# whatshap/whatshap

Measured on AMD Instinct MI355X. Metric: variant-columns/sec at max-coverage 20 (bipartition-costs/sec reported alongside), higher is better.
Workload: dtype u32; 1 GPU; synthetic diploid single-individual, max-coverage 20: 1 block of 200000 SNVs (BASELINE configs[2]); blocks=1, blocks_in_flight_per_gpu=1, tables_per_launch=1, max_coverage=20, optimal_cost_checksum=1611545, rendezvous=none

## Files before the change

### include/whatshap_amd_debug.h

```cpp
#ifndef WHATSHAP_AMD_DEBUG_H
#define WHATSHAP_AMD_DEBUG_H

#include "whatshap_amd.h"

#ifdef __cplusplus
extern "C" {
#endif

whamd_status_t whamd_debug_emulate_slot_plan(const whamd_readset_view* readset, const uint32_t* recombcost, size_t n_recombcost,
                                            const whamd_pedigree_view* pedigree, int distrust_genotypes,
                                            const uint32_t* positions, size_t n_positions, int slot_l, int symmetry,
                                            uint32_t* index_out, uint32_t* score_out, uint64_t* n_run_columns_out);

whamd_status_t whamd_debug_emulate_pedslot_plan(const whamd_readset_view* readset, const uint32_t* recombcost, size_t n_recombcost,
                                               const whamd_pedigree_view* pedigree, int distrust_genotypes,
                                               const uint32_t* positions, size_t n_positions, int slot_l,
                                               uint32_t* index_out, uint32_t* transmission_out, uint32_t* score_out,
                                               uint64_t* n_run_columns_out);

whamd_status_t whamd_debug_lazy_terms_check(const whamd_readset_view* readset, const uint32_t* recombcost, size_t n_recombcost,
                                            const whamd_pedigree_view* pedigree, int distrust_genotypes,
                                            const uint32_t* positions, size_t n_positions, const uint8_t* need, int rounds,
                                            int* lazy_out, uint64_t* differences_out, uint64_t* built_before_out, uint64_t* built_after_out);

// ... 22 lines not shown
whamd_status_t whamd_debug_progeny_gl_host(const whamd_progeny_depths_view* problems, uint64_t n_problems, float* const* table_out,
                                           double* const* table_f64_out);

whamd_status_t whamd_debug_haplotag_host(const whamd_haplotag_view* problems, uint64_t n_problems, whamd_haplotag_result** out);

whamd_status_t whamd_debug_poly_reorder_host(const whamd_poly_reorder_view* problems, uint64_t n_problems, double log_match, double log_err,
                                             whamd_poly_reorder_result** out);

whamd_status_t whamd_debug_poly_compare_host(const whamd_poly_compare_view* jobs, uint64_t n_jobs, whamd_poly_compare_result** out);

whamd_status_t whamd_debug_tagphase_host(const whamd_tagphase_view* problems, uint64_t n_problems, whamd_tagphase_result** out);

whamd_status_t whamd_debug_prior_genotypes_host(const whamd_prior_genotypes_view* problems, uint64_t n_problems, whamd_prior_genotypes_result** out);

typedef struct whamd_debug_kernel {
	const void* kernel;
	const char* name;
	int32_t large_lds_opted_in;
	int32_t debug_only;
} whamd_debug_kernel;
size_t whamd_debug_solve_kernels(whamd_debug_kernel* out, size_t capacity);

enum {
	WHAMD_LAUNCH_COLUMN = 0,
	WHAMD_LAUNCH_RUN = 1,
	WHAMD_LAUNCH_SLOT_RUN = 2,
	WHAMD_LAUNCH_BATCH = 3,
	WHAMD_LAUNCH_GROUP = 4,
	WHAMD_LAUNCH_GROUP_WALK = 5,
	WHAMD_LAUNCH_TAIL = 6,
	WHAMD_LAUNCH_WINDOW_WALK = 7,
	WHAMD_LAUNCH_TABLES = 8
};

typedef struct whamd_debug_launch {
	const void* kernel;
	uint32_t site;
	uint32_t grid_x, grid_y, block;
	uint32_t lds;
	uint32_t own_stream;
	uint32_t forward;
	int32_t lr, yflags, spec, stamps, tb, nf, ncols, threads;
	int32_t streamed, pack;
	int32_t tight, variant;
	int32_t T, n_ind, mode, wide;
	int32_t ped, sym;
	int32_t entries;
	int32_t preview;
	int32_t reserved;
	uint64_t count;
	const char* name;
} whamd_debug_launch;
whamd_status_t whamd_debug_dptable_launches(const whamd_dptable* table, whamd_debug_launch* out, size_t capacity, size_t* n_out);

typedef struct whamd_debug_preview {
	int32_t ran, continued;
	uint32_t pieces, launched_steps, agreed_steps, from_hook;
	const char* why_not;
} whamd_debug_preview;
whamd_status_t whamd_debug_dptable_preview(const whamd_dptable* table, whamd_debug_preview* out);

typedef struct whamd_debug_preview_plan_result {
	uint32_t n_pieces, pieces, steps, n_steps;
	int32_t chunked_predicted, chunked, windowed, reserved;
	uint32_t n_seeds_predicted, n_seeds, stride_predicted, stride;
	uint64_t arena_predicted, arena_laid_out, exchange_predicted, exchange_laid_out;
	const char* why_not;
} whamd_debug_preview_plan_result;
whamd_status_t whamd_debug_preview_plan(const whamd_readset_view* readset, const uint32_t* recombcost, size_t n_recombcost,
                                        const whamd_pedigree_view* pedigree, int distrust_genotypes,
                                        const uint32_t* positions, size_t n_positions, uint32_t pieces, whamd_debug_preview_plan_result* out,
                                        uint64_t* rec_predicted, uint64_t* rec_laid_out, uint32_t* spec_predicted, uint32_t* spec_laid_out, size_t capacity);

typedef struct whamd_debug_head_plan_result {
	uint32_t n_pieces, head_steps, n_steps, hook_calls;
	uint64_t digest, head_digest_in_hook, head_digest;
	uint32_t edge_yflags[2];
	uint32_t n_runs, n_components;
} whamd_debug_head_plan_result;
whamd_status_t whamd_debug_head_first_plan(const whamd_readset_view* readset, const uint32_t* recombcost, size_t n_recombcost,
                                           const whamd_pedigree_view* pedigree, int distrust_genotypes,
                                           const uint32_t* positions, size_t n_positions, uint32_t head_pieces, whamd_debug_head_plan_result* out);

typedef struct whamd_debug_genotype_run {
	uint32_t c0, ncols;
	uint32_t rescale_f, rescale_b, emit_f, emit_b;
	uint32_t n_part_out, part_out_f, part_out_b;
	uint32_t part_in_f, n_part_in_f, part_in_b, n_part_in_b;
	uint32_t reserved;
} whamd_debug_genotype_run;
whamd_status_t whamd_debug_genotype_run_plan(const whamd_readset_view* readset, const uint32_t* recombcost, size_t n_recombcost,
                                             const whamd_pedigree_view* pedigree, const uint32_t* positions, size_t n_positions,
                                             whamd_debug_genotype_run* out, size_t capacity, size_t* n_out, double* min_total_out);

whamd_status_t whamd_debug_poly_thread_inputs_host(const whamd_poly_thread_view* problems, uint64_t n_problems, whamd_poly_thread_result** out);
whamd_status_t whamd_debug_poly_select_clusters_host(uint64_t n_pos, const uint64_t* pc_ptr, const uint32_t* pc_cluster, const uint32_t* pc_total, uint32_t ploidy,
                                                     uint32_t max_cluster_gap, uint64_t* cov_ptr_out, uint32_t* cluster_out, uint8_t* readded_out, uint32_t* rank_out);
whamd_status_t whamd_debug_poly_haplotypes_host(const uint32_t* paths, uint64_t n_pos, uint32_t ploidy, const uint64_t* pc_ptr, const uint32_t* pc_cluster,
                                                const int8_t* pc_consensus, int8_t* haplotypes_out);

#ifdef __cplusplus
}
#endif

#endif
```

### whatshap_amd/_native.py

```python

from __future__ import annotations

import ctypes as C
import os
import threading
from typing import Optional, Sequence

import numpy as np

_HERE = os.path.dirname(os.path.abspath(__file__))
LIB_PATH = os.path.join(_HERE, "libwhatshap_amd.so")
DEBUG_LIB_PATH = os.path.join(_HERE, "libwhatshap_amd_debug.so")
ABI_VERSION = 3

WHAMD_OK = 0
WHAMD_ERR_INVALID = 1
WHAMD_ERR_MENDELIAN_CONFLICT = 2
WHAMD_ERR_UNSORTED = 3
WHAMD_ERR_UNSUPPORTED = 4
WHAMD_ERR_DEVICE = 5
WHAMD_ERR_OVERFLOW = 6
WHAMD_ERR_HOST = 7
GT_OTHER = 255

# ... 813 lines not shown
        except Exception:
            pass

    def positions(self) -> np.ndarray:
        out = np.zeros(self.n_columns, dtype=np.uint32)
        _check(self._L.whamd_dptable_positions(self._h, _ptr(out, C.c_uint32)))
        return out

    def optimal_score(self) -> int:
        v = C.c_uint32()
        _check(self._L.whamd_dptable_get_optimal_score(self._h, C.byref(v)))
        return int(v.value)

    def super_reads(self):
        n, ni = self.n_columns, self.n_individuals
        a0 = np.zeros((ni, n), dtype=np.uint8)
        a1 = np.zeros((ni, n), dtype=np.uint8)
        q = np.zeros((ni, n), dtype=np.uint32)
        tv = np.zeros(n, dtype=np.uint32)
        sid = np.zeros(ni, dtype=np.uint32)
        _check(self._L.whamd_dptable_get_super_reads(
            self._h, _ptr(a0, C.c_uint8), _ptr(a1, C.c_uint8), _ptr(q, C.c_uint32), _ptr(tv, C.c_uint32), _ptr(sid, C.c_uint32)))
        return a0, a1, q, tv, sid

    def partitioning(self) -> np.ndarray:
        out = np.zeros(self.n_reads, dtype=np.uint8)
        _check(self._L.whamd_dptable_get_optimal_partitioning(self._h, _ptr(out, C.c_uint8)))
        return out

    def index_path(self):
        idx = np.zeros(self.n_columns, dtype=np.uint32)
        tv = np.zeros(self.n_columns, dtype=np.uint32)
        _check(self._L.whamd_dptable_get_index_path(self._h, _ptr(idx, C.c_uint32), _ptr(tv, C.c_uint32)))
        return idx, tv

    def stats(self) -> dict:
        s = SolveStats()
        _check(self._L.whamd_dptable_get_stats(self._h, C.byref(s)))
        return s.as_dict()


def plan_summary(problem: ProblemArrays, path: str = "auto") -> dict:
    out = PlanSummary()
    _check(lib().whamd_plan_summarize(*problem.call_args(), path.encode(), C.byref(out)))
    return out.as_dict()


def emulate_slot_plan(problem: ProblemArrays, n_columns: int, slot_l: int = 11, symmetry: int = 1, slot_r: int = 2):
    if slot_r >= 3:
        slot_l += 100
    elif slot_r <= 1:
        slot_l += 200
    idx = np.zeros(max(n_columns, 1), dtype=np.uint32)
    score = C.c_uint32()
    ncols = C.c_uint64()
    D = debug_lib()
    _check(D.whamd_debug_emulate_slot_plan(*problem.call_args(), C.c_int(slot_l), C.c_int(symmetry), _ptr(idx, C.c_uint32),
                                           C.byref(score), C.byref(ncols)), D)
    return idx[:n_columns], int(score.value), int(ncols.value)


def emulate_pedslot_plan(problem: ProblemArrays, n_columns: int, slot_l: int = 0):
    idx = np.zeros(max(n_columns, 1), dtype=np.uint32)
    trans = np.zeros(max(n_columns, 1), dtype=np.uint32)
    score = C.c_uint32()
    ncols = C.c_uint64()
    D = debug_lib()
    _check(D.whamd_debug_emulate_pedslot_plan(*problem.call_args(), C.c_int(slot_l), _ptr(idx, C.c_uint32), _ptr(trans, C.c_uint32),
                                              C.byref(score), C.byref(ncols)), D)
    return idx[:n_columns], trans[:n_columns], int(score.value), int(ncols.value)


def debug_lazy_terms_check(problem: ProblemArrays, need=None, rounds: int = 1) -> dict:
    D = debug_lib()
    fn = D.whamd_debug_lazy_terms_check
    fn.restype = C.c_int
    lazy, diff, before, after = C.c_int(), C.c_uint64(), C.c_uint64(), C.c_uint64()
    need_arr = None if need is None else np.ascontiguousarray(need, dtype=np.uint8)
    _check(fn(*problem.call_args(), None if need_arr is None else _ptr(need_arr, C.c_uint8), C.c_int(int(rounds)), C.byref(lazy), C.byref(diff),
              C.byref(before), C.byref(after)), D)
    return {"lazy": bool(lazy.value), "differences": int(diff.value), "built_before": int(before.value), "built_after": int(after.value)}


class DebugGenotypeRun(C.Structure):
    _fields_ = [(name, C.c_uint32) for name in ("c0", "ncols", "rescale_f", "rescale_b", "emit_f", "emit_b", "n_part_out", "part_out_f", "part_out_b",
                                                "part_in_f", "n_part_in_f", "part_in_b", "n_part_in_b", "reserved")]


def debug_genotype_run_plan(problem: ProblemArrays):
    D = debug_lib()
    fn = D.whamd_debug_genotype_run_plan
    fn.restype = C.c_int
    a = problem.call_args()
    args = (a[0], a[1], a[2], a[3], a[5], a[6])
    n, min_total = C.c_size_t(), C.c_double()
    status = fn(*args, None, C.c_size_t(0), C.byref(n), C.byref(min_total))
    if status == WHAMD_ERR_UNSUPPORTED:
        return None
    _check(status, D)
    runs = (DebugGenotypeRun * max(n.value, 1))()
    _check(fn(*args, runs, C.c_size_t(n.value), C.byref(n), C.byref(min_total)), D)
    names = [f[0] for f in DebugGenotypeRun._fields_ if f[0] != "reserved"]
    return [{k: int(getattr(runs[i], k)) for k in names} for i in range(n.value)], float(min_total.value)


class DebugKernel(C.Structure):
    _fields_ = [("kernel", C.c_void_p), ("name", C.c_char_p), ("large_lds_opted_in", C.c_int32), ("debug_only", C.c_int32)]


LAUNCH_SITES = ("column", "run", "slot_run", "batch", "group", "group_walk", "tail", "window_walk", "tables")
LAUNCH_FACTS = ("lr", "yflags", "spec", "stamps", "tb", "nf", "ncols", "threads", "streamed", "pack", "tight", "variant", "T", "n_ind", "mode", "wide",
                "ped", "sym", "entries")


class DebugLaunch(C.Structure):
    _fields_ = ([("kernel", C.c_void_p), ("site", C.c_uint32), ("grid_x", C.c_uint32), ("grid_y", C.c_uint32), ("block", C.c_uint32), ("lds", C.c_uint32),
                 ("own_stream", C.c_uint32), ("forward", C.c_uint32)] + [(f, C.c_int32) for f in LAUNCH_FACTS] +
                [("preview", C.c_int32), ("reserved", C.c_int32), ("count", C.c_uint64), ("name", C.c_char_p)])


class DebugPreview(C.Structure):
    _fields_ = [("ran", C.c_int32), ("continued", C.c_int32), ("pieces", C.c_uint32), ("launched_steps", C.c_uint32), ("agreed_steps", C.c_uint32),
                ("from_hook", C.c_uint32), ("why_not", C.c_char_p)]


def debug_preview(table) -> dict:
    D = debug_lib()
    if table._L is not D:
        raise ValueError("the preview's record exists in the debug library only (use_debug_library() before the table is made)")
    out = DebugPreview()
    _check(D.whamd_debug_dptable_preview(table._h, C.byref(out)), D)
    return {"ran": bool(out.ran), "continued": bool(out.continued), "pieces": int(out.pieces), "launched_steps": int(out.launched_steps),
            "agreed_steps": int(out.agreed_steps), "from_hook": bool(out.from_hook), "why_not": (out.why_not or b"").decode()}


class DebugHeadPlan(C.Structure):
    _fields_ = [("n_pieces", C.c_uint32), ("head_steps", C.c_uint32), ("n_steps", C.c_uint32), ("hook_calls", C.c_uint32),
                ("digest", C.c_uint64), ("head_digest_in_hook", C.c_uint64), ("head_digest", C.c_uint64),
                ("edge_yflags", C.c_uint32 * 2), ("n_runs", C.c_uint32), ("n_components", C.c_uint32)]


def debug_head_first_plan(problem: ProblemArrays, head_pieces: int = 0) -> dict:
    D = debug_lib()
    fn = D.whamd_debug_head_first_plan
    fn.restype = C.c_int
    out = DebugHeadPlan()
    _check(fn(*problem.call_args(), C.c_uint32(head_pieces), C.byref(out)), D)
    rec = {name: int(getattr(out, name)) for name, _ in DebugHeadPlan._fields_ if name != "edge_yflags"}
    rec["edge_yflags"] = tuple(None if v == 0xFFFFFFFF else int(v) for v in out.edge_yflags)
    return rec


class DebugPreviewPlan(C.Structure):
    _fields_ = [("n_pieces", C.c_uint32), ("pieces", C.c_uint32), ("steps", C.c_uint32), ("n_steps", C.c_uint32),
                ("chunked_predicted", C.c_int32), ("chunked", C.c_int32), ("windowed", C.c_int32), ("reserved", C.c_int32),
                ("n_seeds_predicted", C.c_uint32), ("n_seeds", C.c_uint32), ("stride_predicted", C.c_uint32), ("stride", C.c_uint32),
                ("arena_predicted", C.c_uint64), ("arena_laid_out", C.c_uint64), ("exchange_predicted", C.c_uint64), ("exchange_laid_out", C.c_uint64),
                ("why_not", C.c_char_p)]


def debug_preview_plan(problem: ProblemArrays, pieces: int = 0) -> dict:
    D = debug_lib()
    fn = D.whamd_debug_preview_plan
    fn.restype = C.c_int
    out = DebugPreviewPlan()
    _check(fn(*problem.call_args(), C.c_uint32(pieces), C.byref(out), None, None, None, None, C.c_size_t(0)), D)
# ... 182 lines not shown
```

### whatshap_amd/csrc/c_api.cpp

```cpp
#include <cstdio>
#include <cstdlib>
#include <cstring>
#include <functional>
#include <memory>
#include <new>
#include <stdexcept>
#include <string>

#include "api_guard.h"
#include "debug_build.h"
#ifdef WHAMD_DEBUG_BUILD
#include "../../include/whatshap_amd_debug.h"
#endif
#include "device_runtime.h"
#include "device_table.h"
#include "genotype.h"
#include "genotype_plan.h"
#include "heuristic.h"
#include "host_parallel.h"
#include "problem.h"
#include "resident.h"
#include "slots.h"
#include <algorithm>
#include <vector>

using namespace whamd;

struct whamd_dptable {
	Problem problem;
	Solution solution;
	DeviceTable device;
	whamd_solve_stats stats{};
	int device_index = 0;
	bool uploaded = false;
	bool solved = false;
	bool in_flight = false;
};

namespace {

thread_local std::string g_last_error;

}

namespace whamd {
void set_last_error(const std::string& msg) { g_last_error = msg; }
}

extern "C" {

int whamd_abi_version(void) { return WHAMD_ABI_VERSION; }

int whamd_device_count(void) { return DeviceTable::device_count(); }

whamd_status_t whamd_device_pci_bus_id(int device, char* out, size_t capacity) {
	if (!out || capacity < 16) return fail(WHAMD_ERR_INVALID, "whamd_device_pci_bus_id: buffer of at least 16 bytes expected");
	std::string id;
	if (!DeviceTable::device_pci_bus_id(device, id)) return fail(WHAMD_ERR_DEVICE, "no HIP device " + std::to_string(device));
	if (id.size() + 1 > capacity) return fail(WHAMD_ERR_INVALID, "whamd_device_pci_bus_id: buffer too small");
	std::memcpy(out, id.c_str(), id.size() + 1);
	return WHAMD_OK;
}

const char* whamd_last_error(void) { return g_last_error.c_str(); }

namespace {
whamd_status_t apply_option(whamd_dptable* t, const std::string& k, const char* value);

whamd_status_t create_table(const whamd_readset_view* readset, const uint32_t* recombcost, size_t n_recombcost, const whamd_pedigree_view* pedigree,
                            int distrust_genotypes, const uint32_t* positions, size_t n_positions, const char* const* keys, const char* const* values,
                            size_t n_options, int device, whamd_dptable** out) {
	if (!out) return fail(WHAMD_ERR_INVALID, "out is NULL");
	*out = nullptr;
	if (n_options && (!keys || !values)) return fail(WHAMD_ERR_INVALID, "option arrays are NULL");
	const double t0 = now_ms();
	std::unique_ptr<whamd_dptable> t(new whamd_dptable());
	std::string msg;
	struct ThreadsGuard { uint32_t saved = whamd::host_threads_override(); ~ThreadsGuard() { whamd::host_threads_override() = saved; } } threads_guard;
	for (size_t i = 0; i < n_options; ++i) {
		if (!keys[i] || !values[i]) return fail(WHAMD_ERR_INVALID, "null option");
		if (std::string(keys[i]) == "host_threads") whamd::host_threads_override() = (uint32_t)std::max(0, std::atoi(values[i]));
	}
	whamd_status_t st = build_problem(readset, recombcost, n_recombcost, pedigree, distrust_genotypes != 0,
	                                  positions, n_positions, t->problem, msg, false, true);
	if (st != WHAMD_OK) return fail(st, msg);
	const double t1 = now_ms();
	t->device_index = device;
	t->device.set_thread_budget(whamd::host_threads_override() != 0);
	for (size_t i = 0; i < n_options; ++i) {
		if (std::string(keys[i]) == "host_threads") continue;
		st = apply_option(t.get(), keys[i], values[i]);
		if (st != WHAMD_OK) return st;
	}
	st = t->device.upload(t->problem, device, msg, true);
	if (st != WHAMD_OK) return fail(st, msg);
	if (getenv("WHAMD_DEBUG_TIMING"))
		fprintf(stderr, "[whamd timing] create: flatten %.1f ms, plan + upload %.1f ms\n", t1 - t0, now_ms() - t1);
	t->uploaded = true;
	t->stats.host_prepare_ms = now_ms() - t0;
	t->stats.host_flatten_ms = t1 - t0;
	*out = t.release();
	return WHAMD_OK;
}
}

whamd_status_t whamd_dptable_create(const whamd_readset_view* readset, const uint32_t* recombcost,
                                    size_t n_recombcost, const whamd_pedigree_view* pedigree,
                                    int distrust_genotypes, const uint32_t* positions, size_t n_positions,
                                    int device, whamd_dptable** out) {
	return guarded([&]() -> whamd_status_t {
		return create_table(readset, recombcost, n_recombcost, pedigree, distrust_genotypes, positions, n_positions, nullptr, nullptr, 0, device, out);
	});
}

whamd_status_t whamd_dptable_create_with_options(const whamd_readset_view* readset, const uint32_t* recombcost,
                                                 size_t n_recombcost, const whamd_pedigree_view* pedigree,
                                                 int distrust_genotypes, const uint32_t* positions, size_t n_positions,
                                                 const char* const* keys, const char* const* values, size_t n_options,
                                                 int device, whamd_dptable** out) {
	return guarded([&]() -> whamd_status_t {
		return create_table(readset, recombcost, n_recombcost, pedigree, distrust_genotypes, positions, n_positions, keys, values, n_options, device, out);
	});
}

namespace {

whamd_status_t begin_enqueue(whamd_dptable* t) {
	if (!t) return fail(WHAMD_ERR_INVALID, "table is NULL");
	if (t->in_flight) return fail(WHAMD_ERR_INVALID, "a solve of this table is already in flight");
	std::string msg;
	if (!t->uploaded) {
		whamd_status_t st = t->device.upload(t->problem, t->device_index, msg);
		if (st != WHAMD_OK) return fail(st, msg);
		t->uploaded = true;
	}
	const Problem& p = t->problem;
	whamd_solve_stats& s = t->stats;
	s.n_columns = p.n_cols;
	s.n_cells = p.n_cells;
	s.n_costs = p.n_cells * p.T;
	s.algorithmic_bytes = p.algorithmic_bytes;
	s.max_coverage = p.max_k;
	s.transmissions = p.T;
	t->solved = false;
	return WHAMD_OK;
}

}

whamd_status_t whamd_dptable_enqueue(whamd_dptable* t) {
	return guarded([&]() -> whamd_status_t {
	whamd_status_t st = begin_enqueue(t);
	if (st != WHAMD_OK) return st;
	std::string msg;
	t->device.set_side_by_side(false);
	st = t->device.enqueue(t->problem, t->solution, msg);
	if (st != WHAMD_OK) return fail(st, msg);
	t->in_flight = true;
// ... 479 lines not shown
			if (rc.mode != RES_MODE_GENERIC) s.n_vectorised_columns++;
			if (rc.nfold) ok = ok && rc.nfold <= RES_MAXFOLD && i >= rc.nfold;
			ok = ok && c + 1 < p.n_cols;
		}
		ok = ok && stage == sg.stage_words;
		const uint64_t lds = sg.kind == 1
			? (((uint64_t)sg.ncols * (PED_LDSWORDS + PED_TABLE) + (uint64_t)sg.n_terms * 2 + 3) & ~3ull) * 4 + 2 * (16ull << sg.max_l) + (uint64_t)sg.stage_words * 8
			: (uint64_t)sg.ncols * (64 + RES_TABLE) * 4 + 2 * (4ull << sg.max_l) + (uint64_t)sg.stage_words * 8;
		ok = ok && lds <= 160 * 1024;
		s.max_lds_bytes = std::max<uint64_t>(s.max_lds_bytes, lds);
		s.max_run_columns = std::max<uint64_t>(s.max_run_columns, sg.ncols);
		s.max_workgroups = std::max<uint64_t>(s.max_workgroups, 1ull << (sg.g - sg.half));
		if (sg.half) s.n_halved_runs++;
		s.n_resident_columns += sg.ncols;
		s.backtrace_bytes += (uint64_t)sg.stage_words * (1ull << sg.g) * 8;
	}
	ok = ok && expect == p.n_cols;
	for (uint32_t c = 0; c < p.n_cols; ++c) ok = ok && seen[c] == 1;
	s.invariants_ok = ok ? 1 : 0;
	*out = s;
	return WHAMD_OK;
	});
}

#ifdef WHAMD_DEBUG_BUILD
whamd_status_t whamd_debug_emulate_slot_plan(const whamd_readset_view* readset, const uint32_t* recombcost, size_t n_recombcost,
                                            const whamd_pedigree_view* pedigree, int distrust_genotypes, const uint32_t* positions,
                                            size_t n_positions, int slot_l, int symmetry, uint32_t* index_out, uint32_t* score_out,
                                            uint64_t* n_run_columns_out) {
	return guarded([&]() -> whamd_status_t {
	const int lr = slot_l >= 200 ? 1 : slot_l >= 100 ? 3 : 2;
	if (slot_l >= 100) slot_l -= slot_l >= 200 ? 200 : 100;
	Problem p;
	std::string msg;
	whamd_status_t st = build_problem(readset, recombcost, n_recombcost, pedigree, distrust_genotypes != 0, positions,
	                                  n_positions, p, msg);
	if (st != WHAMD_OK) return fail(st, msg);
	SlotPlan sp;
	if (p.T != 1 || !plan_forward_slots(p, slot_l, symmetry, sp, lr)) return fail(WHAMD_ERR_UNSUPPORTED, "slot runs apply to a single individual only");
	std::vector<uint32_t> path;
	uint32_t score = 0;
	if (!emulate_slot_plan(p, sp, path, score, msg)) return fail(WHAMD_ERR_INVALID, "slot plan inconsistent: " + msg);
	if (index_out && !path.empty()) std::memcpy(index_out, path.data(), path.size() * sizeof(uint32_t));
	if (score_out) *score_out = score;
	if (n_run_columns_out) *n_run_columns_out = sp.n_run_columns;
	return WHAMD_OK;
	});
}

whamd_status_t whamd_debug_emulate_pedslot_plan(const whamd_readset_view* readset, const uint32_t* recombcost, size_t n_recombcost,
                                               const whamd_pedigree_view* pedigree, int distrust_genotypes, const uint32_t* positions,
                                               size_t n_positions, int slot_l, uint32_t* index_out, uint32_t* transmission_out,
                                               uint32_t* score_out, uint64_t* n_run_columns_out) {
	return guarded([&]() -> whamd_status_t {
	Problem p;
	std::string msg;
	whamd_status_t st = build_problem(readset, recombcost, n_recombcost, pedigree, distrust_genotypes != 0, positions,
	                                  n_positions, p, msg);
	if (st != WHAMD_OK) return fail(st, msg);
	SlotPlan sp;
	if (p.T == 1 || !plan_forward_slots(p, slot_l > 0 ? -slot_l : 0, 0, sp) || !sp.ped)
		return fail(WHAMD_ERR_UNSUPPORTED, "pedigree slot runs apply to tables with one or two trios whose columns need at most 4 cost forms per transmission value");
	std::vector<uint32_t> path, trans;
	uint32_t score = 0;
	if (!emulate_pedslot_plan(p, sp, path, trans, score, msg)) return fail(WHAMD_ERR_INVALID, "pedigree slot plan inconsistent: " + msg);
	if (index_out && !path.empty()) std::memcpy(index_out, path.data(), path.size() * sizeof(uint32_t));
	if (transmission_out && !trans.empty()) std::memcpy(transmission_out, trans.data(), trans.size() * sizeof(uint32_t));
	if (score_out) *score_out = score;
	if (n_run_columns_out) *n_run_columns_out = sp.n_run_columns;
	return WHAMD_OK;
	});
}
whamd_status_t whamd_debug_lazy_terms_check(const whamd_readset_view* readset, const uint32_t* recombcost, size_t n_recombcost,
                                            const whamd_pedigree_view* pedigree, int distrust_genotypes, const uint32_t* positions, size_t n_positions,
                                            const uint8_t* need_in, int rounds, int* lazy_out, uint64_t* differences_out, uint64_t* built_before_out,
                                            uint64_t* built_after_out) {
	return guarded([&]() -> whamd_status_t {
	Problem eager, lazy;
	std::string msg;
	whamd_status_t st = build_problem(readset, recombcost, n_recombcost, pedigree, distrust_genotypes != 0, positions, n_positions, eager, msg);
	if (st != WHAMD_OK) return fail(st, msg);
	st = build_problem(readset, recombcost, n_recombcost, pedigree, distrust_genotypes != 0, positions, n_positions, lazy, msg, false, true);
	if (st != WHAMD_OK) return fail(st, msg);
	if (lazy_out) *lazy_out = lazy.lazy_terms ? 1 : 0;
	const uint32_t n = eager.n_cols;
	uint64_t before = 0, after = 0, diff = 0;
	for (uint32_t c = 0; c < n; ++c) before += lazy.term_end(c, lazy.T - 1) > lazy.term_begin(c, 0);
	std::vector<uint8_t> need(n, 1);
	if (need_in) for (uint32_t c = 0; c < n; ++c) need[c] = need_in[c] != 0;
	rounds = std::max(1, rounds);
	for (int r = 0; r < rounds; ++r) {
		std::vector<uint8_t> part(n, 0);
		for (uint32_t c = 0; c < n; ++c) part[c] = need[c] && (int)(c % (uint32_t)rounds) == r;
		st = fill_lazy_terms(lazy, part, msg);
		if (st != WHAMD_OK) return fail(st, msg);
	}
	for (uint32_t c = 0; c < n; ++c) {
		after += lazy.term_end(c, lazy.T - 1) > lazy.term_begin(c, 0);
		if (!need[c]) continue;
		bool same = true;
		for (uint32_t t = 0; t < eager.T && same; ++t) {
			const uint64_t a0 = eager.term_begin(c, t), a1 = eager.term_end(c, t), b0 = lazy.term_begin(c, t), b1 = lazy.term_end(c, t);
			same = a1 - a0 == b1 - b0;
			for (uint64_t i = 0; same && i < a1 - a0; ++i)
				same = eager.terms[a0 + i].c == lazy.terms[b0 + i].c && eager.terms[a0 + i].plus == lazy.terms[b0 + i].plus && eager.terms[a0 + i].minus == lazy.terms[b0 + i].minus;
		}
		diff += !same;
	}
	if (eager.fterm_kind != lazy.fterm_kind || eager.fterms.size() != lazy.fterms.size()) diff += n;
	else for (size_t i = 0; i < eager.fterms.size(); ++i) if (eager.fterms[i].c != lazy.fterms[i].c || eager.fterms[i].plus != lazy.fterms[i].plus || eager.fterms[i].minus != lazy.fterms[i].minus) { ++diff; break; }
	if (lazy.value_bound < eager.value_bound) diff += n;
	if (differences_out) *differences_out = diff;
	if (built_before_out) *built_before_out = before;
	if (built_after_out) *built_after_out = after;
	return WHAMD_OK;
	});
}

size_t whamd_debug_solve_kernels(whamd_debug_kernel* out, size_t capacity) { return DeviceTable::debug_solve_kernels(out, capacity); }

whamd_status_t whamd_debug_dptable_launches(const whamd_dptable* table, whamd_debug_launch* out, size_t capacity, size_t* n_out) {
	if (!table || !n_out) return fail(WHAMD_ERR_INVALID, "null argument");
	if (!table->solved) return fail(WHAMD_ERR_INVALID, "the table has not been solved: its ledger is read after whamd_dptable_wait");
	*n_out = table->device.debug_launches(out, capacity);
	return WHAMD_OK;
}

whamd_status_t whamd_debug_dptable_preview(const whamd_dptable* table, whamd_debug_preview* out) {
	if (!table || !out) return fail(WHAMD_ERR_INVALID, "null argument");
	table->device.debug_preview(out);
	return WHAMD_OK;
}

whamd_status_t whamd_debug_preview_plan(const whamd_readset_view* readset, const uint32_t* recombcost, size_t n_recombcost,
                                        const whamd_pedigree_view* pedigree, int distrust_genotypes,
                                        const uint32_t* positions, size_t n_positions, uint32_t pieces, whamd_debug_preview_plan_result* out,
                                        uint64_t* rec_predicted, uint64_t* rec_laid_out, uint32_t* spec_predicted, uint32_t* spec_laid_out, size_t capacity) {
	return guarded([&]() -> whamd_status_t {
	if (!out) return fail(WHAMD_ERR_INVALID, "out is NULL");
	Problem p;
	std::string msg;
	whamd_status_t st = build_problem(readset, recombcost, n_recombcost, pedigree, distrust_genotypes != 0, positions, n_positions, p, msg);
	if (st != WHAMD_OK) return fail(st, msg);
	st = DeviceTable::debug_preview_plan(p, pieces, out, rec_predicted, rec_laid_out, spec_predicted, spec_laid_out, capacity, msg);
	return st == WHAMD_OK ? WHAMD_OK : fail(st, msg);
	});
}

whamd_status_t whamd_debug_head_first_plan(const whamd_readset_view* readset, const uint32_t* recombcost, size_t n_recombcost,
                                           const whamd_pedigree_view* pedigree, int distrust_genotypes,
                                           const uint32_t* positions, size_t n_positions, uint32_t head_pieces, whamd_debug_head_plan_result* out) {
	return guarded([&]() -> whamd_status_t {
	if (!out) return fail(WHAMD_ERR_INVALID, "out is NULL");
	Problem p;
	std::string msg;
	whamd_status_t st = build_problem(readset, recombcost, n_recombcost, pedigree, distrust_genotypes != 0, positions, n_positions, p, msg);
	if (st != WHAMD_OK) return fail(st, msg);
	if (p.T != 1) return fail(WHAMD_ERR_UNSUPPORTED, "the head hook applies to a single individual only");
	*out = whamd_debug_head_plan_result{};
	auto mix = [](uint64_t& h, const void* data, size_t bytes) {
		const unsigned char* b = static_cast<const unsigned char*>(data);
		for (size_t i = 0; i < bytes; ++i) h = (h ^ b[i]) * 1099511628211ull;
	};
	auto runs_digest = [&mix](const SlotPlan& sp, size_t n_runs) {
		uint64_t h = 1469598103934665603ull;
		for (size_t ri = 0; ri < n_runs; ++ri) {
			const SlotRun& run = sp.runs[ri];
			mix(h, &run, sizeof run);
			mix(h, sp.rows.data() + run.row_off, (size_t)run.ncols * sizeof(SlotRow));
			mix(h, sp.bt_cols.data() + run.row_off, (size_t)run.ncols * sizeof(SlotBtCol));
			mix(h, sp.ctrl.data() + run.ctrl_off, (size_t)SLOT_CTRL_WORDS * 4);
			mix(h, sp.end_slots.data() + sp.end_off[ri], run.n_ends);
		}
		return h;
	};
	SlotPlan sp;
	SlotPlanHead head;
	const uint32_t n_pieces = slot_plan_pieces(p.n_cols);
	head.col_limit = slot_plan_piece_begin(p.n_cols, std::min(head_pieces, n_pieces));
	uint32_t calls = 0, head_steps = 0;
	uint64_t in_hook = 0;
	head.at_head = [&](uint32_t n_head) {
		++calls;
		head_steps = n_head;
		in_hook = runs_digest(sp, n_head);
	};
	if (!plan_forward_slots(p, 11, 1, sp, 2, false, head_pieces ? &head : nullptr)) return fail(WHAMD_ERR_UNSUPPORTED, "the table is not eligible for slot runs");
	out->n_pieces = n_pieces;
	out->head_steps = head_steps;
	out->n_steps = (uint32_t)sp.steps.size();
	out->hook_calls = calls;
	out->head_digest_in_hook = in_hook;
	out->head_digest = runs_digest(sp, head_steps);
	out->n_runs = (uint32_t)sp.runs.size();
	out->n_components = (uint32_t)sp.component_first_step.size();
	uint64_t h = runs_digest(sp, sp.runs.size());
	mix(h, sp.steps.data(), sp.steps.size() * sizeof(Step));
	mix(h, sp.end_off.data(), sp.end_off.size() * 4);
	mix(h, sp.start_slots.data(), sp.start_slots.size());
	mix(h, sp.start_off.data(), sp.start_off.size() * 4);
	mix(h, sp.f_exit.data(), sp.f_exit.size() * 4);
	for (const std::vector<uint8_t>& e : sp.exit_slot) mix(h, e.data(), e.size());
	mix(h, sp.col_to_row.data(), sp.col_to_row.size() * 4);
	mix(h, sp.component_first_step.data(), sp.component_first_step.size() * 4);
	mix(h, &sp.n_run_columns, sizeof sp.n_run_columns);
	out->digest = h;
	out->edge_yflags[0] = out->edge_yflags[1] = 0xFFFFFFFFu;
	if (head_steps) {
		out->edge_yflags[0] = sp.runs[head_steps - 1].yflags;
		if (head_steps < sp.steps.size() && sp.steps[head_steps].kind == 2) out->edge_yflags[1] = sp.runs[sp.steps[head_steps].index].yflags;
	}
	return WHAMD_OK;
	});
}

whamd_status_t whamd_debug_genotype_run_plan(const whamd_readset_view* readset, const uint32_t* recombcost, size_t n_recombcost,
                                             const whamd_pedigree_view* pedigree, const uint32_t* positions, size_t n_positions,
                                             whamd_debug_genotype_run* out, size_t capacity, size_t* n_out, double* min_total_out) {
	return guarded([&]() -> whamd_status_t {
	if (!n_out) return fail(WHAMD_ERR_INVALID, "n_out is NULL");
	Problem p;
	std::string msg;
	whamd_status_t st = build_problem(readset, recombcost, n_recombcost, pedigree, false, positions, n_positions, p, msg, true);
	if (st != WHAMD_OK) return fail(st, msg);
	GenotypeModel model;
	st = build_genotype_model(p, model, msg);
	if (st != WHAMD_OK) return fail(st, msg);
	GenoRunPlan pl;
// ... 259 lines not shown
```

### whatshap_amd/csrc/dp_device.hip

```cpp
#include <hip/hip_runtime.h>

#include <algorithm>
#include <atomic>
#include <cctype>
#include <chrono>
#include <cstdio>
#include <cstdlib>
#include <cstring>
#include <mutex>
#include <string>
#include <vector>

#include "debug_build.h"
#ifdef WHAMD_DEBUG_BUILD
#include "../../include/whatshap_amd_debug.h"
#endif
#include "device_runtime.h"
#include "device_table.h"
#include "genotype.h"
#include "table_plan.h"

namespace whamd {

namespace {
// ... 354 lines not shown

whamd_status_t DeviceTable::Impl::open(int dev, std::string& msg) {
	Impl& m = *this;
	m.device = dev;
	const whamd_status_t opened = open_device(dev, msg);
	if (opened != WHAMD_OK) return opened;
	if (!m.stream) {
		StreamSet ss;
		if (!streamset_take(dev, ss)) { msg = "could not create the table's stream and events"; return WHAMD_ERR_DEVICE; }
		m.adopt(ss);
	}
	m.release();
	if (!m.counted && dev >= 0 && dev < 64) { Impl::tables_on_device[dev].fetch_add(1); m.counted = true; }
	return WHAMD_OK;
}

whamd_status_t DeviceTable::Impl::choose_plan(Problem& p, TableBuild& b, bool from_create, std::string& msg) {
	Impl& m = *this;
	m.preview.tried = false;
	m.preview.from_hook = false;
	m.tp.wide = !select_kernels(p.T, p.n_ind, m.fused, m.keysfn);
	if (m.tp.wide && (p.T > (uint32_t)MAX_T_WIDE || p.n_ind > (uint32_t)MAX_IND_WIDE)) {
		msg = "no device kernel for T=" + std::to_string(p.T) + ", individuals=" + std::to_string(p.n_ind);
		return WHAMD_ERR_UNSUPPORTED;
	}
	for (uint32_t c = 0; c < p.n_cols && !m.tp.wide; ++c) m.tp.wide = p.term_end(c, p.T - 1) - p.term_begin(c, 0) > (uint64_t)COL_MAXTERMS;
	b.laps.lap("plan: kernels chosen, term counts scanned");
	b.force_keys = m.opt.path == "column_keys" || m.tp.wide;
	const bool want_resident = (m.opt.path == "auto" || m.opt.path == "resident") && !m.tp.wide;
	size_t free_b = 0, total_b = 0;
	HIP_TRY(hipMemGetInfo(&free_b, &total_b));
	if (free_b < total_b / 2) {
		genotype_release_cache();
		HIP_TRY(hipMemGetInfo(&free_b, &total_b));
	}
	if (free_b < total_b / 4) {
		arena_release();
		devpool_release();
		HIP_TRY(hipMemGetInfo(&free_b, &total_b));
	}
	free_b += arena_idle_bytes(m.device);
	b.free_b = free_b;
	b.laps.lap("plan: free device memory asked");
	int slot_lr = m.opt.slot_lr, slot_l = m.opt.slot_l;
	if (m.opt.shared_hint && p.T == 1 && p.max_k >= 18 && !m.opt.slot_l_set && m.opt.slot_lr == 2) { slot_lr = 3; slot_l = 12; }
	if (p.T == 1 && p.max_k >= 21 && p.max_k <= 22 && !m.opt.slot_l_set && m.opt.slot_lr == 2 && !debug_env("WHAMD_NO_WIDE_LAYOUT")) { slot_lr = 3; slot_l = 12; }
	m.tp.slot_lr_used = slot_lr;
	whamd_status_t head_status = WHAMD_OK;
	bool steps_adopted = false;
	auto adopt_steps = [&]() {
		m.tp.plan = ResidentPlan();
		m.tp.plan.steps = m.tp.splan.steps;
		m.tp.plan.component_first_step = m.tp.splan.component_first_step;
		m.tp.plan.col_to_res.assign(p.n_cols, -1);
		steps_adopted = true;
	};
	SlotPlanHead head;
	{
		const uint32_t n_pieces = slot_plan_pieces(p.n_cols);
		const uint32_t pieces = std::min(n_pieces - 1, preview_pieces_of(m.opt.preview_pieces, n_pieces));
		head.col_limit = slot_plan_piece_begin(p.n_cols, pieces);
		head.at_head = [&](uint32_t n_head) {
			if (n_head == 0) return;
			m.tp.use_slots = true;
			m.tp.table_bytes = 0;
			adopt_steps();
			b.laps.lap("plan: the planner up to the head's callback");
			m.preview.tried = true;
			m.preview.from_hook = true;
			head_status = m.start_preview(p, b, from_create, msg);
			if (m.preview.why != PV_RAN) m.preview.from_hook = false;
		};
	}
	bool head_first = from_create && p.T == 1 && m.opt.preview_mode != 0 && slot_plan_pieces(p.n_cols) >= 2 && !m.opt.shared_hint && !m.opt.side_by_side && !debug_env("WHAMD_NO_PREVIEW") &&
	                  !debug_env("WHAMD_NO_HEAD_FIRST");
	if (head_first && m.opt.preview_mode < 0)
		head_first = !m.opt.thread_budget && slot_plan_pieces(p.n_cols) >= 8 && m.alone_on_device();
	m.tp.use_slots = (m.opt.path == "auto" || m.opt.path == "slots") && !m.tp.wide &&
	              plan_forward_slots(p, p.T > 1 ? (m.opt.slot_l_set ? -m.opt.slot_l : 0) : std::max(8, slot_l), m.opt.symmetry, m.tp.splan, slot_lr, false, head_first ? &head : nullptr);
	if (head_status != WHAMD_OK) return head_status;
	b.laps.lap("plan: the planner");
	if (m.tp.use_slots && m.tp.splan.ped && m.tp.splan.table_words * 4ull > free_b / 4) m.tp.use_slots = false;
	m.tp.table_bytes = m.tp.use_slots && m.tp.splan.ped ? m.tp.splan.table_words * 4ull : 0ull;
	if (p.lazy_terms) {
		std::vector<uint8_t> need(p.n_cols, 1);
		if (m.tp.use_slots && m.tp.splan.ped) for (uint32_t c = 0; c < p.n_cols; ++c) need[c] = m.tp.splan.col_to_row[c] < 0;
		const whamd_status_t st = fill_lazy_terms(p, need, msg);
		if (st != WHAMD_OK) return st;
	}
	if (m.tp.use_slots) {
		if (!steps_adopted) adopt_steps();
	} else {
		m.tp.splan = SlotPlan();
		plan_forward(p, want_resident, m.opt.l_pref, m.opt.fold, m.tp.plan, m.opt.symmetry);
	}
	m.tp.device_superreads = p.n_ind == 1 && p.T == 1 && p.P == 2 && !p.distrust && p.h2p.size() >= 2 && p.h2p[0] == 0 && p.h2p[1] == 1 && p.genotype.size() >= p.n_cols &&
	                      !debug_env("WHAMD_HOST_SUPERREADS");
	b.laps.lap("plan: steps adopted, lazy terms");
	return WHAMD_OK;
}

void DeviceTable::Impl::dump_plan(const Problem& p) const {
	const Impl& m = *this;
	for (const Step& st : m.tp.plan.steps) {
		if (st.kind == 0) { fprintf(stderr, "[plan] column %u k=%u b=%u f=%u\n", st.index, p.k[st.index], p.b[st.index], p.f[st.index]); continue; }
		if (st.kind == 2) {
			const SlotRun& r = m.tp.splan.runs[st.index];
			fprintf(stderr, "[plan] slot run c0=%u ncols=%u g=%u L=%u half=%u ends=%u has_prev=%u in_identity=%u in_half=%u mirror_pos=%u in_occ=%x out_occ=%x mirror_out=%u\n",
			        r.c0, r.ncols, r.g, r.L, r.half, r.n_ends, r.has_prev, r.in_identity, r.in_half, r.in_mirror_pos, r.in_occ, r.out_occ, r.mirror_out);
			if (m.tp.splan.ped) fprintf(stderr, "[plan]   pedigree run: T=%u forms per value=%u table words=%u record words per workgroup=%u\n", 1u << m.tp.splan.pextra[st.index].tb,
			                         m.tp.splan.pextra[st.index].nf, m.tp.splan.pextra[st.index].s_off + r.ncols * 64u * pslot_ns(m.tp.splan.pextra[st.index].nf), m.tp.splan.pextra[st.index].rec_words);
			continue;
		}
		const ResSegment& sgm = m.tp.plan.segments[st.index];
		fprintf(stderr, "[plan] run c0=%u ncols=%u g=%u threads=%u max_l=%u stage_words=%u\n", sgm.c0, sgm.ncols, sgm.g, sgm.threads, sgm.max_l, sgm.stage_words);
		for (uint32_t i = 0; i < sgm.ncols; ++i) {
			const ResColumn& rc = m.tp.plan.columns[sgm.col_off + i];
			const ResBacktrace& rb = m.tp.plan.backtrace[sgm.col_off + i];
			fprintf(stderr, "[plan]   col %u mode=%u nfold=%u Lb=%u Lf=%u ebits=%u epos0=%u nthr=%u stage_off=%u nwords=%u | bt layout=%u n_g=%u n_l=%u\n",
			        sgm.c0 + i, rc.mode, rc.nfold, rc.Lb, rc.Lf, rc.ebits, rc.epos[0], rc.nthr, rc.stage_off, rc.nwords, rb.layout, rb.n_g, rb.n_l);
		}
	}
}

whamd_status_t DeviceTable::Impl::upload_column_arrays(const Problem& p, TableBuild& b, TableUploader& up, std::string& msg) {
	Impl& m = *this;
	const uint32_t n = b.n;
	static_assert(sizeof(CostTerm) == sizeof(DevTerm), "Problem::terms / fterms are uploaded as they are");
	const RawVec<CostTerm>& terms = p.terms;
	const int32_t* delta_src = p.delta.data();
	size_t delta_count = (size_t)p.col_ptr[n] * p.n_ind;
	if (p.n_ind == 0) { b.delta_fallback.assign(std::max<size_t>(p.col_ptr[n], 1), 0); delta_src = b.delta_fallback.data(); delta_count = b.delta_fallback.size(); }
	const bool sparse_columns = m.tp.use_slots && !b.ped_slots && p.T == 1 && !m.tp.windowed && !debug_env("WHAMD_DENSE_COLUMN_UPLOAD");
	if (sparse_columns) {
		std::vector<std::pair<size_t, size_t>> pc_cols, pc_delta, pc_tptr, pc_terms;
		for (uint32_t c = 0; c < n;) {
			if (m.tp.splan.col_to_row[c] >= 0) { ++c; continue; }
			uint32_t e = c + 1;
			while (e < n && m.tp.splan.col_to_row[e] < 0) ++e;
			pc_cols.emplace_back((size_t)c * sizeof(DevColumn), (size_t)e * sizeof(DevColumn));
			pc_delta.emplace_back((size_t)p.col_ptr[c] * p.n_ind * sizeof(int32_t), (size_t)p.col_ptr[e] * p.n_ind * sizeof(int32_t));
			pc_tptr.emplace_back((size_t)c * (p.T + 1) * sizeof(uint32_t), (size_t)e * (p.T + 1) * sizeof(uint32_t));
			pc_terms.emplace_back((size_t)p.term_ptr[(size_t)c * p.T] * sizeof(DevTerm), (size_t)p.term_ptr[(size_t)e * p.T] * sizeof(DevTerm));
			c = e;
		}
		HIP_TRY(up.up_pieces((void**)&m.dev.d_cols, m.tp.cols.data(), m.tp.cols.size() * sizeof(DevColumn), pc_cols));
		if (m.tp.device_superreads) HIP_TRY(up.up((void**)&m.dev.dp.delta, delta_src, delta_count * sizeof(int32_t)));
		else HIP_TRY(up.up_pieces((void**)&m.dev.dp.delta, delta_src, delta_count * sizeof(int32_t), pc_delta));
		HIP_TRY(up.up_pieces((void**)&m.dev.dp.term_ptr, b.term_ptr32.data(), b.term_ptr32.size() * sizeof(uint32_t), pc_tptr));
		HIP_TRY(up.up_pieces((void**)&m.dev.dp.terms, terms.data(), terms.size() * sizeof(DevTerm), pc_terms));
	} else {
		HIP_TRY(up.up((void**)&m.dev.d_cols, m.tp.cols.data(), m.tp.cols.size() * sizeof(DevColumn)));
		HIP_TRY(up.up((void**)&m.dev.dp.delta, delta_src, delta_count * sizeof(int32_t)));
		HIP_TRY(up.up((void**)&m.dev.dp.term_ptr, b.term_ptr32.data(), b.term_ptr32.size() * sizeof(uint32_t)));
		HIP_TRY(up.up((void**)&m.dev.dp.terms, terms.data(), terms.size() * sizeof(DevTerm)));
	}
	m.dev.dp.cols = m.dev.d_cols;
	if (m.tp.device_superreads) {
		m.dev.super_args = SuperreadArgs{};
		HIP_TRY(up.up((void**)&m.dev.super_args.col_ptr, p.col_ptr.data(), ((size_t)n + 1) * sizeof(uint64_t)));
		HIP_TRY(up.up((void**)&m.dev.super_args.genotype, p.genotype.data(), (size_t)n));
		m.dev.super_args.delta = m.dev.dp.delta;
		m.dev.super_args.n_cols = n;
		m.tp.super_words = (size_t)n + ((size_t)2 * n + 3) / 4;
	}
	b.d_fterms = nullptr;
	if (!p.fterms.empty()) HIP_TRY(up.up((void**)&b.d_fterms, p.fterms.data(), p.fterms.size() * sizeof(DevTerm)));
// ... 280 lines not shown
	e.units = m.dev.d_units; e.chunks = m.dev.d_chunks;
	e.n_chunks = (uint32_t)m.tp.chunks.size(); e.n_units = (uint32_t)m.tp.units.size(); e.n_orient_max = m.tp.n_orient_max; e.n_cols = n;
	e.path2 = m.dev.d_path2; e.trans2 = m.dev.d_trans2; e.out_score = m.dev.d_score; e.unit_x2 = m.dev.d_unit_x; e.guess = m.dev.d_guess; e.sel = m.dev.d_sel; e.counters = m.dev.d_bt_counters;
	e.path_index = m.dev.d_path_index; e.path_trans = m.dev.d_path_trans;
	if (m.tp.device_superreads) e.super = m.dev.super_args;
	void* d_entry = nullptr;
	HIP_TRY(up.alloc(&d_entry, sizeof(BtGroupEntry)));
	HIP_TRY(hipMemcpyAsync(d_entry, &m.dev.h_bt_entry, sizeof(BtGroupEntry), hipMemcpyHostToDevice, up.stream));
	HIP_TRY(hipEventRecord(m.ev_upload, up.stream));
	m.dev.d_bt_entry = (BtGroupEntry*)d_entry;
	return WHAMD_OK;
}

whamd_status_t DeviceTable::Impl::start_preview(const Problem& p, TableBuild& b, bool from_create, std::string& msg) {
	Impl& m = *this;
	Preview& pv = m.preview;
	PreviewPlan pp;
	plan_preview(p, m.opt, b, m.tp, from_create, m.alone_on_device(), pp);
	pv.why = pp.why;
	if (pp.why != PV_RAN) return WHAMD_OK;
	const uint32_t n = b.n, S = pp.steps, pieces = pp.pieces, end_col = pp.end_col, n_spec = pp.n_spec, stride = pp.stride, max_f = pp.max_f;
	const uint64_t bt = pp.arena, tab_words = pp.tab_words;
	const size_t ctrl_words = pp.ctrl_words;
	const bool chunked = pp.chunked;
	const std::vector<uint64_t>& rec = pp.rec;
	const std::vector<uint32_t>& spec = pp.spec;
	const std::vector<SlotRun>& runs = m.tp.splan.runs;
	b.laps.lap("preview: steps, offsets, seeds (host)");
	{
		const whamd_status_t taken = m.take_arena(bt, msg);
		if (taken != WHAMD_OK) return taken;
	}
	pv.exchange_bytes = (size_t)(1ull << max_f) * p.T * 4;
	HIP_TRY(pool_alloc(m.device, m.dev.allocations, (void**)&pv.d_pr[0], pv.exchange_bytes));
	HIP_TRY(pool_alloc(m.device, m.dev.allocations, (void**)&pv.d_pr[1], pv.exchange_bytes));
	pv.spec_bytes = chunked ? ((size_t)n_spec + 1) * stride * 8 : 0;
	if (chunked) HIP_TRY(pool_alloc(m.device, m.dev.allocations, (void**)&pv.spec_keys, pv.spec_bytes));
	DevProblem hdp{};
	hdp.n_cols = n; hdp.T = p.T; hdp.tbits = b.tbits; hdp.n_ind = p.n_ind;
	{
		const hipStream_t us = m.upload_stream;
		TableUploader up(m.device, us, pv.allocations);
		const size_t row_count = (size_t)end_col + SLOT_ROW_PAD;
		up.open_block(row_count * sizeof(SlotRow) + ctrl_words * 4 + (size_t)S * sizeof(SlotRun) + 4096);
		const SlotRun* d_runs = nullptr;
		HIP_TRY(up.up((void**)&hdp.slot_rows, m.tp.splan.rows.data(), row_count * sizeof(SlotRow)));
		HIP_TRY(up.up((void**)&hdp.slot_ctrl, m.tp.splan.ctrl.data(), ctrl_words * 4));
		HIP_TRY(up.up((void**)&d_runs, runs.data(), (size_t)S * sizeof(SlotRun)));
		HIP_TRY(up.alloc((void**)&hdp.slot_tab, tab_words * 4));
		HIP_TRY(up.flush());
		uint32_t most = 0;
		for (uint32_t k = 0; k < S; ++k) most = std::max<uint32_t>(most, ((runs[k].ncols + 8u) << (runs[k].g - runs[k].half)) + (runs[k].ncols + 8u) * ((runs[k].threads >> 6) + 64u));
		const uint32_t bx = std::max(1u, std::min(64u, (most + 255u) / 256u));
		for (uint32_t r0 = 0; r0 < S; r0 += 32768) hipLaunchKernelGGL(slot_tables, dim3(bx, std::min<uint32_t>(32768, S - r0)), dim3(256), 0, us, hdp, d_runs + r0, (uint32_t*)hdp.slot_tab);
		HIP_TRY(hipGetLastError());
		HIP_TRY(hipEventRecord(m.ev_upload, us));
		if (up.unstaged_copies || !up.stage.image || !up.stage.park()) {
			HIP_TRY(hipStreamSynchronize(us));
			up.stage.finish();
		}
	}
	b.laps.lap("preview: rows, control words, tables: allocations + copies");
	{
		const whamd_status_t opted = opt_in_large_lds(m.device, msg);
		if (opted != WHAMD_OK) return opted;
	}
	const hipStream_t rs = m.stream;
	m.inflight.run_stream = rs;
	m.own_stream_used = true;
	HIP_TRY(hipStreamWaitEvent(rs, m.ev_upload, 0));
	hdp.bt = (uint8_t*)m.dev.d_arena;
	hdp.spec_keys = pv.spec_keys;
	hdp.spec_stride = stride;
	if (chunked) HIP_TRY(hipMemsetAsync(pv.spec_keys, 0xFF, pv.spec_bytes, rs));
	m.inflight.timing_pending = false;
	HIP_TRY(hipEventRecord(m.ev0, rs));
	m.tp.use_chunks = chunked;
#ifdef WHAMD_DEBUG_BUILD
	m.ledger.clear();
#endif
	pv.runs.resize(S);
	uint64_t launches = 0;
	pv.launching = true;
	if (b.laps.on)
		fprintf(stderr, "[whamd timing] preview: first launch %.2f ms after the create's upload began, at t = %.2f ms (%s)\n", b.laps.since_origin_ms(), timing_stamp_ms(),
		        pv.from_hook ? "from the planner's head hook" : "behind the plan");
	for (uint32_t k = 0; k < S; ++k) {
		SlotBatchEntry e{};
		e.run = runs[k];
		if (k == 0) e.run.has_prev = 0;
		e.run.rec_lo = (uint32_t)rec[k];
		e.run.rec_hi = (uint32_t)(rec[k] >> 32);
		e.run.spec_id = spec[k];
		e.prev = pv.d_pr[k & 1u];
		e.cur = pv.d_pr[(k & 1u) ^ 1u];
		pv.runs[k] = e.run;
		m.launch_slot_run(hdp, e, launches);
	}
	pv.launching = false;
	HIP_TRY(hipGetLastError());
	HIP_TRY(hipEventRecord(m.ev3, rs));
	pv.dp = hdp;
	pv.use_chunks = chunked;
	pv.why = PV_RAN;
	pv.pieces = pieces;
	pv.launched = S;
	pv.launches = launches;
	pv.pending = true;
	b.laps.lap("preview: launches submitted");
	return WHAMD_OK;
}

void DeviceTable::Impl::verify_preview() {
	Impl& m = *this;
	Preview& pv = m.preview;
	pv.agreed = 0;
	if (!pv.launched) return;
	const bool same_ground = m.tp.use_slots && !m.tp.windowed && m.tp.jobs.size() == 1 && m.tp.lanes.size() == 1 && m.dev.dp.bt == pv.dp.bt && m.dev.dp.spec_keys == pv.dp.spec_keys &&
	                         m.tp.use_chunks == pv.use_chunks && (!m.tp.use_chunks || m.dev.dp.spec_stride == pv.dp.spec_stride) && !m.dev.dp.dbg && !m.dev.dp.dbg_flags &&
	                         m.dev.d_pr[0] == pv.d_pr[0] && m.dev.d_pr[1] == pv.d_pr[1] && !m.opt.side_by_side;
	for (uint32_t k = 0; same_ground && k < pv.launched && k + 1 < m.tp.schedule.size(); ++k) {
		const SuperStep& ss = m.tp.schedule[k];
		if (ss.entry_count != 1 || !ss.singles.empty() || ss.ck_load >= 0 || ss.ck_save >= 0 || ss.bt_window >= 0) break;
		const SlotBatchEntry& e = m.tp.slot_entries[ss.entry_off];
		if (std::memcmp(&e.run, &pv.runs[k], sizeof(SlotRun)) != 0 || e.prev != pv.d_pr[k & 1u] || e.cur != pv.d_pr[(k & 1u) ^ 1u] || e.score_out) break;
		++pv.agreed;
	}
	if (const char* at = debug_env("WHAMD_PREVIEW_MISMATCH_AT")) pv.agreed = std::min<uint32_t>(pv.agreed, (uint32_t)std::max(0, atoi(at)));
	if (getenv("WHAMD_DEBUG_TIMING"))
		fprintf(stderr, "[whamd timing] preview: %u plan pieces, %u steps launched, %u agree with the schedule\n", pv.pieces, pv.launched, pv.agreed);
}

whamd_status_t DeviceTable::upload(Problem& p, int device, std::string& msg, bool from_create) {
	Impl& m = *impl_;
	whamd_status_t st = m.open(device, msg);
	if (st != WHAMD_OK || p.n_cols == 0) return st;
	TableBuild b;
	b.n = p.n_cols;
	b.tbits = 2 * p.n_triples;
	b.ni = std::max<uint32_t>(p.n_ind, 1);
	m.dev.dp.n_cols = b.n;
	m.dev.dp.T = p.T;
	m.dev.dp.tbits = b.tbits;
	m.dev.dp.n_ind = p.n_ind;
	m.upload_stream = debug_env("WHAMD_UPLOAD_ON_TABLE_STREAM") ? nullptr : upload_stream_of(device);
	if (!m.upload_stream) m.upload_stream = m.stream;
	if (m.upload_stream == m.stream) m.own_stream_used = true;
	if ((st = m.choose_plan(p, b, from_create, msg)) != WHAMD_OK) return st;
	b.ped_slots = m.tp.use_slots && m.tp.splan.ped;
	b.laps.next_stage();
	if (debug_env("WHAMD_DEBUG_PLAN")) m.dump_plan(p);
	if (!m.preview.tried && (st = m.start_preview(p, b, from_create, msg)) != WHAMD_OK) return st;
	if ((st = describe_columns(p, b, m.tp, msg)) != WHAMD_OK) return st;
	if ((st = lay_out_arena(p, m.opt, b, m.tp, msg)) != WHAMD_OK) return st;
	TableUploader up(device, m.upload_stream, m.dev.allocations);
	b.laps.lap("staging area taken");
	up.open_block(upload_bound(p, b, m.tp));
	b.laps.lap("staging image sized, device block taken");
	if ((st = m.upload_column_arrays(p, b, up, msg)) != WHAMD_OK) return st;
	if ((st = m.upload_slot_arrays(b, up, msg)) != WHAMD_OK) return st;
	make_jobs(m.opt, m.tp);
	make_units(b, m.tp);
	if ((st = m.make_windows(b, up, msg)) != WHAMD_OK) return st;
	if ((st = m.take_result_block(b.n, up, msg)) != WHAMD_OK) return st;
	if ((st = m.make_chunks(p, up, msg)) != WHAMD_OK) return st;
	if ((st = m.take_solve_buffers(p, b, up, msg)) != WHAMD_OK) return st;
	if ((st = m.make_lanes(b, up, msg)) != WHAMD_OK) return st;
	if ((st = make_schedule(b, m.dev.dp, m.dev.d_job_scores, m.tp, msg)) != WHAMD_OK) return st;
	make_briefs(m.tp);
	if ((st = m.upload_entries(up, msg)) != WHAMD_OK) return st;
	if ((st = m.launch_table_kernels(p, b, up, msg)) != WHAMD_OK) return st;
	b.laps.summary((double)b.bt / 1e9);
	if ((st = m.arm_debug_stamps(up, msg)) != WHAMD_OK) return st;
	if ((st = opt_in_large_lds(device, msg)) != WHAMD_OK) return st;
	if ((st = m.record_group_backtrace(b.n, up, msg)) != WHAMD_OK) return st;
	m.verify_preview();
	return WHAMD_OK;
}

namespace {

SegmentFn segment_kernel(bool stamps, bool sym) {
#ifdef WHAMD_DEBUG_BUILD
	if (stamps) return resident_segment<true, true>;
#endif
	return sym ? resident_segment<false, true> : resident_segment<false, false>;
}

PedSegmentFn ped_segment_kernel(bool stamps, bool spec) {
#ifdef WHAMD_DEBUG_BUILD
	if (stamps) return resident_segment_ped<true>;
#endif
	return spec ? resident_segment_ped<false, true> : resident_segment_ped<false>;
}

ResBatchFn resident_batch_kernel(bool sym) { return sym ? resident_batch<true> : resident_batch<false>; }

#ifdef WHAMD_DEBUG_BUILD
PedSlotRunFn pedslot_runx_kernel(uint32_t tb, uint32_t nf, uint32_t xc, bool spec) {
#define WHAMD_ROW(TB, NF) { pedslot_runx<TB, NF, 16, true>, pedslot_runx<TB, NF, 16, false>, pedslot_runx<TB, NF, 32, true>, pedslot_runx<TB, NF, 32, false> }
	static const PedSlotRunFn table[6][4] = {WHAMD_ROW(2, PSLOT_FACT), WHAMD_ROW(2, 16), WHAMD_ROW(2, 2), WHAMD_ROW(2, 4), WHAMD_ROW(4, 2), WHAMD_ROW(4, 4)};
#undef WHAMD_ROW
	const int row = tb == 2 ? (nf == (uint32_t)PSLOT_FACT ? 0 : nf == 16 ? 1 : nf == 2 ? 2 : 3) : (nf == 2 ? 4 : 5);
	return table[row][(xc == 16 ? 0 : 2) + (spec ? 0 : 1)];
}
#endif

PedSlotRunFn pedslot_run_kernel(uint32_t tb, uint32_t nf, bool spec, bool packed) {
#define WHAMD_ROW(TB, NF) { pedslot_run<TB, NF, true, true>, pedslot_run<TB, NF, true, false>, pedslot_run<TB, NF, false, true>, pedslot_run<TB, NF, false, false> }
	static const PedSlotRunFn table[7][4] = {WHAMD_ROW(2, PSLOT_FACT), WHAMD_ROW(4, PSLOT_FACT4), WHAMD_ROW(2, 16), WHAMD_ROW(2, 2), WHAMD_ROW(2, 4), WHAMD_ROW(4, 2), WHAMD_ROW(4, 4)};
#undef WHAMD_ROW
	const int row = tb == 2 && nf == (uint32_t)PSLOT_FACT ? 0 : tb == 4 && nf == (uint32_t)PSLOT_FACT4 ? 1 : tb == 2 ? (nf == 16 ? 2 : nf == 2 ? 3 : 4) : (nf == 2 ? 5 : 6);
	return table[row][(spec ? 0 : 2) + (packed ? 0 : 1)];
}

SlotRunXFn slot_runx_kernel(uint32_t xc, bool stamps, bool spec) {
#define WHAMD_PAIR(XC, STAMPS) { slot_runx<2, XC, STAMPS, true>, slot_runx<2, XC, STAMPS, false> }
#ifdef WHAMD_DEBUG_BUILD
	static const SlotRunXFn stamped[2][2] = {WHAMD_PAIR(24, true), WHAMD_PAIR(32, true)};
	if (stamps && xc) return stamped[xc == 24 ? 0 : 1][spec ? 0 : 1];
#endif
	static const SlotRunXFn table[5][2] = {WHAMD_PAIR(0, false), WHAMD_PAIR(8, false), WHAMD_PAIR(16, false), WHAMD_PAIR(24, false), WHAMD_PAIR(32, false)};
#undef WHAMD_PAIR
	return table[xc / 8][spec ? 0 : 1];
}

SlotRunFn slot_run_kernel(uint32_t lr, bool yform, bool stamps, bool spec) {
#ifdef WHAMD_DEBUG_BUILD
#define WHAMD_ROW(LR, YF) { slot_run<LR, true, true, YF>, slot_run<LR, true, false, YF>, slot_run<LR, false, true, YF>, slot_run<LR, false, false, YF> }
#else
#define WHAMD_ROW(LR, YF) { nullptr, nullptr, slot_run<LR, false, true, YF>, slot_run<LR, false, false, YF> }
#endif
	static const SlotRunFn table[5][4] = {WHAMD_ROW(3, true), WHAMD_ROW(3, false), WHAMD_ROW(1, false), WHAMD_ROW(2, true), WHAMD_ROW(2, false)};
#undef WHAMD_ROW
	const int row = lr == 3 ? (yform ? 0 : 1) : lr == 1 ? 2 : (yform ? 3 : 4);
	return table[row][(stamps ? 0 : 2) + (spec ? 0 : 1)];
}
// ... 861 lines not shown
```

### whatshap_amd/csrc/problem.cpp

```cpp
#include "debug_build.h"
#include "problem.h"

#include <algorithm>
#include <chrono>
#include <cmath>
#include <cstdio>
#include <cstdlib>
#include <cstring>
#include <thread>
#include <unordered_map>

namespace whamd {

namespace {

bool id_to_index(const Problem& p, uint32_t id, uint32_t& index, std::string& msg) {
	for (uint32_t i = p.n_ind; i-- > 0;) {
		if (p.individual_id[i] == id) {
			index = i;
			return true;
		}
	}
	msg = "Individual with ID " + std::to_string(id) + " not present in pedigree.";
	return false;
}

bool build_partitions(Problem& p, std::string& msg) {
	p.P = 2 * (p.n_ind - p.n_triples);
	p.h2p.assign((size_t)p.T * p.n_ind * 2, -1);
	std::vector<int> child_triple(p.n_ind, -1);
	for (uint32_t i = 0; i < p.n_triples; ++i) child_triple[p.triples[i][2]] = (int)i;
	std::vector<uint32_t> order;
	std::vector<uint8_t> state(p.n_ind, 0);
	for (uint32_t root = 0; root < p.n_ind; ++root) {
		std::vector<std::pair<uint32_t, int>> stack{{root, 0}};
		while (!stack.empty()) {
			auto [i, phase] = stack.back();
			stack.pop_back();
			if (state[i] == 2) continue;
			if (phase == 1) {
				state[i] = 2;
				order.push_back(i);
				continue;
			}
			if (state[i] == 1) {
				msg = "pedigree relationships contain a cycle";
				return false;
			}
			state[i] = 1;
			stack.push_back({i, 1});
			if (child_triple[i] >= 0) {
				stack.push_back({p.triples[child_triple[i]][1], 0});
				stack.push_back({p.triples[child_triple[i]][0], 0});
			}
		}
	}
	for (uint32_t t = 0; t < p.T; ++t) {
		int8_t* map = p.h2p.data() + (size_t)t * p.n_ind * 2;
		int next = 0;
		for (uint32_t i = 0; i < p.n_ind; ++i) {
			if (child_triple[i] < 0) {
				map[2 * i] = (int8_t)next;
				map[2 * i + 1] = (int8_t)(next + 1);
				next += 2;
			}
		}
		for (uint32_t i : order) {
			int ti = child_triple[i];
			if (ti < 0) continue;
			uint32_t father = p.triples[ti][0], mother = p.triples[ti][1];
			map[2 * i] = map[2 * father + (((t >> (2 * ti)) & 1) ? 0 : 1)];
			map[2 * i + 1] = map[2 * mother + (((t >> (2 * ti + 1)) & 1) ? 0 : 1)];
		}
	}
	return true;
}

}

whamd_status_t build_problem(const whamd_readset_view* rs, const uint32_t* recombcost, size_t n_recombcost,
                             const whamd_pedigree_view* ped, bool distrust, const uint32_t* positions,
                             size_t n_positions, Problem& p, std::string& msg, bool columns_only, bool lazy_fact_terms) {
	if (!rs || !ped) {
		msg = "null readset or pedigree view";
		return WHAMD_ERR_INVALID;
	}
	const bool timing = getenv("WHAMD_DEBUG_TIMING") != nullptr;
	auto lap_t = std::chrono::steady_clock::now();
	long lap_faults = timing ? thread_minor_faults() : 0;
	auto lap = [&](const char* what) {
		if (!timing) return;
		const auto now = std::chrono::steady_clock::now();
		const long faults = thread_minor_faults();
		fprintf(stderr, "[whamd timing]   flatten: %s %.2f ms (%ld page faults of this thread)\n", what, std::chrono::duration<double, std::milli>(now - lap_t).count(), faults - lap_faults);
		lap_faults = faults;
		lap_t = now;
	};
	p.n_reads = rs->n_reads;
	const uint64_t nnz = rs->n_reads ? rs->read_ptr[rs->n_reads] : 0;
	p.read_ptr.assign(rs->n_reads + 1, 0);
	if (rs->n_reads) std::copy(rs->read_ptr, rs->read_ptr + rs->n_reads + 1, p.read_ptr.begin());
	{
		const uint32_t n_threads = host_threads(nnz, 1u << 18);
		std::vector<uint8_t> bad(n_threads, 0);
		parallel_ranges(nnz, n_threads, [&](uint64_t i0, uint64_t i1, uint32_t t) {
			if (i1 <= i0) return;
			uint8_t worst = 0;
			for (uint64_t i = i0; i < i1; ++i) worst = std::max(worst, rs->var_allele[i]);
			bad[t] = worst > WHAMD_ALLELE_BLANK;
		});
		for (uint8_t v : bad) {
			if (v) {
				msg = "read allele must be 0 (REF), 1 (ALT) or 2 (BLANK)";
				return WHAMD_ERR_INVALID;
			}
		}
	}
	lap("copies of the read arrays");
	p.n_ind = ped->n_individuals;
	p.n_triples = ped->n_triples;
	p.n_variants = ped->n_variants;
	p.individual_id.assign(ped->individual_id, ped->individual_id + p.n_ind);
	const size_t ng = (size_t)p.n_ind * p.n_variants;
	if (ng) p.genotype.assign(ped->genotype, ped->genotype + ng);
	p.have_gl = ped->genotype_likelihoods != nullptr;
	if (p.have_gl && ng) {
		p.gl.assign(ped->genotype_likelihoods, ped->genotype_likelihoods + ng * 3);
		if (ped->gl_present) {
			for (size_t i = 0; i < ng; ++i) {
				if (!ped->gl_present[i]) p.gl[3 * i] = p.gl[3 * i + 1] = p.gl[3 * i + 2] = std::nan("");
			}
		}
	}
	p.distrust = distrust;
	p.triples.resize(p.n_triples);
	for (uint32_t i = 0; i < p.n_triples; ++i) {
		for (int m = 0; m < 3; ++m) {
			if (!id_to_index(p, ped->triple_ids[3 * i + m], p.triples[i][m], msg)) return WHAMD_ERR_INVALID;
		}
	}
	if (columns_only) {
		if (p.n_triples > 2 || p.n_ind > (uint32_t)MAX_IND) {
			msg = "pedigree too large for the genotyping device path (at most " + std::to_string(MAX_IND) + " individuals and 2 trios)";
			return WHAMD_ERR_UNSUPPORTED;
		}
	} else if (p.n_triples > (uint32_t)MAX_TRIPLES_WIDE || p.n_ind > (uint32_t)MAX_IND_WIDE || 2 * (p.n_ind - std::min(p.n_ind, p.n_triples)) > 14) {
		msg = "pedigree too large for the device path (at most " + std::to_string(MAX_IND_WIDE) + " individuals, " + std::to_string(MAX_TRIPLES_WIDE) +
		      " trios, 14 founder haplotypes)";
		return WHAMD_ERR_UNSUPPORTED;
	}
	p.T = 1u << (2 * p.n_triples);

	if (positions == nullptr) {
		p.positions.resize(nnz);
		for (uint64_t i = 0; i < nnz; ++i) p.positions[i] = (uint32_t)rs->var_position[i];
		std::sort(p.positions.begin(), p.positions.end());
		p.positions.erase(std::unique(p.positions.begin(), p.positions.end()), p.positions.end());
	} else {
		p.positions.assign(positions, positions + n_positions);
	}
	p.n_cols = (uint32_t)p.positions.size();
	const uint32_t n = p.n_cols;
	lap("pedigree + positions");
	bool positions_increase = true;
	for (uint32_t i = 1; i < n && positions_increase; ++i) positions_increase = p.positions[i - 1] < p.positions[i];
	std::unordered_map<uint32_t, uint32_t> position_map;
	if (!positions_increase) {
		position_map.reserve(n * 2 + 1);
		for (uint32_t i = 0; i < n; ++i) position_map[p.positions[i]] = i;
	}
	auto column_of = [&](uint32_t position, uint32_t& col, uint32_t hint = 0) -> bool {
		if (positions_increase) {
			if (n == 0) return false;
			const uint32_t* pos0 = p.positions.data();
			size_t lo_i = hint < n ? hint : 0, step = 1;
			if (pos0[lo_i] > position) lo_i = 0;
			size_t hi_i = lo_i;
			while (hi_i < n && pos0[hi_i] < position) { lo_i = hi_i; hi_i += step; step <<= 1; }
			if (hi_i > n) hi_i = n;
			const auto it = std::lower_bound(p.positions.begin() + lo_i, p.positions.begin() + hi_i + (hi_i < n ? 1 : 0), position);
			if (it == p.positions.end() || *it != position) return false;
			col = (uint32_t)(it - p.positions.begin());
			return true;
		}
		const auto it = position_map.find(position);
		if (it == position_map.end()) return false;
		col = it->second;
		return true;
	};
	p.read_first_col.resize(p.n_reads);
	p.read_last_col.resize(p.n_reads);
	std::vector<uint32_t>&first_col = p.read_first_col, &last_col = p.read_last_col;
	{
		struct ReadError { uint32_t read = 0xFFFFFFFFu; whamd_status_t status = WHAMD_OK; std::string msg; };
		const uint32_t n_threads = positions_increase ? host_threads(p.n_reads, 1u << 14) : 1u;
		std::vector<ReadError> errors(n_threads);
		const uint64_t* ptr = rs->read_ptr;
		const int32_t* vp = rs->var_position;
		parallel_ranges(p.n_reads, n_threads, [&](uint64_t r0, uint64_t r1, uint32_t t) {
			auto fail_read = [&](uint32_t r, whamd_status_t st, std::string m) { errors[t].read = r; errors[t].status = st; errors[t].msg = std::move(m); };
			uint32_t hint_col = 0;
			for (uint32_t r = (uint32_t)r0; r < (uint32_t)r1; ++r) {
				const uint64_t lo = ptr[r], hi = ptr[r + 1];
				if (hi <= lo || hi > nnz) return fail_read(r, WHAMD_ERR_INVALID, "No variants present");
				const int pos = r == 0 ? 0 : ((ptr[r] > ptr[r - 1] && ptr[r] <= nnz) ? vp[ptr[r - 1]] : 0);
				if (vp[lo] < pos) return fail_read(r, WHAMD_ERR_UNSORTED, "ColumnIterator: reads in ReadSet are not sorted.");
				for (uint64_t i = lo + 1; i < hi; ++i) {
					if (!(vp[i - 1] < vp[i])) return fail_read(r, WHAMD_ERR_UNSORTED, "ColumnIterator: encountered read with unsorted variants.");
				}
				uint32_t fc = 0, lc = 0;
				if (vp[lo] < 0 || !column_of((uint32_t)vp[lo], fc, hint_col) || !column_of((uint32_t)vp[hi - 1], lc, fc) || fc > lc) {
					return fail_read(r, WHAMD_ERR_INVALID, "read " + std::to_string(r) + " starts or ends at a position that is not in the position list");
				}
				first_col[r] = fc;
				last_col[r] = lc;
				hint_col = fc;
			}
		});
		for (const ReadError& e : errors) {
			if (e.status != WHAMD_OK) {
				msg = e.msg;
				return e.status;
			}
		}
	}
	if (!positions_increase) {
		msg = "positions must be strictly increasing";
		return WHAMD_ERR_INVALID;
	}
	lap("position map + read validation");
	p.read_source.resize(p.n_reads);
	for (uint32_t r = 0; r < p.n_reads; ++r) {
		if (!id_to_index(p, (uint32_t)rs->read_sample_id[r], p.read_source[r], msg)) return WHAMD_ERR_INVALID;
	}
	if (n && p.n_ind && p.n_variants < n) {
		msg = "pedigree has fewer variants (" + std::to_string(p.n_variants) + ") than there are columns (" + std::to_string(n) + ")";
		return WHAMD_ERR_INVALID;
	}
	if (n && p.n_ind && distrust) {
		bool ok = p.have_gl;
		for (uint32_t i = 0; ok && i < p.n_ind; ++i) {
			for (uint32_t c = 0; ok && c < n; ++c) {
				for (int g = 0; g < 3; ++g) {
					const double v = p.gl[((size_t)i * p.n_variants + c) * 3 + g];
					if (!(v >= 0.0 && v <= 1e9)) ok = false;
				}
			}
		}
		if (!ok) {
			msg = "distrust_genotypes requires genotype likelihoods in [0, 1e9] for every individual and column";
			return WHAMD_ERR_INVALID;
		}
	}
	p.recomb.assign(n, n_recombcost ? recombcost[n_recombcost - 1] : 0u);
	for (uint32_t c = 0; c < n && c < n_recombcost; ++c) p.recomb[c] = recombcost[c];

	if (!build_partitions(p, msg)) return WHAMD_ERR_INVALID;
	if (n == 0) return WHAMD_OK;

	std::vector<uint32_t> start_idx(n + 2, 0);
	p.col_ptr.assign(n + 1, 0);
	{
		std::vector<int64_t> diff(n + 1, 0);
		for (uint32_t r = 0; r < p.n_reads; ++r) {
			start_idx[first_col[r] + 1]++;
			diff[first_col[r]]++;
			diff[last_col[r] + 1]--;
		}
		for (uint32_t c = 0; c <= n; ++c) start_idx[c + 1] += start_idx[c];
		int64_t cov = 0;
		for (uint32_t c = 0; c < n; ++c) {
			cov += diff[c];
			if (cov > (int64_t)MAX_COVERAGE) {
				msg = "coverage " + std::to_string(cov) + " at column " + std::to_string(c) + " exceeds the device limit of " + std::to_string(MAX_COVERAGE);
				return WHAMD_ERR_UNSUPPORTED;
			}
			p.col_ptr[c + 1] = p.col_ptr[c] + (uint64_t)cov;
		}
	}
	lap("column pointers");
	p.entries.resize(p.col_ptr[n]);
	p.k.resize(n);
	p.b.resize(n);
	p.f.resize(n);
	p.fwd_mask.resize(n);
	if (!columns_only) {
		p.delta.resize((size_t)p.col_ptr[n] * std::max<uint32_t>(p.n_ind, 1));
		p.term_ptr.assign((size_t)n * p.T + 1, 0);
		p.terms.clear();
	}
	struct RangeResult {
		std::vector<CostTerm> terms;
		double bound = 0.0;
		uint64_t n_cells = 0, algorithmic_bytes = 0;
		uint32_t max_k = 0;
		bool conflict = false;
		bool fact_ok = true;
	};
	struct FactRoles {
		int child = -1, X = -1, Y = -1;
		bool oX = false, oY = false;
		uint32_t bx = 0, bx2 = 0, by = 0, by2 = 0;
		bool ok = false;
	};
	bool want_fact = distrust && p.n_ind == 3 && p.P == 4 && p.T == 4 && !columns_only && !getenv("WHAMD_NO_PED_FACT");
	FactRoles roles[4];
	for (uint32_t t = 0; t < 4 && want_fact; ++t) {
		const int8_t* map = p.h2p.data() + (size_t)t * p.n_ind * 2;
		const int8_t* map0 = p.h2p.data();
		FactRoles r;
		int n_children = 0;
		for (uint32_t s = 0; s < 3; ++s) {
			bool varies = false;
			for (uint32_t tt = 1; tt < p.T; ++tt) {
				const int8_t* mt = p.h2p.data() + (size_t)tt * p.n_ind * 2;
				varies = varies || mt[2 * s] != map0[2 * s] || mt[2 * s + 1] != map0[2 * s + 1];
			}
			if (varies) { r.child = (int)s; ++n_children; }
		}
		int nx = 0, ny = 0;
		for (uint32_t s = 0; s < 3 && n_children == 1; ++s) {
			if ((int)s == r.child) continue;
			for (int h = 0; h < 2; ++h) {
				if (map[2 * s + h] == map[2 * r.child]) { r.X = (int)s; r.oX = h == 0; r.bx = (uint32_t)map[2 * s + h]; r.bx2 = (uint32_t)map[2 * s + 1 - h]; ++nx; }
				if (map[2 * s + h] == map[2 * r.child + 1]) { r.Y = (int)s; r.oY = h == 0; r.by = (uint32_t)map[2 * s + h]; r.by2 = (uint32_t)map[2 * s + 1 - h]; ++ny; }
			}
		}
		r.ok = n_children == 1 && nx == 1 && ny == 1 && r.X != r.Y;
		if (!r.ok) want_fact = false;
		roles[t] = r;
	}
	if (want_fact) { p.fterms.resize((size_t)n * p.T * 16); p.fterm_kind = 1; }
	struct Fact4Roles {
		int X = -1, Y = -1, C1 = -1, C2 = -1;
		uint32_t px[2] = {0, 0}, py[2] = {0, 0};
		uint32_t u[2][16], v[2][16];
		bool ok = false;
	} roles4;
	bool want_fact4 = distrust && p.n_ind == 4 && p.P == 4 && p.T == 16 && p.n_triples == 2 && !columns_only && !getenv("WHAMD_NO_PED_FACT");
	if (want_fact4) {
		Fact4Roles& r = roles4;
		const int8_t* map0 = p.h2p.data();
		int n_children = 0;
		for (uint32_t s = 0; s < 4; ++s) {
			bool varies = false;
			for (uint32_t tt = 1; tt < p.T; ++tt) {
				const int8_t* mt = p.h2p.data() + (size_t)tt * p.n_ind * 2;
				varies = varies || mt[2 * s] != map0[2 * s] || mt[2 * s + 1] != map0[2 * s + 1];
			}
			if (varies) { (n_children == 0 ? r.C1 : r.C2) = (int)s; ++n_children; }
		}
		r.ok = n_children == 2;
		for (uint32_t s = 0; s < 4 && r.ok; ++s) {
			if ((int)s == r.C1 || (int)s == r.C2) continue;
			for (int h = 0; h < 2; ++h) {
				if (map0[2 * s + h] == map0[2 * r.C1]) r.X = (int)s;
				if (map0[2 * s + h] == map0[2 * r.C1 + 1]) r.Y = (int)s;
			}
		}
		r.ok = r.ok && r.X >= 0 && r.Y >= 0 && r.X != r.Y;
// ... 6 lines not shown
					const int c = k == 0 ? r.C1 : r.C2;
					const uint32_t h0 = (uint32_t)mt[2 * c], h1 = (uint32_t)mt[2 * c + 1];
					r.ok = (h0 == r.px[0] || h0 == r.px[1]) && (h1 == r.py[0] || h1 == r.py[1]);
					r.u[k][t] = h0 == r.px[1] ? 1u : 0u;
					r.v[k][t] = h1 == r.py[1] ? 1u : 0u;
				}
			}
		}
		want_fact4 = r.ok;
		if (want_fact4) {
			p.fterms.resize((size_t)n * 20);
			p.fterm_kind = 2;
			p.fact4_roles[0] = p.fact4_roles[1] = 0;
			for (uint32_t t = 0; t < 16; ++t) {
				p.fact4_roles[0] |= (r.u[0][t] << t) | (r.v[0][t] << (16 + t));
				p.fact4_roles[1] |= ((r.u[0][t] == r.u[1][t] ? 1u : 0u) << t) | ((r.v[0][t] == r.v[1][t] ? 1u : 0u) << (16 + t));
			}
		}
	}
	auto factorised_line4 = [&](uint32_t c, const std::vector<uint32_t>& R, const std::vector<uint32_t>& W) -> CostTerm* {
		const Fact4Roles& r = roles4;
		auto g = [&](int s, uint32_t k) { return (uint32_t)(0.0 + p.gl[((size_t)s * p.n_variants + c) * 3 + k]); };
		CostTerm* ft = p.fterms.data() + (size_t)c * 20;
		const int who[4] = {r.X, r.Y, r.C1, r.C2};
		for (int i = 0; i < 4; ++i) {
			const int s = who[i];
			ft[i] = CostTerm{0, 1u << s, 0};
			ft[4 + 4 * i + 0] = CostTerm{g(s, 0) + R[s], 0, 0};
			ft[4 + 4 * i + 1] = CostTerm{g(s, 1) + R[s], 0, 0};
			ft[4 + 4 * i + 2] = CostTerm{g(s, 1) + W[s] - R[s], 0, 0};
			ft[4 + 4 * i + 3] = CostTerm{g(s, 2) + W[s] - R[s], 0, 0};
		}
		return ft;
	};
	auto factorised_form4 = [&](const CostTerm* ft, uint32_t t, uint32_t asg) -> CostTerm {
		const Fact4Roles& r = roles4;
		const uint32_t a[2] = {(asg >> r.px[0]) & 1u, (asg >> r.px[1]) & 1u}, b[2] = {(asg >> r.py[0]) & 1u, (asg >> r.py[1]) & 1u};
		const uint32_t h[4][2] = {{a[0], a[1]}, {b[0], b[1]}, {a[r.u[0][t]], b[r.v[0][t]]}, {a[r.u[1][t]], b[r.v[1][t]]}};
		const int who[4] = {r.X, r.Y, r.C1, r.C2};
		CostTerm tm{0, 0, 0};
		for (int i = 0; i < 4; ++i) {
			tm.c += ft[4 + 4 * i + h[i][0] * 2 + h[i][1]].c;
			if (h[i][0] != h[i][1]) (h[i][0] == 0 ? tm.plus : tm.minus) |= 1u << who[i];
		}
		return tm;
	};
	auto factorised_line = [&](uint32_t c, uint32_t t, const std::vector<uint32_t>& R, const std::vector<uint32_t>& W) -> CostTerm* {
		const FactRoles& r = roles[t];
		auto g = [&](int s, uint32_t k) { return (uint32_t)(0.0 + p.gl[((size_t)s * p.n_variants + c) * 3 + k]); };
		CostTerm* ft = p.fterms.data() + ((size_t)c * p.T + t) * 16;
		auto signed_sum = [](int s, bool positive) { return positive ? CostTerm{0, 1u << s, 0} : CostTerm{0, 0, 1u << s}; };
		ft[0] = signed_sum(r.X, r.oX);
		ft[1] = signed_sum(r.Y, r.oY);
		ft[2] = signed_sum(r.child, true);
		ft[3] = CostTerm{0, 0, 0};
		auto founder = [&](int s, bool o, CostTerm* k) {
			k[0] = CostTerm{g(s, 0) + R[s], 0, 0};
			k[1] = CostTerm{g(s, 1) + (o ? R[s] : W[s] - R[s]), 0, 0};
			k[2] = CostTerm{g(s, 2) + W[s] - R[s], 0, 0};
			k[3] = CostTerm{g(s, 1) + (o ? W[s] - R[s] : R[s]), 0, 0};
		};
		founder(r.X, r.oX, ft + 4);
		founder(r.Y, r.oY, ft + 8);
		ft[12] = CostTerm{g(r.child, 0) + R[r.child], 0, 0};
		ft[13] = CostTerm{g(r.child, 1) + R[r.child], 0, 0};
		ft[14] = CostTerm{g(r.child, 1) + W[r.child] - R[r.child], 0, 0};
		ft[15] = CostTerm{g(r.child, 2) + W[r.child] - R[r.child], 0, 0};
		return ft;
	};
	auto factorised_form = [&](const CostTerm* ft, uint32_t t, uint32_t asg) -> CostTerm {
		const FactRoles& r = roles[t];
		const uint32_t a = (asg >> r.bx) & 1u, a2 = (asg >> r.bx2) & 1u, b = (asg >> r.by) & 1u, b2 = (asg >> r.by2) & 1u;
		CostTerm tm{0, 0, 0};
		tm.c = ft[4 + (a == 0 ? (a2 == 0 ? 0 : 1) : (a2 == 1 ? 2 : 3))].c + ft[8 + (b == 0 ? (b2 == 0 ? 0 : 1) : (b2 == 1 ? 2 : 3))].c + ft[12 + a * 2 + b].c;
		if (a != a2) ((a == 0) == r.oX ? tm.plus : tm.minus) |= 1u << r.X;
		if (b != b2) ((b == 0) == r.oY ? tm.plus : tm.minus) |= 1u << r.Y;
		if (a != b) (a == 0 ? tm.plus : tm.minus) |= 1u << r.child;
		return tm;
	};
	bool lazy = lazy_fact_terms && (want_fact || want_fact4) && !debug_env("WHAMD_EAGER_TERMS");
	auto lazy_sample = [](uint32_t c) { return c < 256u || (c & 63u) == 0u; };
	p.lazy_terms = false;
	const bool single_trusted = p.n_ind == 1 && p.T == 1 && p.P == 2 && !distrust && p.h2p.size() >= 2 && p.h2p[0] == 0 && p.h2p[1] == 1 && !debug_env("WHAMD_NO_SINGLE_FAST_TERMS");
	struct CompatCache {
		bool enabled = false;
		std::vector<uint8_t> known;
		std::vector<std::vector<uint8_t>> lists;
	};
	auto make_compat = [&]() {
		CompatCache cc;
		cc.enabled = !distrust && p.n_ind >= 2 && p.n_ind <= 6 && p.P <= 8 && !debug_env("WHAMD_NO_COMPAT_CACHE");
		if (cc.enabled) {
			const size_t slots = ((size_t)1 << (2 * p.n_ind)) * p.T;
			cc.known.assign(slots, 0);
			cc.lists.resize(slots);
		}
		return cc;
	};
	auto column_terms = [&](uint32_t c, RangeResult& out, std::vector<uint32_t>& R, std::vector<uint32_t>& W, CompatCache& compat) -> bool {
		const ColumnEntry* col = p.col_begin(c);
		const uint32_t kc = p.k[c];
		std::fill(R.begin(), R.end(), 0u);
		std::fill(W.begin(), W.end(), 0u);
		int32_t* dl = p.delta.data() + (size_t)p.col_ptr[c] * p.n_ind;
		double wsum = 0.0;
		if (p.n_ind == 1) {
			uint32_t w = 0, r = 0;
			uint64_t wide = 0;
			for (uint32_t j = 0; j < kc; ++j) {
				const ColumnEntry& e = col[j];
				const uint32_t q = e.allele == WHAMD_ALLELE_BLANK ? 0u : e.phred;
				const uint32_t alt = e.allele == WHAMD_ALLELE_ALT ? q : 0u;
				w += q;
				wide += q;
				r += alt;
				dl[j] = (int32_t)(q - 2u * alt);
			}
			W[0] = w;
			R[0] = r;
			wsum = (double)wide;
		} else {
		std::fill(dl, dl + (size_t)kc * p.n_ind, 0);
		uint64_t wide = 0;
		for (uint32_t j = 0; j < kc; ++j) {
			const ColumnEntry& e = col[j];
			const uint32_t q = e.allele == WHAMD_ALLELE_BLANK ? 0u : e.phred;
			const uint32_t alt = e.allele == WHAMD_ALLELE_ALT ? q : 0u;
			W[e.sample] += q;
			wide += q;
			R[e.sample] += alt;
			dl[(size_t)e.sample * kc + j] = (int32_t)(q - 2u * alt);
		}
		wsum = (double)wide;
		}
		double max_acost = 0.0;
		bool any = false;
		if (single_trusted) {
			const uint8_t g = p.genotype[c];
			if (g == 1) {
				out.terms.push_back(CostTerm{W[0] - R[0], 0, 1u});
				out.terms.push_back(CostTerm{R[0], 1u, 0});
				any = true;
			} else if (g == 0) {
				out.terms.push_back(CostTerm{R[0], 0, 0});
				any = true;
			} else if (g == 2) {
				out.terms.push_back(CostTerm{W[0] - R[0], 0, 0});
				any = true;
			}
			p.term_ptr[(size_t)c + 1] = out.terms.size();
		} else if (lazy && out.fact_ok && !lazy_sample(c)) {
			for (uint32_t t = 0; t < p.T; ++t) {
				if (want_fact) (void)factorised_line(c, t, R, W);
				else if (t == 0) (void)factorised_line4(c, R, W);
				p.term_ptr[(size_t)c * p.T + t + 1] = out.terms.size();
			}
			for (uint32_t s2 = 0; s2 < p.n_ind; ++s2) {
				const double* g3 = p.gl.data() + ((size_t)s2 * p.n_variants + c) * 3;
				max_acost += std::max(g3[0], std::max(g3[1], g3[2]));
			}
			any = true;
		} else
		for (uint32_t t = 0; t < p.T; ++t) {
			const int8_t* map = p.h2p.data() + (size_t)t * p.n_ind * 2;
			const size_t begin = out.terms.size();
			const CostTerm* fline = (want_fact && out.fact_ok) ? factorised_line(c, t, R, W) : nullptr;
			const CostTerm* fline4 = (want_fact4 && out.fact_ok) ? (t == 0 ? factorised_line4(c, R, W) : p.fterms.data() + (size_t)c * 20) : nullptr;
			const std::vector<uint8_t>* shortlist = nullptr;
			if (!distrust && compat.enabled) {
				uint32_t key = 0;
				for (uint32_t s = 0; s < p.n_ind; ++s) key = key * 4u + std::min<uint32_t>(p.genotype[(size_t)s * p.n_variants + c], 3u);
				const size_t slot = (size_t)key * p.T + t;
				if (!compat.known[slot]) {
					std::vector<uint8_t>& list = compat.lists[slot];
					for (uint32_t a = 0; a < (1u << p.P); ++a) {
						bool ok = true;
						for (uint32_t s = 0; s < p.n_ind && ok; ++s)
							ok = p.genotype[(size_t)s * p.n_variants + c] == ((a >> map[2 * s]) & 1) + ((a >> map[2 * s + 1]) & 1);
						if (ok) list.push_back((uint8_t)a);
					}
					compat.known[slot] = 1;
				}
				shortlist = &compat.lists[slot];
			}
			const uint32_t n_try = shortlist ? (uint32_t)shortlist->size() : (1u << p.P);
			for (uint32_t ai = 0; ai < n_try; ++ai) {
				const uint32_t a = shortlist ? (*shortlist)[ai] : ai;
				bool compatible = true;
				uint32_t acost = 0;
				CostTerm term{0, 0, 0};
				for (uint32_t s = 0; s < p.n_ind; ++s) {
					const uint32_t a0 = (a >> map[2 * s]) & 1, a1 = (a >> map[2 * s + 1]) & 1;
					const size_t gi = (size_t)s * p.n_variants + c;
					if (distrust) {
						acost = (uint32_t)((double)acost + p.gl[gi * 3 + a0 + a1]);
					} else if (p.genotype[gi] != a0 + a1) {
						compatible = false;
						break;
					}
					if (a0 == 0 && a1 == 0) term.c += R[s];
					else if (a0 == 1 && a1 == 1) term.c += W[s] - R[s];
					else if (a0 == 0) { term.c += R[s]; term.plus |= 1u << s; }
					else { term.c += W[s] - R[s]; term.minus |= 1u << s; }
				}
				if (!compatible) continue;
				term.c += acost;
				max_acost = std::max(max_acost, (double)acost);
				if (fline) {
					const CostTerm pred = factorised_form(fline, t, a);
					if (pred.c != term.c || pred.plus != term.plus || pred.minus != term.minus) { out.fact_ok = false; fline = nullptr; }
				}
				if (fline4) {
					const CostTerm pred = factorised_form4(fline4, t, a);
					if (pred.c != term.c || pred.plus != term.plus || pred.minus != term.minus) { out.fact_ok = false; fline4 = nullptr; }
				}
				bool dominated = false;
				for (size_t q = begin; q < out.terms.size(); ++q) {
					if (out.terms[q].plus == term.plus && out.terms[q].minus == term.minus) {
						if (term.c < out.terms[q].c) out.terms[q].c = term.c;
						dominated = true;
						break;
					}
				}
				if (!dominated) out.terms.push_back(term);
			}
			if (out.terms.size() > begin) any = true;
			p.term_ptr[(size_t)c * p.T + t + 1] = out.terms.size();
		}
		if (!any) {
			out.conflict = true;
			return false;
		}
		out.bound += wsum + max_acost + 2.0 * p.n_triples * (double)p.recomb[c];
		const uint64_t Tl = p.T;
		out.n_cells += 1ull << kc;
		out.algorithmic_bytes += (c > 0 ? 4 * Tl * (1ull << p.b[c]) : 0) + (c + 1 < n ? 12 * Tl * (1ull << p.f[c]) : 0) + 12ull * kc;
		return true;
	};
	auto columns_range = [&](uint32_t c_begin, uint32_t c_end, RangeResult& out) {
		if (c_begin >= c_end) return;
		out.terms.reserve(columns_only ? 0 : (size_t)(c_end - c_begin) * p.T * (distrust ? (size_t)1 << p.P : 2));
		std::vector<uint32_t> R(p.n_ind), W(p.n_ind);
		CompatCache compat = make_compat();
		const uint32_t width = c_end - c_begin;
		std::vector<uint8_t> cnt(width, 0);
		std::vector<uint32_t> masks(width, 0);
		for (uint32_t r = 0; r < start_idx[c_end]; ++r) {
			const uint32_t last = last_col[r];
			if (last < c_begin) continue;
			const uint32_t first = first_col[r];
			uint64_t v = p.read_ptr[r];
			if (first < c_begin) {
				const int32_t* lo = rs->var_position + p.read_ptr[r];
				const int32_t* hi = rs->var_position + p.read_ptr[r + 1];
				v = (uint64_t)(std::lower_bound(lo, hi, (int32_t)p.positions[c_begin]) - rs->var_position);
			}
			const uint8_t sample = (uint8_t)p.read_source[r];
			const uint32_t c_hi = std::min(last, c_end - 1u);
			for (uint32_t c = std::max(first, c_begin); c <= c_hi; ++c) {
				const int cpos = (int)p.positions[c];
				while (rs->var_position[v] < cpos) ++v;
				const uint32_t j = cnt[c - c_begin]++;
				ColumnEntry& e = p.entries[p.col_ptr[c] + j];
				e.read_id = r;
				e.sample = sample;
				if (rs->var_position[v] == cpos) {
					e.allele = rs->var_allele[v];
					e.phred = rs->var_quality[v];
				} else {
					e.allele = WHAMD_ALLELE_BLANK;
					e.phred = 0;
				}
				if (last > c) masks[c - c_begin] |= 1u << j;
			}
		}
		for (uint32_t c = c_begin; c < c_end; ++c) {
			const uint32_t kc = cnt[c - c_begin], mask = masks[c - c_begin];
			p.k[c] = (uint8_t)kc;
			p.b[c] = (uint8_t)(kc - (start_idx[c + 1] - start_idx[c]));
			p.fwd_mask[c] = mask;
			p.f[c] = (uint8_t)__builtin_popcount(mask);
			out.max_k = std::max(out.max_k, kc);
			if (!columns_only && !column_terms(c, out, R, W, compat)) return;
		}
	};
	double bound = 0.0;
	{
		const uint32_t n_threads = host_threads(n, 8192);
		std::vector<RangeResult> parts(n_threads);
		std::vector<uint32_t> bounds(n_threads + 1);
		for (uint32_t t = 0; t <= n_threads; ++t) bounds[t] = (uint32_t)((uint64_t)n * t / n_threads);
		parallel_ranges(n, n_threads, [&](uint64_t c0, uint64_t c1, uint32_t t) { columns_range((uint32_t)c0, (uint32_t)c1, parts[t]); });
		if (lazy) {
			bool all_ok = true;
			for (uint32_t t = 0; t < n_threads; ++t) all_ok = all_ok && parts[t].fact_ok;
			if (!all_ok) {
				lazy = false;
				for (RangeResult& part : parts) part = RangeResult();
				parallel_ranges(n, n_threads, [&](uint64_t c0, uint64_t c1, uint32_t t) { columns_range((uint32_t)c0, (uint32_t)c1, parts[t]); });
			}
		}
		p.lazy_terms = lazy;
		for (uint32_t t = 0; t < n_threads; ++t) p.max_k = std::max(p.max_k, parts[t].max_k);
		lap("column entries, indexing scheme, deltas + cost terms");
		if (columns_only) return WHAMD_OK;
		std::vector<uint64_t> base(n_threads + 1, 0);
		for (uint32_t t = 0; t < n_threads; ++t) {
			if (parts[t].conflict) {
				msg = "Error: Mendelian conflict";
				return WHAMD_ERR_MENDELIAN_CONFLICT;
			}
			base[t + 1] = base[t] + parts[t].terms.size();
			bound += parts[t].bound;
			if (!parts[t].fact_ok) { p.fterms.clear(); p.fterm_kind = 0; }
			p.n_cells += parts[t].n_cells;
			p.algorithmic_bytes += parts[t].algorithmic_bytes;
		}
		p.terms.resize(base[n_threads]);
		parallel_ranges(n_threads, n_threads, [&](uint64_t t0, uint64_t t1, uint32_t) {
			for (uint64_t t = t0; t < t1; ++t) {
				for (size_t i = (size_t)bounds[t] * p.T + 1; i <= (size_t)bounds[t + 1] * p.T; ++i) p.term_ptr[i] += base[t];
				if (!parts[t].terms.empty()) std::memcpy(p.terms.data() + base[t], parts[t].terms.data(), parts[t].terms.size() * sizeof(CostTerm));
			}
		});
	}
	lap("term lists joined");
	p.value_bound = bound;
	if (bound >= 4294967295.0) {
		msg = "costs may exceed 32 bits (upper bound " + std::to_string(bound) + "); the reference's unsigned arithmetic wraps there and results are undefined";
		return WHAMD_ERR_OVERFLOW;
	}
	return WHAMD_OK;
}

whamd_status_t fill_lazy_terms(Problem& p, const std::vector<uint8_t>& need, std::string& msg) {
	if (!p.lazy_terms) return WHAMD_OK;
	const uint32_t n = p.n_cols;
	if (p.terms_built.size() != n) {
		p.terms_built.assign(n, 0);
		for (uint32_t c = 0; c < n; ++c) p.terms_built[c] = p.term_end(c, p.T - 1) > p.term_begin(c, 0);
	}
	std::vector<uint32_t> todo;
	for (uint32_t c = 0; c < n; ++c) if (need[c] && !p.terms_built[c]) todo.push_back(c);
	if (todo.empty()) return WHAMD_OK;
	std::vector<std::vector<CostTerm>> fresh(todo.size());
	std::vector<std::vector<uint32_t>> fresh_count(todo.size());
	parallel_ranges(todo.size(), host_threads(todo.size(), 256), [&](uint64_t i0, uint64_t i1, uint32_t) {
		std::vector<uint32_t> R(p.n_ind), W(p.n_ind);
		for (size_t i = i0; i < i1; ++i) {
			const uint32_t c = todo[i];
			const ColumnEntry* col = p.col_begin(c);
			std::fill(R.begin(), R.end(), 0u);
			std::fill(W.begin(), W.end(), 0u);
			for (uint32_t j = 0; j < p.k[c]; ++j) {
				const ColumnEntry& e = col[j];
				if (e.allele == WHAMD_ALLELE_BLANK) continue;
				W[e.sample] += e.phred;
				if (e.allele == WHAMD_ALLELE_ALT) R[e.sample] += e.phred;
			}
			std::vector<CostTerm>& out = fresh[i];
			fresh_count[i].assign(p.T, 0);
			for (uint32_t t = 0; t < p.T; ++t) {
				const int8_t* map = p.h2p.data() + (size_t)t * p.n_ind * 2;
				const size_t begin = out.size();
				for (uint32_t a = 0; a < (1u << p.P); ++a) {
					bool compatible = true;
					uint32_t acost = 0;
					CostTerm term{0, 0, 0};
					for (uint32_t s = 0; s < p.n_ind; ++s) {
						const uint32_t a0 = (a >> map[2 * s]) & 1, a1 = (a >> map[2 * s + 1]) & 1;
						const size_t gi = (size_t)s * p.n_variants + c;
						if (p.distrust) acost = (uint32_t)((double)acost + p.gl[gi * 3 + a0 + a1]);
						else if (p.genotype[gi] != a0 + a1) { compatible = false; break; }
						if (a0 == 0 && a1 == 0) term.c += R[s];
						else if (a0 == 1 && a1 == 1) term.c += W[s] - R[s];
						else if (a0 == 0) { term.c += R[s]; term.plus |= 1u << s; }
						else { term.c += W[s] - R[s]; term.minus |= 1u << s; }
					}
					if (!compatible) continue;
					term.c += acost;
					bool dominated = false;
					for (size_t q = begin; q < out.size(); ++q) {
						if (out[q].plus == term.plus && out[q].minus == term.minus) {
							if (term.c < out[q].c) out[q].c = term.c;
							dominated = true;
							break;
						}
					}
					if (!dominated) out.push_back(term);
				}
				fresh_count[i][t] = (uint32_t)(out.size() - begin);
			}
		}
	});
	RawVec<CostTerm> merged;
	std::vector<uint64_t> ptr((size_t)n * p.T + 1, 0);
	size_t total = p.terms.size();
	for (const auto& v : fresh) total += v.size();
	merged.resize(total);
	size_t at = 0, ti = 0;
	for (uint32_t c = 0; c < n; ++c) {
		const bool is_new = ti < todo.size() && todo[ti] == c;
		size_t off = 0;
		for (uint32_t t = 0; t < p.T; ++t) {
			ptr[(size_t)c * p.T + t] = at;
			if (is_new) {
				const uint32_t cnt = fresh_count[ti][t];
				if (cnt) std::memcpy(merged.data() + at, fresh[ti].data() + off, cnt * sizeof(CostTerm));
				off += cnt;
				at += cnt;
			} else {
				const uint64_t b = p.term_begin(c, t), e = p.term_end(c, t);
				if (e > b) std::memcpy(merged.data() + at, p.terms.data() + b, (e - b) * sizeof(CostTerm));
				at += e - b;
			}
		}
		if (is_new) { p.terms_built[c] = 1; ++ti; }
	}
	ptr[(size_t)n * p.T] = at;
	merged.resize(at);
// ... 152 lines not shown
```

### whatshap_amd/csrc/problem.h

```cpp
#pragma once

#include <array>
#include <cstdint>
#include <string>
#include <vector>

#include "../../include/whatshap_amd.h"
#include "host_parallel.h"

namespace whamd {

constexpr uint32_t INF = 0xFFFFFFFFu;
constexpr int MAX_COVERAGE = 25;
constexpr int MAX_IND = 6;
constexpr int MAX_T = 16;
constexpr int MAX_IND_WIDE = 12;
constexpr int MAX_TRIPLES_WIDE = 3;
constexpr int MAX_T_WIDE = 64;

struct ColumnEntry {
	uint32_t read_id;
	uint32_t phred;
	uint8_t allele;
	uint8_t sample;
};

struct CostTerm {
	uint32_t c;
	uint32_t plus;
	uint32_t minus;
};

struct Problem {
	uint32_t n_reads = 0;
	std::vector<uint64_t> read_ptr;
	RawVec<int32_t> var_position;
	RawVec<uint8_t> var_allele;
	RawVec<uint32_t> var_quality;
	std::vector<uint32_t> read_source;
	std::vector<uint32_t> read_first_col, read_last_col;
	uint32_t n_ind = 0, n_triples = 0, n_variants = 0;
	std::vector<uint32_t> individual_id;
	std::vector<std::array<uint32_t, 3>> triples;
	std::vector<uint8_t> genotype;
	std::vector<double> gl;
	bool have_gl = false;
	bool distrust = false;
	std::vector<uint32_t> recomb;
	std::vector<uint32_t> positions;
	uint32_t n_cols = 0;
	uint32_t T = 1, P = 0;
	std::vector<int8_t> h2p;
	std::vector<uint64_t> col_ptr;
	RawVec<ColumnEntry> entries;
	std::vector<uint8_t> k, b, f;
	std::vector<uint32_t> fwd_mask;
	std::vector<uint64_t> term_ptr;
	RawVec<CostTerm> terms;
	RawVec<CostTerm> fterms;
	uint32_t fterm_kind = 0;
	bool lazy_terms = false;
	std::vector<uint8_t> terms_built;
	uint32_t fact4_roles[2] = {0, 0};
	RawVec<int32_t> delta;
	uint32_t max_k = 0;
	uint64_t n_cells = 0, algorithmic_bytes = 0;
	double value_bound = 0.0;

	const ColumnEntry* col_begin(uint32_t c) const { return entries.data() + col_ptr[c]; }
	uint64_t term_begin(uint32_t c, uint32_t t) const { return term_ptr[(size_t)c * T + t]; }
	uint64_t term_end(uint32_t c, uint32_t t) const { return term_ptr[(size_t)c * T + t + 1]; }
};

whamd_status_t build_problem(const whamd_readset_view* rs, const uint32_t* recombcost, size_t n_recombcost,
                             const whamd_pedigree_view* ped, bool distrust, const uint32_t* positions,
                             size_t n_positions, Problem& out, std::string& msg, bool columns_only = false, bool lazy_fact_terms = false);
whamd_status_t fill_lazy_terms(Problem& p, const std::vector<uint8_t>& need, std::string& msg);

struct Solution {
	uint32_t optimal_score = 0;
	std::vector<uint32_t> path_index, path_trans;
	std::vector<uint8_t> allele0, allele1;
	std::vector<uint32_t> quality;
	std::vector<uint8_t> partition;
	bool superreads_done = false;
};
whamd_status_t finish_solution(const Problem& p, Solution& s, std::string& msg);

}
```

### whatshap_amd/csrc/slot_plan.cpp

```cpp
#include <algorithm>
#include <cstdlib>
#include <cstring>
#include <chrono>
#include <iterator>
#include <cstdio>
#include <thread>

#include "debug_build.h"
#include "slots.h"
#include "genotype_plan.h"

namespace whamd {

namespace {

struct RunDraft {
	uint32_t c0 = 0, ncols = 0, g = 0, L = 0, lw = 0;
	std::vector<int32_t> entry_read;
	std::vector<int32_t> exit_read;
	bool symmetric = true;
};

inline uint32_t parity32(uint32_t v) { return (uint32_t)__builtin_popcount(v) & 1u; }

}

bool plan_forward_slots(const Problem& p, int l_pref, int use_symmetry, SlotPlan& plan, int lr, bool genotype_mode, const SlotPlanHead* head) {
	const auto tp0 = std::chrono::steady_clock::now();
	const long pf0 = thread_minor_faults();
	plan = SlotPlan();
	const uint32_t n = p.n_cols;
	const bool ped = p.T > 1 || genotype_mode;
	const uint32_t TB = p.T == 4 ? 2u : (p.T == 16 ? 4u : 0u);
	if (ped && !genotype_mode && (TB == 0 || p.n_ind < 3)) return false;
	if (genotype_mode && p.T != 1 && TB == 0) return false;
	if (!ped && !(p.T == 1 && p.n_ind == 1)) return false;
	if (!genotype_mode && !(p.value_bound < 1073741824.0)) return false;
	plan.ped = ped;
	const uint32_t fact_nf = (ped && !genotype_mode && !p.fterms.empty()) ? (TB == 2 && p.fterm_kind == 1 ? (uint32_t)PSLOT_FACT : (TB == 4 && p.fterm_kind == 2 ? (uint32_t)PSLOT_FACT4 : 0u)) : 0u;
	const bool fact = fact_nf != 0;
	lr = ped ? 0 : std::max(1, std::min(lr, SLOT_LR));
	const int n_lane = ped ? 6 - (int)TB : SLOT_LANE;
	plan.col_to_row.assign(n, -1);
	const int LMIN = lr + n_lane, LMAX = lr + n_lane + SLOT_LWMAX;
	if (ped) l_pref = l_pref < 0 ? -l_pref : LMAX;
	l_pref = std::max(LMIN, std::min(l_pref, LMAX));
	const uint32_t max_run_cols = ped ? (uint32_t)PSLOT_MAXCOLS : (uint32_t)SLOT_MAXCOLS;
	const std::vector<uint32_t>& last_col = p.read_last_col;
	std::vector<int32_t>& col_to_row = plan.col_to_row;
	if (ped) plan.prows.resize(n);
	else {
		plan.rows.reserve((size_t)n + SLOT_ROW_PAD);
		plan.rows.resize(n);
	}
	plan.bt_cols.resize(n);
	auto& rows_g = plan.rows;
	auto& prows_g = plan.prows;
	auto& btc_g = plan.bt_cols;
	auto plan_range = [&](const uint32_t c_begin, const uint32_t c_end, SlotPlan& plan, std::vector<RunDraft>& drafts) {
	std::vector<int8_t> slot_of(p.n_reads, -1);
	SlotRow scratch_row{};
	PedSlotRow scratch_prow{};
	uint32_t c = c_begin;
	while (c < c_end) {
		auto column_step = [&]() { plan.steps.push_back(Step{0, c}); ++c; };
		if (c + 1 >= n && !genotype_mode) { column_step(); continue; }
		const uint32_t b0 = p.b[c];
		const ColumnEntry* first = p.col_begin(c);
		constexpr uint32_t LOOK = 12;
		uint32_t kmax_at[LOOK], n_look = 0;
		for (uint32_t cc = c; cc < std::min(n, c + LOOK); ++cc) {
			if (cc > c && p.b[cc] == 0) break;
			kmax_at[n_look] = std::max<uint32_t>(n_look ? kmax_at[n_look - 1] : 0u, p.k[cc]);
			++n_look;
		}
		const uint32_t kmax = kmax_at[std::min<uint32_t>(n_look, genotype_mode ? 6u : LOOK) - 1];
		const uint32_t L = std::min<uint32_t>((uint32_t)l_pref, std::max<uint32_t>((uint32_t)LMIN, kmax));
		uint32_t g = kmax > L ? kmax - L : 0;
		if (genotype_mode) g = std::min(g, b0);
		std::vector<uint32_t> order(b0);
		for (uint32_t j = 0; j < b0; ++j) order[j] = j;
		std::stable_sort(order.begin(), order.end(), [&](uint32_t a, uint32_t bb) {
			const uint32_t ea = last_col[first[a].read_id], eb = last_col[first[bb].read_id];
			if (ea != eb) return ea > eb;
			return a > bb;
		});
		if (!genotype_mode) {
			auto probe = [&](uint32_t gg) -> uint32_t {
				uint32_t grid_end = 0xFFFFFFFFu;
				for (uint32_t i = 0; i < gg; ++i) grid_end = std::min(grid_end, last_col[first[order[i]].read_id]);
				uint32_t n_free = L - (b0 - gg), ends = 0, c1 = c;
				for (; c1 < n && c1 - c < max_run_cols; ++c1) {
					if (c1 + 1 == n || c1 >= grid_end || c1 >= c_end || (c1 > c && p.b[c1] == 0)) break;
					const uint32_t kc = p.k[c1], bc = c1 == c ? b0 : p.b[c1], n_new = kc - bc, n_end = kc - p.f[c1];
					if (n_end > (uint32_t)(ped ? PSLOT_MAXEND : SLOT_MAXEND) || ends + n_end > (uint32_t)SLOT_MAXENDS_RUN || n_new > n_free) break;
					n_free = n_free - n_new + n_end;
					ends += n_end;
				}
				return c1 - c;
			};
			uint32_t best_g = 0xFFFFFFFFu, best_len = 0, last_g = 0xFFFFFFFFu;
			for (uint32_t q = 0; q < n_look; ++q) {
				const uint32_t gg = kmax_at[q] > L ? kmax_at[q] - L : 0;
				if (gg == last_g) continue;
				last_g = gg;
				if (gg > b0 || gg > (uint32_t)SLOT_GMAX || p.k[c] > L + gg || b0 - gg > L) continue;
				const uint32_t len = probe(gg);
				if (len > best_len) { best_len = len; best_g = gg; }
			}
			if (best_g == 0xFFFFFFFFu) { column_step(); continue; }
			g = best_g;
		}
		if (g > b0 || g > (uint32_t)SLOT_GMAX || p.k[c] > L + g) { column_step(); continue; }
		if (genotype_mode) {
			while (g > 0 && c + 1 < n && last_col[first[order[g - 1]].read_id] <= c) --g;
			if (p.k[c] > L + g) { column_step(); continue; }
		}
		RunDraft d;
		d.c0 = c; d.g = g; d.L = L; d.lw = L - (uint32_t)LMIN;
		const uint32_t nslots = L + g;
		d.entry_read.assign(nslots, -1);
		uint32_t grid_end = 0xFFFFFFFFu;
		{
			std::vector<uint32_t> grid_reads;
			for (uint32_t i = 0; i < g; ++i) {
				grid_reads.push_back(first[order[i]].read_id);
				grid_end = std::min(grid_end, last_col[first[order[i]].read_id]);
			}
			std::stable_sort(grid_reads.begin(), grid_reads.end(), [&](uint32_t a, uint32_t bb) {
				if (last_col[a] != last_col[bb]) return last_col[a] < last_col[bb];
				return a < bb;
			});
			if (g >= 5) {
				d.entry_read[L + g - 1] = (int32_t)grid_reads[g - 1];
				for (uint32_t i = 0; i < 3; ++i) d.entry_read[L + i] = (int32_t)grid_reads[g - 4 + i];
				for (uint32_t i = 3; i + 1 < g; ++i) d.entry_read[L + i] = (int32_t)grid_reads[i - 3];
			} else {
				for (uint32_t i = 0; i < g; ++i) d.entry_read[L + i] = (int32_t)grid_reads[i];
			}
			uint32_t s = 0;
			for (uint32_t i = b0; i-- > g;) d.entry_read[s++] = (int32_t)first[order[i]].read_id;
		}
		std::vector<int32_t> cur = d.entry_read;
		auto release_marks = [&]() {
			for (int32_t r : d.entry_read) if (r >= 0) slot_of[r] = -1;
			for (int32_t r : cur) if (r >= 0) slot_of[r] = -1;
		};
		for (uint32_t s = 0; s < nslots; ++s) if (cur[s] >= 0) slot_of[cur[s]] = (int8_t)s;
		const size_t rows_mark = c, ends_mark = plan.end_slots.size(), starts_mark = plan.start_slots.size();
		std::vector<int32_t> started;
		uint32_t c1 = c, n_ends = 0;
		bool symmetric = true;
		uint32_t run_forms = 2;
		while (c1 < n && c1 - c < max_run_cols) {
			if (c1 + 1 == n && !genotype_mode) break;
			if (c1 >= grid_end && !(genotype_mode && c1 + 1 == n)) break;
			if (c1 >= c_end) break;
			if (c1 > c && p.b[c1] == 0) break;
			const ColumnEntry* col = p.col_begin(c1);
			const uint32_t kc = p.k[c1], bc = c1 == c ? b0 : p.b[c1];
			const uint32_t n_new = kc - bc, n_end = kc - p.f[c1];
			if (!genotype_mode && (n_end > (uint32_t)(ped ? PSLOT_MAXEND : SLOT_MAXEND) || n_ends + n_end > (uint32_t)SLOT_MAXENDS_RUN)) break;
			if (genotype_mode && n_ends + n_end > 250u) break;
			if (genotype_mode && c1 > c && run_lds_bytes(64u << d.lw, c1 - c + 1, p.T, 2u * p.P, 1u << p.P) > GS_MAX_LDS) break;
			uint32_t n_free = 0;
			for (uint32_t s = 0; s < L; ++s) n_free += cur[s] < 0;
			if (n_new > n_free) break;
			bool ok = true;
			if (!ped) {
				const int32_t* dcol = p.delta.data() + (size_t)p.col_ptr[c1];
				uint32_t bad = 0;
				for (uint32_t j = 0; j < kc; ++j) bad |= (uint32_t)(std::abs(dcol[j]) >= SLOT_DELTA_LIMIT);
				for (uint32_t j = 0; j < bc; ++j) bad |= (uint32_t)(slot_of[col[j].read_id] < 0);
				ok = bad == 0;
			}
			if (ped && !genotype_mode) {
				uint32_t most = 0;
				for (uint32_t t = 0; t < p.T; ++t) most = std::max<uint32_t>(most, (uint32_t)(p.term_end(c1, t) - p.term_begin(c1, t)));
				if (!fact && (most > (uint32_t)PSLOT_MAXFORMS || (most > 4u && TB != 2u))) {
					if (debug_env("WHAMD_DEBUG_PLAN")) fprintf(stderr, "[plan] column %u: %u cost forms per transmission value: no pedigree run\n", c1, most);
					break;
				}
				const uint32_t nf = fact ? pslot_na(fact_nf) : std::max(run_forms, most > 4 ? 16u : (most > 2 ? 4u : 2u));
				if ((c1 - c + 1) * pslot_ta(fact_nf, p.T) * nf > (uint32_t)PSLOT_FORMWORDS) break;
				run_forms = nf;
			}
			if (ped) for (uint32_t j = 0; j < bc && ok; ++j) ok = slot_of[col[j].read_id] >= 0;
			if (!ok) break;
			{
				uint32_t s = 0;
				for (uint32_t j = bc; j < kc; ++j) {
					while (cur[s] >= 0) ++s;
					cur[s] = (int32_t)col[j].read_id;
					slot_of[col[j].read_id] = (int8_t)s;
					started.push_back((int32_t)col[j].read_id);
					if (genotype_mode) plan.start_slots.push_back((uint8_t)s);
				}
			}
			const int32_t* dl = genotype_mode ? nullptr : p.delta.data() + (size_t)p.col_ptr[c1] * p.n_ind;
			SlotRow& row = ped ? scratch_row : rows_g[c1];
			PedSlotRow& prow = ped ? prows_g[c1] : scratch_prow;
			if (ped) prow = PedSlotRow{}; else row = SlotRow{};
			SlotBtCol bc_rec{};
			bc_rec.k = (uint8_t)kc;
			bc_rec.kf = (uint8_t)n_ends;
			if (ped) {
				prow.recomb = p.recomb[c1];
				for (uint32_t j = 0; j < kc; ++j) {
					const int s = slot_of[col[j].read_id];
					if (!genotype_mode) prow.dslot[s] = dl[(size_t)col[j].sample * kc + j];
					prow.ind[s] = col[j].sample;
					bc_rec.slot[j] = (uint8_t)s;
				}
				symmetric = false;
			} else {
				uint32_t Cp = RES_ABSENT, Cm = RES_ABSENT, Cc = INF;
				for (uint64_t q = p.term_begin(c1, 0); q < p.term_end(c1, 0); ++q) {
					const CostTerm& t = p.terms[q];
					if (t.plus) Cp = t.c;
					else if (t.minus) Cm = t.c;
					else Cc = std::min(Cc, t.c);
				}
				row.K = Cp + Cm;
				row.Cc = Cc;
				row.Cp = Cp;
				uint32_t dsum = 0;
				for (uint32_t j = 0; j < kc; ++j) {
					const int s = slot_of[col[j].read_id];
					row.dslot[s] = dl[j];
					dsum += (uint32_t)dl[j];
					bc_rec.slot[j] = (uint8_t)s;
				}
				for (int s = 0; s < lr; ++s) row.dreg[s] = row.dslot[s];
				for (int s = 0; s < SLOT_LANE; ++s) row.dlane[s] = row.dslot[lr + s];
				const bool both_absent = Cp == RES_ABSENT && Cm == RES_ABSENT;
				if (!both_absent && (Cp == RES_ABSENT || Cm == RES_ABSENT || Cp + dsum != Cm)) symmetric = false;
			}
			uint32_t en = 0;
			const uint32_t ending_bits = ~p.fwd_mask[c1] & (kc >= 32 ? 0xFFFFFFFFu : ((1u << kc) - 1u));
			for (uint32_t rest = ending_bits; rest; rest &= rest - 1u) {
				const uint32_t j = (uint32_t)__builtin_ctz(rest);
				if (genotype_mode && c1 + 1 == n) break;
				const int s = slot_of[col[j].read_id];
				if (s >= (int)L) { ok = false; break; }
				uint32_t M = 0;
				for (uint32_t q = j + 1; q < kc; ++q) M |= 1u << slot_of[col[q].read_id];
				const uint32_t mflip = parity32(M);
				uint32_t qmask = 0;
				for (uint32_t r = 0; r < (1u << lr); ++r) {
					uint32_t bit = parity32(r & M);
					if (s < lr) bit ^= ((r >> s) & 1u) & mflip;
					qmask |= bit << r;
				}
				if (qmask & 1u) { ok = false; break; }
				if (en < (uint32_t)SLOT_MAXEND) {
					row.end[en].info = (uint32_t)s | (qmask << 8) | (mflip << 24);
					row.end[en].M = s >= lr ? M ^ (mflip << s) : M;
				}
				if (ped && !genotype_mode) {
					if (en == 0) { prow.info0 = (uint32_t)s; prow.M0 = M; }
					else if (en == 1) { prow.info1 = (uint32_t)s; prow.M1 = M; }
					else if (en == 2) { prow.info2 = (uint32_t)s; prow.M2 = M; }
					else { prow.pad[2] = (uint32_t)s; prow.pad[3] = M; }
					if (en < 3) bc_rec.slot[25 + en] = (uint8_t)s; else bc_rec.pad[1] = (uint8_t)s;
				}
				plan.end_slots.push_back((uint8_t)s);
				++en;
			}
			if (!ok) break;
			row.n_end = en;
			prow.n_end = en;
			if (ped) bc_rec.pad[0] = (uint8_t)en;
			if (genotype_mode) {
				prow.pad[0] = n_new;
				prow.pad[1] = (uint32_t)(plan.start_slots.size() - starts_mark) - n_new;
			}
			for (uint32_t rest = ending_bits; rest; rest &= rest - 1u) cur[slot_of[col[__builtin_ctz(rest)].read_id]] = -1;
			n_ends += en;
			col_to_row[c1] = (int32_t)c1;
			btc_g[c1] = bc_rec;
			++c1;
		}
		{
			size_t keep = 0;
			for (size_t i = rows_mark; i < c1; ++i) keep += ped ? prows_g[i].n_end : rows_g[i].n_end;
			plan.end_slots.resize(ends_mark + keep);
			if (genotype_mode) {
				size_t keep_starts = 0;
				for (size_t i = rows_mark; i < c1; ++i) keep_starts += prows_g[i].pad[0];
				plan.start_slots.resize(starts_mark + keep_starts);
			}
		}
		if (c1 - c < (genotype_mode ? 1u : 2u)) {
			for (uint32_t cc = c; cc < c1; ++cc) col_to_row[cc] = -1;
			plan.end_slots.resize(ends_mark);
			plan.start_slots.resize(starts_mark);
			release_marks();
			for (int32_t r : started) slot_of[r] = -1;
			column_step();
			continue;
		}
		d.exit_read.assign(nslots, -1);
		{
			const ColumnEntry* col = p.col_begin(c1 - 1);
			for (uint32_t j = 0; j < p.k[c1 - 1]; ++j)
				if ((p.fwd_mask[c1 - 1] >> j) & 1u) d.exit_read[btc_g[c1 - 1].slot[j]] = (int32_t)col[j].read_id;
		}
		release_marks();
		for (int32_t r : started) slot_of[r] = -1;
		d.ncols = c1 - c;
		d.symmetric = symmetric;
		SlotRun run{};
		run.c0 = c; run.ncols = d.ncols; run.g = g; run.L = L; run.lw = d.lw;
		run.ctrl_off = (uint32_t)plan.ctrl.size();
		plan.ctrl.resize(plan.ctrl.size() + SLOT_CTRL_WORDS, 0);
		uint32_t exchanges = 0;
		for (uint32_t i = 0; i < d.ncols; ++i) {
			if (!ped) {
				SlotRow& xrow = rows_g[rows_mark + i];
				for (uint32_t k = 0; k < std::min<uint32_t>(xrow.n_end, SLOT_MAXEND); ++k) {
					if ((xrow.end[k].info & 31u) < (uint32_t)(lr + SLOT_LANE)) continue;
					if (exchanges & 1u) xrow.end[k].info |= 1u << 16;
					++exchanges;
				}
			}
			const uint32_t ne = ped ? prows_g[rows_mark + i].n_end : rows_g[rows_mark + i].n_end;
			const uint32_t s0 = ped ? prows_g[rows_mark + i].info0 : (rows_g[rows_mark + i].end[0].info & 31u);
			const uint32_t byte = std::min(ne, 3u) | ((ne ? (s0 & 31u) : 0u) << 2);
			if (ped) plan.ctrl[run.ctrl_off + (i >> 2)] |= byte << ((i & 3u) * 8u);
			else {
				const uint32_t qm = ne ? ((rows_g[rows_mark + i].end[0].info >> 8) & 255u) : 0u;
				const uint32_t xbuf = ne ? ((rows_g[rows_mark + i].end[0].info >> 16) & 1u) : 0u;
				plan.ctrl[run.ctrl_off + (i >> 1)] |= (byte | (qm << 7) | (xbuf << 15)) << ((i & 1u) * 16u);
			}
		}
		run.lr = (uint32_t)lr;
		run.row_off = (uint32_t)rows_mark;
		run.n_ends = 0;
		for (size_t i = rows_mark; i < c1; ++i) run.n_ends += ped ? prows_g[i].n_end : rows_g[i].n_end;
		if (ped) {
			PedSlotExtra ex{};
			ex.tb = TB;
			ex.nf = 2;
			for (uint32_t i = 0; i < d.ncols && !genotype_mode; ++i)
				for (uint32_t t = 0; t < p.T; ++t) {
					const uint32_t cnt = (uint32_t)(p.term_end(c + i, t) - p.term_begin(c + i, t));
					ex.nf = std::max(ex.nf, cnt > 4 ? 16u : (cnt > 2 ? 4u : 2u));
				}
			if (fact) ex.nf = fact_nf;
			if (fact_nf == (uint32_t)PSLOT_FACT4) { ex.pad[0] = p.fact4_roles[0]; ex.pad[1] = p.fact4_roles[1]; }
			ex.fwn = d.ncols * pslot_ta(ex.nf, p.T) * pslot_na(ex.nf);
			ex.arow = (ex.fwn + 3u) & ~3u;
			ex.rec_words = ((d.ncols + 3u) / 4u) * (64u << d.lw);
			plan.pextra.push_back(ex);
		}
		run.threads = 64u << d.lw;
		run.has_prev = c > 0;
		run.half = (use_symmetry > 0 && symmetric && g >= 1) ? 1u : 0u;
		for (uint32_t s = 0; s < nslots; ++s) {
			if (d.entry_read[s] >= 0) run.in_occ |= 1u << s;
			if (d.exit_read[s] >= 0) run.out_occ |= 1u << s;
		}
		plan.steps.push_back(Step{2, (uint32_t)plan.runs.size()});
		plan.runs.push_back(run);
		plan.end_off.push_back((uint32_t)ends_mark);
		plan.start_off.push_back((uint32_t)starts_mark);
		drafts.push_back(d);
		plan.n_run_columns += d.ncols;
		c = c1;
	}
	};
	std::vector<RunDraft> drafts;
	const auto tp1 = std::chrono::steady_clock::now();
	const long pf1 = thread_minor_faults();
	long pf2 = pf1;
	auto tp2 = tp1;
	{
		const uint32_t n_pieces = slot_plan_pieces(n);
		std::vector<SlotPlan> parts(n_pieces);
		std::vector<std::vector<RunDraft>> part_drafts(n_pieces);
		std::vector<uint32_t> bounds(n_pieces + 1);
		for (uint32_t t = 0; t <= n_pieces; ++t) bounds[t] = slot_plan_piece_begin(n, t);
		parallel_ranges(n_pieces, host_threads(n_pieces, 1), [&](uint64_t q0, uint64_t q1, uint32_t) {
			for (uint64_t q = q0; q < q1; ++q) plan_range(bounds[q], bounds[q + 1], parts[q], part_drafts[q]);
		});
		tp2 = std::chrono::steady_clock::now();
		pf2 = thread_minor_faults();
		const uint32_t n_threads = n_pieces;
		{
			size_t n_steps = 0, n_runs = 0, n_ends_all = 0, n_starts = 0, n_ctrl = 0, n_extra = 0;
			for (const SlotPlan& q : parts) {
				n_steps += q.steps.size(); n_runs += q.runs.size(); n_ends_all += q.end_slots.size(); n_starts += q.start_slots.size();
				n_ctrl += q.ctrl.size(); n_extra += q.pextra.size();
			}
			plan.steps.reserve(n_steps); plan.runs.reserve(n_runs); plan.end_off.reserve(n_runs); plan.start_off.reserve(n_runs);
			plan.end_slots.reserve(n_ends_all); plan.start_slots.reserve(n_starts); plan.ctrl.reserve(n_ctrl); plan.pextra.reserve(n_extra);
			drafts.reserve(n_runs);
		}
		for (uint32_t t = 0; t < n_threads; ++t) {
			const SlotPlan& q = parts[t];
			const uint32_t run_base = (uint32_t)plan.runs.size();
			const uint32_t end_base = (uint32_t)plan.end_slots.size(), ctrl_base = (uint32_t)plan.ctrl.size();
			for (Step st : q.steps) { if (st.kind == 2) st.index += run_base; plan.steps.push_back(st); }
			for (SlotRun run : q.runs) { run.ctrl_off += ctrl_base; plan.runs.push_back(run); }
			plan.pextra.insert(plan.pextra.end(), q.pextra.begin(), q.pextra.end());
			for (uint32_t off : q.end_off) plan.end_off.push_back(off + end_base);
			for (uint32_t off : q.start_off) plan.start_off.push_back(off + (uint32_t)plan.start_slots.size());
			plan.start_slots.insert(plan.start_slots.end(), q.start_slots.begin(), q.start_slots.end());
			plan.end_slots.insert(plan.end_slots.end(), q.end_slots.begin(), q.end_slots.end());
			plan.ctrl.insert(plan.ctrl.end(), q.ctrl.begin(), q.ctrl.end());
			plan.n_run_columns += q.n_run_columns;
			drafts.insert(drafts.end(), std::make_move_iterator(part_drafts[t].begin()), std::make_move_iterator(part_drafts[t].end()));
		}
	}
	const auto tp3 = std::chrono::steady_clock::now();
	const long pf3 = thread_minor_faults();
	const bool timing = getenv("WHAMD_DEBUG_TIMING") != nullptr;
	const double concatenated_at = timing ? timing_stamp_ms() : 0.0;
	double lap_ms[7] = {0, 0, 0, 0, 0, 0, 0};
	auto lap_from = tp3;
	auto lap = [&](int which) {
		if (!timing) return;
		const auto now = std::chrono::steady_clock::now();
		lap_ms[which] += std::chrono::duration<double, std::milli>(now - lap_from).count();
		lap_from = now;
	};
	const size_t n_steps = plan.steps.size();
	for (size_t si = 0; si < n_steps; ++si) {
		const uint32_t c0 = plan.steps[si].kind == 2 ? plan.runs[plan.steps[si].index].c0 : plan.steps[si].index;
		if (!ped && (si == 0 || p.b[c0] == 0)) plan.component_first_step.push_back((uint32_t)si);
	}
	lap(0);
	const bool head_first = head && head->at_head && !ped && !genotype_mode;
	size_t n_head = 0;
	if (head_first)
		while (n_head < n_steps && plan.steps[n_head].kind == 2 && plan.steps[n_head].index == n_head && plan.runs[n_head].c0 + plan.runs[n_head].ncols <= head->col_limit) ++n_head;
	std::vector<uint64_t> B;
	std::vector<uint8_t> yrun;
	if (!ped && (lr == 2 || lr == 3) && !debug_env("WHAMD_NO_YFORM")) {
		std::vector<uint8_t> pure(n, 0);
		B.assign((size_t)n + 1, 0);
		parallel_ranges(n, host_threads(n, 8192), [&](uint64_t c_lo, uint64_t c_hi, uint32_t) {
			for (uint32_t c = (uint32_t)c_lo; c < (uint32_t)c_hi; ++c) {
				uint64_t kstar = 0;
				uint32_t Cp = RES_ABSENT, Cm = RES_ABSENT, Cc = INF;
				for (uint64_t q = p.term_begin(c, 0); q < p.term_end(c, 0); ++q) {
					const CostTerm& t = p.terms[q];
					if (t.plus) Cp = t.c; else if (t.minus) Cm = t.c; else Cc = std::min(Cc, t.c);
				}
				pure[c] = Cp != RES_ABSENT && Cm != RES_ABSENT && Cc == INF;
				if (pure[c]) {
					kstar = (uint64_t)(uint32_t)(Cp + Cm);
				} else {
					uint64_t dabs = 0, ub = ~0ull;
					const int32_t* dl = p.delta.data() + (size_t)p.col_ptr[c];
					for (uint32_t j = 0; j < p.k[c]; ++j) dabs += (uint64_t)std::abs((int64_t)dl[j]);
					for (uint64_t q = p.term_begin(c, 0); q < p.term_end(c, 0); ++q) {
						const CostTerm& t = p.terms[q];
						ub = std::min<uint64_t>(ub, (uint64_t)t.c + ((t.plus || t.minus) ? dabs : 0));
					}
					kstar = 2 * (ub == ~0ull ? 0 : ub);
				}
				B[c + 1] = kstar;
			}
		});
		for (uint32_t c = 0; c < n; ++c) B[c + 1] += B[c];
		lap(1);
		if (B[n] < 0xFFFFFFF0ull) {
			yrun.assign(plan.runs.size(), 0);
			parallel_ranges(plan.runs.size(), host_threads(plan.runs.size(), 512), [&](uint64_t r_lo, uint64_t r_hi, uint32_t) {
				for (size_t ri = r_lo; ri < r_hi; ++ri) {
					const SlotRun& run = plan.runs[ri];
					bool ok = run.lr == 2 || run.lr == 3;
					for (uint32_t i = 0; i < run.ncols && ok; ++i) ok = pure[run.c0 + i];
					yrun[ri] = ok;
				}
			});
		}
		lap(2);
	}
	auto rewrite_rows = [&](const size_t s_first, const size_t s_last) {
		if (yrun.empty()) return;
		parallel_ranges(s_last - s_first, host_threads(s_last - s_first, 256), [&](uint64_t s_lo, uint64_t s_hi, uint32_t) {
		for (size_t si = s_first + s_lo; si < s_first + s_hi; ++si) {
			if (plan.steps[si].kind != 2 || !yrun[plan.steps[si].index]) continue;
			SlotRun& run = plan.runs[plan.steps[si].index];
			auto y_neighbour = [&](size_t sj) { return plan.steps[sj].kind == 2 && yrun[plan.steps[sj].index]; };
			const bool in = si > 0 && p.b[run.c0] != 0 && y_neighbour(si - 1);
			bool out = false;
			if (si + 1 < n_steps && y_neighbour(si + 1)) out = p.b[plan.runs[plan.steps[si + 1].index].c0] != 0;
			run.yflags = 1u | (in ? 2u : 0u) | (out ? 4u : 0u);
			run.base_in = (uint32_t)B[run.c0];
			run.base_out = (uint32_t)B[run.c0 + run.ncols];
			for (uint32_t i = 0; i < run.ncols; ++i) {
				SlotRow& row = plan.rows[run.row_off + i];
				const uint32_t K = row.K, dreg[3] = {(uint32_t)row.dreg[0], (uint32_t)row.dreg[1], (uint32_t)row.dreg[2]};
				uint32_t* words = reinterpret_cast<uint32_t*>(&row);
				for (uint32_t r = 0; r < (1u << run.lr); ++r) {
					uint32_t dsum = 0;
					for (uint32_t sb = 0; sb < run.lr; ++sb) if ((r >> sb) & 1u) dsum += dreg[sb];
					words[r] = K - 2u * dsum + SLOT_YBIAS;
				}
			}
		}
		});
	};
	if (ped && !genotype_mode) {
		if (plan.n_run_columns * 2 < n) return false;
		uint64_t words = 0;
		for (size_t ri = 0; ri < plan.runs.size(); ++ri) {
			const SlotRun& run = plan.runs[ri];
			PedSlotExtra& ex = plan.pextra[ri];
			ex.g_lo = (uint32_t)words;
			ex.g_hi = (uint32_t)(words >> 32);
			if (p.value_bound < (double)((1u << (31u - TB)) - 1u) && !debug_env("WHAMD_NO_PED_KEYS")) plan.runs[ri].yflags |= 16u;
			const uint64_t gsz = ((uint64_t)1 << run.g) * ex.fwn;
			ex.w_off = (uint32_t)gsz;
			ex.s_off = (uint32_t)(gsz + ((uint64_t)1 << run.lw) * ex.fwn);
			words += (uint64_t)ex.s_off + (uint64_t)run.ncols * 64u * pslot_ns(ex.nf) + (uint64_t)run.ncols * p.T * pslot_nk(ex.nf);
			if (run.ncols <= (uint32_t)SLOT_XCOLS && run.n_ends <= (uint32_t)SLOT_XENDS && ex.nf != (uint32_t)PSLOT_FACT4 && debug_env("WHAMD_PED_XRUN") && !debug_env("WHAMD_NO_XRUN")) {
				plan.runs[ri].yflags |= 8u;
				ex.x_off = (uint32_t)(words - (((uint64_t)ex.g_hi << 32) | ex.g_lo));
				words += (pslotx_words(run.ncols, run.threads, run.g) + 3u) & ~(uint64_t)3;
			}
		}
		if (debug_env("WHAMD_PED_XRUN")) words += 65536;
		plan.table_words = words;
	}
	plan.f_exit.assign(plan.runs.size(), 0);
	plan.exit_slot.assign(plan.runs.size(), std::vector<uint8_t>());
	auto exit_slots = [&](const size_t s_first, const size_t s_last) {
	parallel_ranges(s_last - s_first, host_threads(s_last - s_first, 512), [&](uint64_t s_begin, uint64_t s_end, uint32_t) {
	for (size_t si = s_first + s_begin; si < s_first + s_end; ++si) {
		if (plan.steps[si].kind != 2) continue;
		const size_t ri = plan.steps[si].index;
		const SlotRun& run = plan.runs[ri];
		const uint32_t cl = run.c0 + run.ncols - 1;
		const SlotBtCol& bc = plan.bt_cols[run.row_off + run.ncols - 1];
		for (uint32_t j = 0; j < p.k[cl]; ++j)
			if ((p.fwd_mask[cl] >> j) & 1u) plan.exit_slot[ri].push_back(bc.slot[j]);
		plan.f_exit[ri] = (uint32_t)plan.exit_slot[ri].size();
	}
	});
	};
	auto link_layouts = [&](const size_t s_first, const size_t s_last) {
	parallel_ranges(s_last - s_first, host_threads(s_last - s_first, 512), [&](uint64_t s_begin, uint64_t s_end, uint32_t) {
	for (size_t si = s_first + s_begin; si < s_first + s_end; ++si) {
		if (plan.steps[si].kind != 2) continue;
		const uint32_t ri = plan.steps[si].index;
		SlotRun& B = plan.runs[ri];
		const RunDraft& db = drafts[ri];
		const bool prev_is_run = si > 0 && plan.steps[si - 1].kind == 2 && B.has_prev;
		if (prev_is_run) {
		} else if (B.has_prev) {
			const ColumnEntry* first = p.col_begin(B.c0);
			std::memset(B.in_pos, 0, sizeof B.in_pos);
			for (uint32_t j = 0; j < p.b[B.c0]; ++j) {
				for (uint32_t s = 0; s < B.L + B.g; ++s)
					if (db.entry_read[s] == (int32_t)first[j].read_id) slot_set_pos(B.in_pos, s, j);
			}
			B.in_fullmask = p.b[B.c0] >= 32 ? 0xFFFFFFFFu : ((1u << p.b[B.c0]) - 1u);
		}
		const bool next_is_run = si + 1 < plan.steps.size() && plan.steps[si + 1].kind == 2 &&
		                         plan.runs[plan.steps[si + 1].index].has_prev;
		if (next_is_run) {
			SlotRun& C = plan.runs[plan.steps[si + 1].index];
			const RunDraft& dc = drafts[plan.steps[si + 1].index];
			const uint32_t nb = B.L + B.g, nc = C.L + C.g;
			std::vector<std::pair<uint32_t, uint32_t>> local_keys;
			std::vector<int> slot_in_b(nc, -1);
			for (uint32_t t = 0; t < nc; ++t) {
				if (dc.entry_read[t] < 0) continue;
				for (uint32_t s2 = 0; s2 < nb; ++s2) if (db.exit_read[s2] == dc.entry_read[t]) slot_in_b[t] = (int)s2;
			}
			for (uint32_t t = 0; t < C.L; ++t) {
				if (dc.entry_read[t] < 0) continue;
				const uint32_t s2 = (uint32_t)slot_in_b[t];
				uint32_t key = s2;
				if (s2 >= B.L) {
					const uint32_t gi = s2 - B.L;
					key = (B.g >= 5 && gi + 1 == B.g) ? 3000u : ((B.g >= 5 && gi < 3) ? 2000u + gi : 1000u + gi);
				}
				local_keys.push_back({key, t});
			}
			std::sort(local_keys.begin(), local_keys.end());
			const uint32_t n_loc = (uint32_t)local_keys.size();
			std::memset(C.in_pos, 0, sizeof C.in_pos);
			for (uint32_t i = 0; i < n_loc; ++i) slot_set_pos(C.in_pos, local_keys[i].second, i);
			for (uint32_t i = 0; i < C.g; ++i) slot_set_pos(C.in_pos, C.L + i, n_loc + i);
			C.in_identity = 1;
			for (uint32_t t = 0; t < nc; ++t) if (dc.entry_read[t] >= 0 && slot_pos(C.in_pos, t) != t) C.in_identity = 0;
			C.in_fullmask = (n_loc + C.g) >= 32 ? 0xFFFFFFFFu : ((1u << (n_loc + C.g)) - 1u);
			for (uint32_t t = 0; t < nc; ++t) if (slot_in_b[t] >= 0) slot_set_pos(B.out_pos, (uint32_t)slot_in_b[t], slot_pos(C.in_pos, t));
			B.out_fullmask = C.in_fullmask;
			if (B.half) {
				C.in_half = 1;
				C.in_mirror_pos = slot_pos(B.out_pos, B.L + B.g - 1);
			}
		} else {
			for (uint32_t j = 0; j < plan.f_exit[ri]; ++j) slot_set_pos(B.out_pos, plan.exit_slot[ri][j], j);
			B.out_fullmask = plan.f_exit[ri] >= 32 ? 0xFFFFFFFFu : ((1u << plan.f_exit[ri]) - 1u);
			B.mirror_out = B.half;
		}
	}
	});
	};
	auto finish_steps = [&](const size_t s_first, const size_t s_last) {
		rewrite_rows(s_first, s_last);
		lap(3);
		exit_slots(s_first, s_last);
		lap(4);
		link_layouts(s_first, s_last);
		lap(5);
	};
	double head_done_at = 0.0;
	if (head_first) {
		finish_steps(0, n_head);
		head_done_at = timing ? timing_stamp_ms() : 0.0;
		head->at_head((uint32_t)n_head);
		lap(6);
		finish_steps(n_head, n_steps);
	} else {
		finish_steps(0, n_steps);
	}
	if (timing) {
		auto ms = [](std::chrono::steady_clock::time_point a, std::chrono::steady_clock::time_point b) { return std::chrono::duration<double, std::milli>(b - a).count(); };
		const double inside = head_first ? lap_ms[6] : 0.0;
		fprintf(stderr, "[whamd timing] slot plan: setup %.1f ms, column ranges %.1f ms, concatenation %.1f ms, layouts %.1f ms (page faults of this thread: %ld, %ld, %ld, %ld)\n",
		        ms(tp0, tp1), ms(tp1, tp2), ms(tp2, tp3), ms(tp3, std::chrono::steady_clock::now()) - inside, pf1 - pf0, pf2 - pf1, pf3 - pf2, thread_minor_faults() - pf3);
		fprintf(stderr, "[whamd timing] slot plan layouts: component list %.2f ms, Y form per column + prefix sum %.2f ms, runs in Y form %.2f ms, rows rewritten %.2f ms, exit slots %.2f ms, "
		        "entry / exit layouts %.2f ms; concatenation done at t = %.2f ms\n", lap_ms[0], lap_ms[1], lap_ms[2], lap_ms[3], lap_ms[4], lap_ms[5], concatenated_at);
		if (head_first)
			fprintf(stderr, "[whamd timing] slot plan head: %zu of %zu steps finished %.2f ms behind the concatenation, %.2f ms inside the callback\n", n_head, n_steps,
			        head_done_at - concatenated_at, inside);
	}
	return true;
}

}
```

### whatshap_amd/csrc/slots.h

```cpp
#pragma once
#include <chrono>
#include <cmath>
#include <cstdint>
#include <functional>
#include <memory>
#include <string>
#include <utility>
#include <vector>

#include "problem.h"
#include "host_parallel.h"
#include "resident.h"

namespace whamd {

constexpr int SLOT_LR = 3;
constexpr int SLOT_LANE = 6;
constexpr int SLOT_LWMAX = 3;
constexpr int SLOT_GMAX = 12;
constexpr int SLOT_MAXSLOTS = 26;
constexpr int SLOT_MAXCOLS = 64;
constexpr int SLOT_MAXEND = 8;
constexpr int PSLOT_MAXEND = 4;
constexpr int SLOT_MAXENDS_RUN = 96;
// ... 94 lines not shown
	uint32_t tb, nf, fwn, arow;
	uint32_t g_lo, g_hi, w_off, s_off;
	uint32_t rec_words, x_off, pad[2];
};
constexpr uint64_t pslotx_words(uint32_t ncols, uint32_t threads, uint32_t g) { return (uint64_t)2 * (ncols + SLOT_XPAD) + threads + ((uint64_t)1 << g); }
static_assert(sizeof(PedSlotExtra) == 48, "PedSlotExtra layout");
inline size_t pedslot_lds_bytes(uint32_t threads, uint32_t ncols, const PedSlotExtra& ex) {
	return ((size_t)2 * threads + (PSLOT_MAXCOLS + 4) * 8 + (size_t)(threads >> 6) * (ex.arow + (4u << ex.tb) * pslot_na(ex.nf)) + (size_t)(ncols + 4) * 64 * pslot_ns(ex.nf) +
	        ((size_t)(ncols + 4) << ex.tb) * pslot_nk(ex.nf)) * 4;
}

struct SlotBatchEntry {
	SlotRun run;
	PedSlotExtra ex;
	const uint32_t* prev;
	uint32_t* cur;
	uint32_t* score_out;
	uint64_t pad;
	const uint32_t* tab;
	const void* rows;
	const uint32_t* ctrl;
	uint8_t* bt;
	unsigned long long* spec_keys;
	uint32_t spec_stride, pad2;
};
static_assert(sizeof(SlotBatchEntry) == 320 && sizeof(SlotBatchEntry) % 64 == 0, "entries are fetched with wide scalar loads, whole 64-byte lines");

constexpr int SLOT_GROUP_MAX = 248;
struct SlotGroupArgs {
	uint32_t n, pad;
	const SlotBatchEntry* entry[SLOT_GROUP_MAX];
};

struct SlotBtCol {
	uint8_t k, kf, pad[2];
	uint8_t slot[28];
};
static_assert(sizeof(SlotBtCol) == 32, "SlotBtCol must stay 8 dwords");

struct SlotBtUnit {
	uint32_t kind, c0, ncols, blob_off;
	uint32_t g, L, n_ends, threads;
	uint32_t bt_lo, bt_hi, half, blob_words;
	uint32_t f_exit, lr, pad0[2];
	uint8_t exit_slot[32];
	uint8_t exit_pos[32];
};
static_assert(sizeof(SlotBtUnit) == 128, "SlotBtUnit must stay 32 words");

template <class T>
using NoInitAllocator = NoInitAlloc<T>;

struct SlotPlan {
	std::vector<Step> steps;
	std::vector<SlotRun> runs;
	std::vector<SlotRow, NoInitAllocator<SlotRow>> rows;
	std::vector<SlotBtCol, NoInitAllocator<SlotBtCol>> bt_cols;
	std::vector<uint8_t> end_slots;
	std::vector<uint32_t> end_off;
	std::vector<uint32_t> f_exit;
	std::vector<std::vector<uint8_t>> exit_slot;
	std::vector<uint32_t> ctrl;
	std::vector<int32_t> col_to_row;
	std::vector<uint32_t> component_first_step;
	uint64_t n_run_columns = 0;
	bool ped = false;
	std::vector<uint8_t> start_slots;
	std::vector<uint32_t> start_off;
	std::vector<PedSlotRow, NoInitAllocator<PedSlotRow>> prows;
	std::vector<PedSlotExtra> pextra;
	uint64_t table_words = 0;
};

constexpr uint32_t PLAN_PIECE = 8192;
inline uint32_t slot_plan_pieces(uint32_t n_cols) { return n_cols / PLAN_PIECE > 1 ? n_cols / PLAN_PIECE : 1; }
inline uint32_t slot_plan_piece_begin(uint32_t n_cols, uint32_t piece) { return (uint32_t)((uint64_t)n_cols * piece / slot_plan_pieces(n_cols)); }

struct SlotPlanHead {
	uint32_t col_limit = 0;
	std::function<void(uint32_t)> at_head;
};
bool plan_forward_slots(const Problem& p, int l_pref, int use_symmetry, SlotPlan& plan, int lr = 2, bool genotype_mode = false, const SlotPlanHead* head = nullptr);
inline double timing_stamp_ms() { return std::fmod(std::chrono::duration<double, std::milli>(std::chrono::steady_clock::now().time_since_epoch()).count(), 1e6); }

bool emulate_slot_plan(const Problem& p, const SlotPlan& plan, std::vector<uint32_t>& path_index, uint32_t& score, std::string& msg);
bool emulate_pedslot_plan(const Problem& p, const SlotPlan& plan, std::vector<uint32_t>& path_index, std::vector<uint32_t>& path_trans,
                          uint32_t& score, std::string& msg);
uint32_t pedslot_table_entry(const Problem& p, const SlotPlan& plan, uint32_t run_index, int kind, uint32_t unit, uint32_t c, uint32_t t, uint32_t f);

}
```

Measured before the change: 2.359 million variant-columns/s.

## Defer single-individual cost terms and slot rows, parallelize problem flattening

For single-individual problems the cost-term lists are no longer built before slot planning. They are filled afterwards, and only for columns that fall outside slot runs. Slot rows are written per run behind the planner walk, using closed-form single-term costs. Problem building now parallelizes the position-monotonicity check, sample validation and the column-pointer prefix sums across host threads. The aim is to cut host-side preprocessing before the first device launch, at the cost of more code paths and extra debug hooks used to verify the eager and lazy plans agree.

After: 2.392 million variant-columns/s, median of 6. +1.4%, better.

```diff
diff --git a/include/whatshap_amd_debug.h b/include/whatshap_amd_debug.h
--- a/include/whatshap_amd_debug.h
+++ b/include/whatshap_amd_debug.h
@@ -128,6 +128,18 @@
                                            const whamd_pedigree_view* pedigree, int distrust_genotypes,
                                            const uint32_t* positions, size_t n_positions, uint32_t head_pieces, whamd_debug_head_plan_result* out);
 
+whamd_status_t whamd_debug_lazy_single_plan(const whamd_readset_view* readset, const uint32_t* recombcost, size_t n_recombcost, const whamd_pedigree_view* pedigree,
+                                            int distrust_genotypes, const uint32_t* positions, size_t n_positions, int* lazy_out, int* planned_out,
+                                            uint64_t* digest_eager_out, uint64_t* digest_lazy_out, uint64_t* columns_outside_runs_out);
+
+typedef struct whamd_debug_flatten_result {
+	uint64_t n_columns, n_reads, n_entries, n_deltas;
+} whamd_debug_flatten_result;
+whamd_status_t whamd_debug_flatten(const whamd_readset_view* readset, const uint32_t* recombcost, size_t n_recombcost, const whamd_pedigree_view* pedigree,
+                                   int distrust_genotypes, const uint32_t* positions, size_t n_positions, uint32_t host_threads,
+                                   whamd_debug_flatten_result* out, uint64_t* col_ptr, uint8_t* k, uint8_t* b, uint8_t* f, uint32_t* read_last_col,
+                                   uint32_t* entry_read, uint32_t* entry_phred, uint8_t* entry_allele, int32_t* delta);
+
 typedef struct whamd_debug_genotype_run {
 	uint32_t c0, ncols;
 	uint32_t rescale_f, rescale_b, emit_f, emit_b;
diff --git a/whatshap_amd/_native.py b/whatshap_amd/_native.py
--- a/whatshap_amd/_native.py
+++ b/whatshap_amd/_native.py
@@ -919,6 +919,36 @@
     return {"lazy": bool(lazy.value), "differences": int(diff.value), "built_before": int(before.value), "built_after": int(after.value)}
 
 
+def debug_lazy_single_plan(problem: ProblemArrays) -> dict:
+    D = debug_lib()
+    fn = D.whamd_debug_lazy_single_plan
+    fn.restype = C.c_int
+    lazy, planned, eager_d, lazy_d, outside = C.c_int(), C.c_int(), C.c_uint64(), C.c_uint64(), C.c_uint64()
+    _check(fn(*problem.call_args(), C.byref(lazy), C.byref(planned), C.byref(eager_d), C.byref(lazy_d), C.byref(outside)), D)
+    return {"lazy": bool(lazy.value), "planned": int(planned.value), "digest_eager": int(eager_d.value), "digest_lazy": int(lazy_d.value),
+            "columns_outside_runs": int(outside.value)}
+
+
+class DebugFlatten(C.Structure):
+    _fields_ = [(name, C.c_uint64) for name in ("n_columns", "n_reads", "n_entries", "n_deltas")]
+
+
+def debug_flatten(problem: ProblemArrays, host_threads: int = 0) -> dict:
+    D = debug_lib()
+    fn = D.whamd_debug_flatten
+    fn.restype = C.c_int
+    out = DebugFlatten()
+    nothing = (None,) * 9
+    _check(fn(*problem.call_args(), C.c_uint32(host_threads), C.byref(out), *nothing), D)
+    n, nr, ne, nd = int(out.n_columns), int(out.n_reads), int(out.n_entries), int(out.n_deltas)
+    sized = (("col_ptr", n + 1, np.uint64), ("k", n, np.uint8), ("b", n, np.uint8), ("f", n, np.uint8), ("read_last_col", nr, np.uint32),
+             ("entry_read", ne, np.uint32), ("entry_phred", ne, np.uint32), ("entry_allele", ne, np.uint8), ("delta", nd, np.int32))
+    arrays = {name: np.zeros(max(size, 1), dtype=dtype) for name, size, dtype in sized}
+    ctype = {np.uint64: C.c_uint64, np.uint8: C.c_uint8, np.uint32: C.c_uint32, np.int32: C.c_int32}
+    _check(fn(*problem.call_args(), C.c_uint32(host_threads), C.byref(out), *[_ptr(arrays[name], ctype[dtype]) for name, _, dtype in sized]), D)
+    return {name: arrays[name][:size] for name, size, _ in sized}
+
+
 class DebugGenotypeRun(C.Structure):
     _fields_ = [(name, C.c_uint32) for name in ("c0", "ncols", "rescale_f", "rescale_b", "emit_f", "emit_b", "n_part_out", "part_out_f", "part_out_b",
                                                 "part_in_f", "n_part_in_f", "part_in_b", "n_part_in_b", "reserved")]
diff --git a/whatshap_amd/csrc/c_api.cpp b/whatshap_amd/csrc/c_api.cpp
--- a/whatshap_amd/csrc/c_api.cpp
+++ b/whatshap_amd/csrc/c_api.cpp
@@ -74,6 +74,7 @@
 	*out = nullptr;
 	if (n_options && (!keys || !values)) return fail(WHAMD_ERR_INVALID, "option arrays are NULL");
 	const double t0 = now_ms();
+	if (getenv("WHAMD_DEBUG_TIMING")) create_entered_at() = std::chrono::steady_clock::now();
 	std::unique_ptr<whamd_dptable> t(new whamd_dptable());
 	std::string msg;
 	struct ThreadsGuard { uint32_t saved = whamd::host_threads_override(); ~ThreadsGuard() { whamd::host_threads_override() = saved; } } threads_guard;
@@ -719,7 +720,7 @@
 	if (st != WHAMD_OK) return fail(st, msg);
 	st = build_problem(readset, recombcost, n_recombcost, pedigree, distrust_genotypes != 0, positions, n_positions, lazy, msg, false, true);
 	if (st != WHAMD_OK) return fail(st, msg);
-	if (lazy_out) *lazy_out = lazy.lazy_terms ? 1 : 0;
+	if (lazy_out) *lazy_out = lazy.lazy_terms && !lazy.lazy_single ? 1 : 0;
 	const uint32_t n = eager.n_cols;
 	uint64_t before = 0, after = 0, diff = 0;
 	for (uint32_t c = 0; c < n; ++c) before += lazy.term_end(c, lazy.T - 1) > lazy.term_begin(c, 0);
@@ -781,6 +782,82 @@
 	if (st != WHAMD_OK) return fail(st, msg);
 	st = DeviceTable::debug_preview_plan(p, pieces, out, rec_predicted, rec_laid_out, spec_predicted, spec_laid_out, capacity, msg);
 	return st == WHAMD_OK ? WHAMD_OK : fail(st, msg);
+	});
+}
+
+whamd_status_t whamd_debug_lazy_single_plan(const whamd_readset_view* readset, const uint32_t* recombcost, size_t n_recombcost, const whamd_pedigree_view* pedigree,
+                                            int distrust_genotypes, const uint32_t* positions, size_t n_positions, int* lazy_out, int* planned_out,
+                                            uint64_t* digest_eager_out, uint64_t* digest_lazy_out, uint64_t* columns_outside_runs_out) {
+	return guarded([&]() -> whamd_status_t {
+	Problem both[2];
+	std::string msg;
+	uint64_t digest[2] = {0, 0}, outside = 0;
+	bool planned[2] = {false, false};
+	for (int k = 0; k < 2; ++k) {
+		whamd_status_t st = build_problem(readset, recombcost, n_recombcost, pedigree, distrust_genotypes != 0, positions, n_positions, both[k], msg, false, k == 1);
+		if (st != WHAMD_OK) return fail(st, msg);
+		SlotPlan sp;
+		planned[k] = both[k].T == 1 && plan_forward_slots(both[k], 11, 1, sp, 2, false);
+		if (!planned[k]) continue;
+		uint64_t h = 1469598103934665603ull;
+		auto mix = [&h](const void* data, size_t bytes) {
+			const unsigned char* b = static_cast<const unsigned char*>(data);
+			for (size_t i = 0; i < bytes; ++i) h = (h ^ b[i]) * 1099511628211ull;
+		};
+		for (size_t ri = 0; ri < sp.runs.size(); ++ri) {
+			const SlotRun& run = sp.runs[ri];
+			mix(&run, sizeof run);
+			mix(sp.rows.data() + run.row_off, (size_t)run.ncols * sizeof(SlotRow));
+			mix(sp.bt_cols.data() + run.row_off, (size_t)run.ncols * sizeof(SlotBtCol));
+			mix(sp.ctrl.data() + run.ctrl_off, (size_t)SLOT_CTRL_WORDS * 4);
+			mix(sp.end_slots.data() + sp.end_off[ri], run.n_ends);
+		}
+		mix(sp.steps.data(), sp.steps.size() * sizeof(Step));
+		mix(sp.col_to_row.data(), sp.col_to_row.size() * 4);
+		digest[k] = h;
+		if (k == 1) for (int32_t r : sp.col_to_row) outside += r < 0;
+	}
+	if (lazy_out) *lazy_out = both[1].lazy_single ? 1 : 0;
+	if (planned_out) *planned_out = planned[0] && planned[1] ? 1 : (planned[0] == planned[1] ? 0 : -1);
+	if (digest_eager_out) *digest_eager_out = digest[0];
+	if (digest_lazy_out) *digest_lazy_out = digest[1];
+	if (columns_outside_runs_out) *columns_outside_runs_out = outside;
+	return WHAMD_OK;
+	});
+}
+
+whamd_status_t whamd_debug_flatten(const whamd_readset_view* readset, const uint32_t* recombcost, size_t n_recombcost, const whamd_pedigree_view* pedigree,
+                                   int distrust_genotypes, const uint32_t* positions, size_t n_positions, uint32_t host_threads_wanted,
+                                   whamd_debug_flatten_result* out, uint64_t* col_ptr, uint8_t* k, uint8_t* b, uint8_t* f, uint32_t* read_last_col,
+                                   uint32_t* entry_read, uint32_t* entry_phred, uint8_t* entry_allele, int32_t* delta) {
+	return guarded([&]() -> whamd_status_t {
+	if (!out) return fail(WHAMD_ERR_INVALID, "out is NULL");
+	struct ThreadsGuard { uint32_t saved = whamd::host_threads_override(); ~ThreadsGuard() { whamd::host_threads_override() = saved; } } threads_guard;
+	whamd::host_threads_override() = host_threads_wanted;
+	Problem p;
+	std::string msg;
+	whamd_status_t st = build_problem(readset, recombcost, n_recombcost, pedigree, distrust_genotypes != 0, positions, n_positions, p, msg);
+	if (st != WHAMD_OK) return fail(st, msg);
+	const bool sized = out->n_columns == p.n_cols && out->n_reads == p.n_reads && out->n_entries == p.entries.size() && out->n_deltas == p.delta.size();
+	out->n_columns = p.n_cols;
+	out->n_reads = p.n_reads;
+	out->n_entries = p.entries.size();
+	out->n_deltas = p.delta.size();
+	if (!col_ptr) return WHAMD_OK;
+	if (!sized || !k || !b || !f || !read_last_col || !entry_read || !entry_phred || !entry_allele || !delta)
+		return fail(WHAMD_ERR_INVALID, "whamd_debug_flatten: the arrays must be sized by a first call (out as that call left it)");
+	if (p.n_cols) std::copy(p.col_ptr.begin(), p.col_ptr.end(), col_ptr); else col_ptr[0] = 0;
+	std::copy(p.k.begin(), p.k.end(), k);
+	std::copy(p.b.begin(), p.b.end(), b);
+	std::copy(p.f.begin(), p.f.end(), f);
+	std::copy(p.read_last_col.begin(), p.read_last_col.end(), read_last_col);
+	for (size_t i = 0; i < p.entries.size(); ++i) {
+		entry_read[i] = p.entries[i].read_id;
+		entry_phred[i] = p.entries[i].phred;
+		entry_allele[i] = p.entries[i].allele;
+	}
+	std::copy(p.delta.begin(), p.delta.end(), delta);
+	return WHAMD_OK;
 	});
 }
 
diff --git a/whatshap_amd/csrc/dp_device.hip b/whatshap_amd/csrc/dp_device.hip
--- a/whatshap_amd/csrc/dp_device.hip
+++ b/whatshap_amd/csrc/dp_device.hip
@@ -460,7 +460,7 @@
 	b.laps.lap("plan: the planner");
 	if (m.tp.use_slots && m.tp.splan.ped && m.tp.splan.table_words * 4ull > free_b / 4) m.tp.use_slots = false;
 	m.tp.table_bytes = m.tp.use_slots && m.tp.splan.ped ? m.tp.splan.table_words * 4ull : 0ull;
-	if (p.lazy_terms) {
+	if (p.lazy_terms && !(p.lazy_single && m.tp.use_slots)) {
 		std::vector<uint8_t> need(p.n_cols, 1);
 		if (m.tp.use_slots && m.tp.splan.ped) for (uint32_t c = 0; c < p.n_cols; ++c) need[c] = m.tp.splan.col_to_row[c] < 0;
 		const whamd_status_t st = fill_lazy_terms(p, need, msg);
@@ -907,9 +907,11 @@
 	pv.runs.resize(S);
 	uint64_t launches = 0;
 	pv.launching = true;
-	if (b.laps.on)
+	if (b.laps.on) {
 		fprintf(stderr, "[whamd timing] preview: first launch %.2f ms after the create's upload began, at t = %.2f ms (%s)\n", b.laps.since_origin_ms(), timing_stamp_ms(),
 		        pv.from_hook ? "from the planner's head hook" : "behind the plan");
+		if (from_create) fprintf(stderr, "[whamd timing] create entered -> preview's first launch: %.2f ms\n", std::chrono::duration<double, std::milli>(std::chrono::steady_clock::now() - create_entered_at()).count());
+	}
 	for (uint32_t k = 0; k < S; ++k) {
 		SlotBatchEntry e{};
 		e.run = runs[k];
@@ -978,6 +980,18 @@
 	if (!m.preview.tried && (st = m.start_preview(p, b, from_create, msg)) != WHAMD_OK) return st;
 	if ((st = describe_columns(p, b, m.tp, msg)) != WHAMD_OK) return st;
 	if ((st = lay_out_arena(p, m.opt, b, m.tp, msg)) != WHAMD_OK) return st;
+	if (p.lazy_single && m.tp.use_slots) {
+		const bool sparse = !b.ped_slots && p.T == 1 && !m.tp.windowed && !debug_env("WHAMD_DENSE_COLUMN_UPLOAD");
+		std::vector<uint8_t> need(p.n_cols, 1);
+		if (sparse) for (uint32_t c = 0; c < p.n_cols; ++c) need[c] = m.tp.splan.col_to_row[c] < 0;
+		if ((st = fill_lazy_terms(p, need, msg)) != WHAMD_OK) return st;
+		if (p.terms.size() >= 0xFFFFFFFFull) { msg = "term lists exceed 32-bit offsets"; return WHAMD_ERR_OVERFLOW; }
+		parallel_ranges(p.n_cols, host_threads(p.n_cols, 16384), [&](uint64_t c0, uint64_t c1, uint32_t) {
+			for (uint64_t c = c0; c < c1; ++c)
+				for (uint32_t t = 0; t <= p.T; ++t) b.term_ptr32[(size_t)c * (p.T + 1) + t] = (uint32_t)p.term_ptr[(size_t)c * p.T + t];
+		});
+		b.laps.lap("terms filled after planning");
+	}
 	TableUploader up(device, m.upload_stream, m.dev.allocations);
 	b.laps.lap("staging area taken");
 	up.open_block(upload_bound(p, b, m.tp));
diff --git a/whatshap_amd/csrc/problem.cpp b/whatshap_amd/csrc/problem.cpp
--- a/whatshap_amd/csrc/problem.cpp
+++ b/whatshap_amd/csrc/problem.cpp
@@ -76,6 +76,11 @@
 	return true;
 }
 
+uint32_t flatten_threads(uint64_t n_items, uint64_t grain) {
+	if (const char* e = debug_env("WHAMD_FLATTEN_GRAIN")) grain = (uint64_t)std::max(1, atoi(e));
+	return host_threads(n_items, grain);
+}
+
 }
 
 whamd_status_t build_problem(const whamd_readset_view* rs, const uint32_t* recombcost, size_t n_recombcost,
@@ -101,7 +106,7 @@
 	p.read_ptr.assign(rs->n_reads + 1, 0);
 	if (rs->n_reads) std::copy(rs->read_ptr, rs->read_ptr + rs->n_reads + 1, p.read_ptr.begin());
 	{
-		const uint32_t n_threads = host_threads(nnz, 1u << 18);
+		const uint32_t n_threads = flatten_threads(nnz, 1u << 18);
 		std::vector<uint8_t> bad(n_threads, 0);
 		parallel_ranges(nnz, n_threads, [&](uint64_t i0, uint64_t i1, uint32_t t) {
 			if (i1 <= i0) return;
@@ -163,7 +168,16 @@
 	const uint32_t n = p.n_cols;
 	lap("pedigree + positions");
 	bool positions_increase = true;
-	for (uint32_t i = 1; i < n && positions_increase; ++i) positions_increase = p.positions[i - 1] < p.positions[i];
+	{
+		const uint32_t n_threads = flatten_threads(n, 1u << 15);
+		std::vector<uint8_t> falls(n_threads, 0);
+		parallel_ranges(n, n_threads, [&](uint64_t i0, uint64_t i1, uint32_t t) {
+			bool ok = true;
+			for (uint32_t i = std::max<uint32_t>((uint32_t)i0, 1u); i < (uint32_t)i1 && ok; ++i) ok = p.positions[i - 1] < p.positions[i];
+			falls[t] = !ok;
+		});
+		for (uint8_t v : falls) positions_increase = positions_increase && !v;
+	}
 	std::unordered_map<uint32_t, uint32_t> position_map;
 	if (!positions_increase) {
 		position_map.reserve(n * 2 + 1);
@@ -190,16 +204,20 @@
 	};
 	p.read_first_col.resize(p.n_reads);
 	p.read_last_col.resize(p.n_reads);
+	std::vector<uint32_t> unknown_sample;
 	std::vector<uint32_t>&first_col = p.read_first_col, &last_col = p.read_last_col;
 	{
 		struct ReadError { uint32_t read = 0xFFFFFFFFu; whamd_status_t status = WHAMD_OK; std::string msg; };
-		const uint32_t n_threads = positions_increase ? host_threads(p.n_reads, 1u << 14) : 1u;
+		const uint32_t n_threads = positions_increase ? flatten_threads(p.n_reads, 1u << 12) : 1u;
 		std::vector<ReadError> errors(n_threads);
+		p.read_source.resize(p.n_reads);
+		unknown_sample.assign(n_threads, 0xFFFFFFFFu);
 		const uint64_t* ptr = rs->read_ptr;
 		const int32_t* vp = rs->var_position;
 		parallel_ranges(p.n_reads, n_threads, [&](uint64_t r0, uint64_t r1, uint32_t t) {
 			auto fail_read = [&](uint32_t r, whamd_status_t st, std::string m) { errors[t].read = r; errors[t].status = st; errors[t].msg = std::move(m); };
 			uint32_t hint_col = 0;
+			std::string ignored;
 			for (uint32_t r = (uint32_t)r0; r < (uint32_t)r1; ++r) {
 				const uint64_t lo = ptr[r], hi = ptr[r + 1];
 				if (hi <= lo || hi > nnz) return fail_read(r, WHAMD_ERR_INVALID, "No variants present");
@@ -215,6 +233,7 @@
 				first_col[r] = fc;
 				last_col[r] = lc;
 				hint_col = fc;
+				if (!id_to_index(p, (uint32_t)rs->read_sample_id[r], p.read_source[r], ignored) && unknown_sample[t] == 0xFFFFFFFFu) unknown_sample[t] = r;
 			}
 		});
 		for (const ReadError& e : errors) {
@@ -229,9 +248,11 @@
 		return WHAMD_ERR_INVALID;
 	}
 	lap("position map + read validation");
-	p.read_source.resize(p.n_reads);
-	for (uint32_t r = 0; r < p.n_reads; ++r) {
-		if (!id_to_index(p, (uint32_t)rs->read_sample_id[r], p.read_source[r], msg)) return WHAMD_ERR_INVALID;
+	for (uint32_t r : unknown_sample) {
+		if (r != 0xFFFFFFFFu) {
+			(void)id_to_index(p, (uint32_t)rs->read_sample_id[r], p.read_source[r], msg);
+			return WHAMD_ERR_INVALID;
+		}
 	}
 	if (n && p.n_ind && p.n_variants < n) {
 		msg = "pedigree has fewer variants (" + std::to_string(p.n_variants) + ") than there are columns (" + std::to_string(n) + ")";
@@ -258,9 +279,9 @@
 	if (!build_partitions(p, msg)) return WHAMD_ERR_INVALID;
 	if (n == 0) return WHAMD_OK;
 
-	std::vector<uint32_t> start_idx(n + 2, 0);
-	p.col_ptr.assign(n + 1, 0);
-	{
+	std::vector<uint32_t> start_idx(n + 2);
+	p.col_ptr.resize(n + 1);
+	if (flatten_threads(n, 6144) == 1 && flatten_threads(p.n_reads, 1u << 14) == 1) {
 		std::vector<int64_t> diff(n + 1, 0);
 		for (uint32_t r = 0; r < p.n_reads; ++r) {
 			start_idx[first_col[r] + 1]++;
@@ -269,6 +290,7 @@
 		}
 		for (uint32_t c = 0; c <= n; ++c) start_idx[c + 1] += start_idx[c];
 		int64_t cov = 0;
+		p.col_ptr[0] = 0;
 		for (uint32_t c = 0; c < n; ++c) {
 			cov += diff[c];
 			if (cov > (int64_t)MAX_COVERAGE) {
@@ -276,6 +298,55 @@
 				return WHAMD_ERR_UNSUPPORTED;
 			}
 			p.col_ptr[c + 1] = p.col_ptr[c] + (uint64_t)cov;
+		}
+	} else {
+		std::vector<uint32_t> ends(n, 0);
+		const uint32_t nr = p.n_reads;
+		const uint32_t read_ranges = flatten_threads(nr, 1u << 14);
+		parallel_ranges(nr, read_ranges, [&](uint64_t r0, uint64_t r1, uint32_t) {
+			for (uint32_t r = (uint32_t)r0; r < (uint32_t)r1; ++r) {
+				for (uint32_t c = r == 0 ? 0u : first_col[r - 1] + 1u; c <= first_col[r]; ++c) start_idx[c] = r;
+				if (read_ranges > 1) __atomic_fetch_add(&ends[last_col[r]], 1u, __ATOMIC_RELAXED);
+				else ++ends[last_col[r]];
+			}
+			if (r1 == nr) for (uint32_t c = nr ? first_col[nr - 1] + 1u : 0u; c < n + 2; ++c) start_idx[c] = nr;
+		});
+		const uint32_t n_ranges = flatten_threads(n, 6144);
+		struct RangeSums { uint64_t ends = 0, ended_before = 0, started = 0; };
+		std::vector<RangeSums> sums(n_ranges);
+		parallel_ranges(n, n_ranges, [&](uint64_t c0, uint64_t c1, uint32_t t) {
+			RangeSums s;
+			for (uint32_t c = (uint32_t)c0; c < (uint32_t)c1; ++c) {
+				s.ended_before += s.ends;
+				s.ends += ends[c];
+				s.started += start_idx[c + 1];
+			}
+			sums[t] = s;
+		});
+		std::vector<uint64_t> ended_at(n_ranges + 1, 0), ptr_at(n_ranges + 1, 0);
+		for (uint32_t t = 0; t < n_ranges; ++t) {
+			const uint64_t width = (uint64_t)n * (t + 1) / n_ranges - (uint64_t)n * t / n_ranges;
+			ended_at[t + 1] = ended_at[t] + sums[t].ends;
+			ptr_at[t + 1] = ptr_at[t] + sums[t].started - (width * ended_at[t] + sums[t].ended_before);
+		}
+		struct Over { uint32_t column = 0xFFFFFFFFu; uint64_t coverage = 0; };
+		std::vector<Over> over(n_ranges);
+		parallel_ranges(n, n_ranges, [&](uint64_t c0, uint64_t c1, uint32_t t) {
+			uint64_t ended = ended_at[t], ptr = ptr_at[t];
+			if (c0 == 0) p.col_ptr[0] = 0;
+			for (uint32_t c = (uint32_t)c0; c < (uint32_t)c1; ++c) {
+				const uint64_t cov = start_idx[c + 1] - ended;
+				if (cov > (uint64_t)MAX_COVERAGE && over[t].column == 0xFFFFFFFFu) over[t] = Over{c, cov};
+				ptr += cov;
+				p.col_ptr[c + 1] = ptr;
+				ended += ends[c];
+			}
+		});
+		for (const Over& o : over) {
+			if (o.column != 0xFFFFFFFFu) {
+				msg = "coverage " + std::to_string(o.coverage) + " at column " + std::to_string(o.column) + " exceeds the device limit of " + std::to_string(MAX_COVERAGE);
+				return WHAMD_ERR_UNSUPPORTED;
+			}
 		}
 	}
 	lap("column pointers");
@@ -448,6 +519,9 @@
 	auto lazy_sample = [](uint32_t c) { return c < 256u || (c & 63u) == 0u; };
 	p.lazy_terms = false;
 	const bool single_trusted = p.n_ind == 1 && p.T == 1 && p.P == 2 && !distrust && p.h2p.size() >= 2 && p.h2p[0] == 0 && p.h2p[1] == 1 && !debug_env("WHAMD_NO_SINGLE_FAST_TERMS");
+	const bool lazy_single = single_trusted && lazy_fact_terms && !columns_only && !debug_env("WHAMD_EAGER_TERMS");
+	p.lazy_single = false;
+	if (lazy_single) p.col_rw.resize(2 * (size_t)n);
 	struct CompatCache {
 		bool enabled = false;
 		std::vector<uint8_t> known;
@@ -503,7 +577,11 @@
 		bool any = false;
 		if (single_trusted) {
 			const uint8_t g = p.genotype[c];
-			if (g == 1) {
+			if (lazy_single) {
+				p.col_rw[2 * (size_t)c] = R[0];
+				p.col_rw[2 * (size_t)c + 1] = W[0];
+				any = g <= 2;
+			} else if (g == 1) {
 				out.terms.push_back(CostTerm{W[0] - R[0], 0, 1u});
 				out.terms.push_back(CostTerm{R[0], 1u, 0});
 				any = true;
@@ -652,7 +730,7 @@
 	};
 	double bound = 0.0;
 	{
-		const uint32_t n_threads = host_threads(n, 8192);
+		const uint32_t n_threads = flatten_threads(n, 8192);
 		std::vector<RangeResult> parts(n_threads);
 		std::vector<uint32_t> bounds(n_threads + 1);
 		for (uint32_t t = 0; t <= n_threads; ++t) bounds[t] = (uint32_t)((uint64_t)n * t / n_threads);
@@ -666,7 +744,8 @@
 				parallel_ranges(n, n_threads, [&](uint64_t c0, uint64_t c1, uint32_t t) { columns_range((uint32_t)c0, (uint32_t)c1, parts[t]); });
 			}
 		}
-		p.lazy_terms = lazy;
+		p.lazy_terms = lazy || lazy_single;
+		p.lazy_single = lazy_single;
 		for (uint32_t t = 0; t < n_threads; ++t) p.max_k = std::max(p.max_k, parts[t].max_k);
 		lap("column entries, indexing scheme, deltas + cost terms");
 		if (columns_only) return WHAMD_OK;
@@ -702,6 +781,23 @@
 whamd_status_t fill_lazy_terms(Problem& p, const std::vector<uint8_t>& need, std::string& msg) {
 	if (!p.lazy_terms) return WHAMD_OK;
 	const uint32_t n = p.n_cols;
+	if (p.lazy_single && p.terms_built.empty() && p.terms.empty() && need.size() >= n) {
+		p.terms_built.assign(n, 0);
+		std::vector<CostTerm> made;
+		for (uint32_t c = 0; c < n; ++c) {
+			p.term_ptr[c] = made.size();
+			if (!need[c]) continue;
+			const uint32_t R = p.col_rw[2 * (size_t)c], W = p.col_rw[2 * (size_t)c + 1];
+			const uint8_t g = p.genotype[c];
+			if (g == 1) { made.push_back(CostTerm{W - R, 0, 1u}); made.push_back(CostTerm{R, 1u, 0}); }
+			else if (g == 0) made.push_back(CostTerm{R, 0, 0});
+			else if (g == 2) made.push_back(CostTerm{W - R, 0, 0});
+			p.terms_built[c] = 1;
+		}
+		p.term_ptr[n] = made.size();
+		p.terms.assign(made.begin(), made.end());
+		return WHAMD_OK;
+	}
 	if (p.terms_built.size() != n) {
 		p.terms_built.assign(n, 0);
 		for (uint32_t c = 0; c < n; ++c) p.terms_built[c] = p.term_end(c, p.T - 1) > p.term_begin(c, 0);
diff --git a/whatshap_amd/csrc/problem.h b/whatshap_amd/csrc/problem.h
--- a/whatshap_amd/csrc/problem.h
+++ b/whatshap_amd/csrc/problem.h
@@ -60,6 +60,8 @@
 	RawVec<CostTerm> fterms;
 	uint32_t fterm_kind = 0;
 	bool lazy_terms = false;
+	bool lazy_single = false;
+	RawVec<uint32_t> col_rw;
 	std::vector<uint8_t> terms_built;
 	uint32_t fact4_roles[2] = {0, 0};
 	RawVec<int32_t> delta;
@@ -71,6 +73,24 @@
 	uint64_t term_begin(uint32_t c, uint32_t t) const { return term_ptr[(size_t)c * T + t]; }
 	uint64_t term_end(uint32_t c, uint32_t t) const { return term_ptr[(size_t)c * T + t + 1]; }
 };
+
+inline void single_forms(const Problem& p, uint32_t c, uint32_t absent, uint32_t& Cp, uint32_t& Cm, uint32_t& Cc) {
+	Cp = absent; Cm = absent; Cc = INF;
+	if (p.lazy_single && p.term_end(c, 0) == p.term_begin(c, 0)) {
+		const uint32_t R = p.col_rw[2 * (size_t)c], W = p.col_rw[2 * (size_t)c + 1];
+		const uint8_t g = p.genotype[c];
+		if (g == 1) { Cm = W - R; Cp = R; }
+		else if (g == 0) Cc = R;
+		else if (g == 2) Cc = W - R;
+		return;
+	}
+	for (uint64_t q = p.term_begin(c, 0); q < p.term_end(c, 0); ++q) {
+		const CostTerm& t = p.terms[q];
+		if (t.plus) Cp = t.c;
+		else if (t.minus) Cm = t.c;
+		else Cc = t.c < Cc ? t.c : Cc;
+	}
+}
 
 whamd_status_t build_problem(const whamd_readset_view* rs, const uint32_t* recombcost, size_t n_recombcost,
                              const whamd_pedigree_view* ped, bool distrust, const uint32_t* positions,
diff --git a/whatshap_amd/csrc/slot_plan.cpp b/whatshap_amd/csrc/slot_plan.cpp
--- a/whatshap_amd/csrc/slot_plan.cpp
+++ b/whatshap_amd/csrc/slot_plan.cpp
@@ -57,9 +57,12 @@
 	auto& rows_g = plan.rows;
 	auto& prows_g = plan.prows;
 	auto& btc_g = plan.bt_cols;
+	const bool defer_rows = !ped && !genotype_mode && head && head->at_head && !debug_env("WHAMD_ROWS_IN_WALK");
 	auto plan_range = [&](const uint32_t c_begin, const uint32_t c_end, SlotPlan& plan, std::vector<RunDraft>& drafts) {
 	std::vector<int8_t> slot_of(p.n_reads, -1);
 	SlotRow scratch_row{};
+	std::vector<SlotRow> walk_rows(defer_rows ? max_run_cols : 0u);
+	auto row_of = [&](size_t col, size_t run_c0) -> SlotRow& { return defer_rows ? walk_rows[col - run_c0] : rows_g[col]; };
 	PedSlotRow scratch_prow{};
 	uint32_t c = c_begin;
 	while (c < c_end) {
@@ -198,9 +201,9 @@
 				}
 			}
 			const int32_t* dl = genotype_mode ? nullptr : p.delta.data() + (size_t)p.col_ptr[c1] * p.n_ind;
-			SlotRow& row = ped ? scratch_row : rows_g[c1];
+			SlotRow& row = ped ? scratch_row : row_of(c1, c);
 			PedSlotRow& prow = ped ? prows_g[c1] : scratch_prow;
-			if (ped) prow = PedSlotRow{}; else row = SlotRow{};
+			if (ped) prow = PedSlotRow{}; else if (!defer_rows) row = SlotRow{};
 			SlotBtCol bc_rec{};
 			bc_rec.k = (uint8_t)kc;
 			bc_rec.kf = (uint8_t)n_ends;
@@ -214,17 +217,18 @@
 				}
 				symmetric = false;
 			} else {
-				uint32_t Cp = RES_ABSENT, Cm = RES_ABSENT, Cc = INF;
-				for (uint64_t q = p.term_begin(c1, 0); q < p.term_end(c1, 0); ++q) {
-					const CostTerm& t = p.terms[q];
-					if (t.plus) Cp = t.c;
-					else if (t.minus) Cm = t.c;
-					else Cc = std::min(Cc, t.c);
-				}
+				uint32_t Cp, Cm, Cc;
+				single_forms(p, c1, RES_ABSENT, Cp, Cm, Cc);
+				uint32_t dsum = 0;
+				if (defer_rows) {
+					for (uint32_t j = 0; j < kc; ++j) {
+						dsum += (uint32_t)dl[j];
+						bc_rec.slot[j] = (uint8_t)slot_of[col[j].read_id];
+					}
+				} else {
 				row.K = Cp + Cm;
 				row.Cc = Cc;
 				row.Cp = Cp;
-				uint32_t dsum = 0;
 				for (uint32_t j = 0; j < kc; ++j) {
 					const int s = slot_of[col[j].read_id];
 					row.dslot[s] = dl[j];
@@ -233,6 +237,7 @@
 				}
 				for (int s = 0; s < lr; ++s) row.dreg[s] = row.dslot[s];
 				for (int s = 0; s < SLOT_LANE; ++s) row.dlane[s] = row.dslot[lr + s];
+				}
 				const bool both_absent = Cp == RES_ABSENT && Cm == RES_ABSENT;
 				if (!both_absent && (Cp == RES_ABSENT || Cm == RES_ABSENT || Cp + dsum != Cm)) symmetric = false;
 			}
@@ -243,14 +248,15 @@
 				if (genotype_mode && c1 + 1 == n) break;
 				const int s = slot_of[col[j].read_id];
 				if (s >= (int)L) { ok = false; break; }
-				uint32_t M = 0;
+				uint32_t M = 0, mflip = 0, qmask = 0;
+				if (!(defer_rows && en > 0)) {
 				for (uint32_t q = j + 1; q < kc; ++q) M |= 1u << slot_of[col[q].read_id];
-				const uint32_t mflip = parity32(M);
-				uint32_t qmask = 0;
+				mflip = parity32(M);
 				for (uint32_t r = 0; r < (1u << lr); ++r) {
 					uint32_t bit = parity32(r & M);
 					if (s < lr) bit ^= ((r >> s) & 1u) & mflip;
 					qmask |= bit << r;
+				}
 				}
 				if (qmask & 1u) { ok = false; break; }
 				if (en < (uint32_t)SLOT_MAXEND) {
@@ -283,7 +289,7 @@
 		}
 		{
 			size_t keep = 0;
-			for (size_t i = rows_mark; i < c1; ++i) keep += ped ? prows_g[i].n_end : rows_g[i].n_end;
+			for (size_t i = rows_mark; i < c1; ++i) keep += ped ? prows_g[i].n_end : row_of(i, rows_mark).n_end;
 			plan.end_slots.resize(ends_mark + keep);
 			if (genotype_mode) {
 				size_t keep_starts = 0;
@@ -317,27 +323,27 @@
 		uint32_t exchanges = 0;
 		for (uint32_t i = 0; i < d.ncols; ++i) {
 			if (!ped) {
-				SlotRow& xrow = rows_g[rows_mark + i];
+				SlotRow& xrow = row_of(rows_mark + i, rows_mark);
 				for (uint32_t k = 0; k < std::min<uint32_t>(xrow.n_end, SLOT_MAXEND); ++k) {
 					if ((xrow.end[k].info & 31u) < (uint32_t)(lr + SLOT_LANE)) continue;
 					if (exchanges & 1u) xrow.end[k].info |= 1u << 16;
 					++exchanges;
 				}
 			}
-			const uint32_t ne = ped ? prows_g[rows_mark + i].n_end : rows_g[rows_mark + i].n_end;
-			const uint32_t s0 = ped ? prows_g[rows_mark + i].info0 : (rows_g[rows_mark + i].end[0].info & 31u);
+			const uint32_t ne = ped ? prows_g[rows_mark + i].n_end : row_of(rows_mark + i, rows_mark).n_end;
+			const uint32_t s0 = ped ? prows_g[rows_mark + i].info0 : (row_of(rows_mark + i, rows_mark).end[0].info & 31u);
 			const uint32_t byte = std::min(ne, 3u) | ((ne ? (s0 & 31u) : 0u) << 2);
 			if (ped) plan.ctrl[run.ctrl_off + (i >> 2)] |= byte << ((i & 3u) * 8u);
 			else {
-				const uint32_t qm = ne ? ((rows_g[rows_mark + i].end[0].info >> 8) & 255u) : 0u;
-				const uint32_t xbuf = ne ? ((rows_g[rows_mark + i].end[0].info >> 16) & 1u) : 0u;
+				const uint32_t qm = ne ? ((row_of(rows_mark + i, rows_mark).end[0].info >> 8) & 255u) : 0u;
+				const uint32_t xbuf = ne ? ((row_of(rows_mark + i, rows_mark).end[0].info >> 16) & 1u) : 0u;
 				plan.ctrl[run.ctrl_off + (i >> 1)] |= (byte | (qm << 7) | (xbuf << 15)) << ((i & 1u) * 16u);
 			}
 		}
 		run.lr = (uint32_t)lr;
 		run.row_off = (uint32_t)rows_mark;
 		run.n_ends = 0;
-		for (size_t i = rows_mark; i < c1; ++i) run.n_ends += ped ? prows_g[i].n_end : rows_g[i].n_end;
+		for (size_t i = rows_mark; i < c1; ++i) run.n_ends += ped ? prows_g[i].n_end : row_of(i, rows_mark).n_end;
 		if (ped) {
 			PedSlotExtra ex{};
 			ex.tb = TB;
@@ -417,7 +423,7 @@
 	const long pf3 = thread_minor_faults();
 	const bool timing = getenv("WHAMD_DEBUG_TIMING") != nullptr;
 	const double concatenated_at = timing ? timing_stamp_ms() : 0.0;
-	double lap_ms[7] = {0, 0, 0, 0, 0, 0, 0};
+	double lap_ms[9] = {0, 0, 0, 0, 0, 0, 0, 0, 0};
 	auto lap_from = tp3;
 	auto lap = [&](int which) {
 		if (!timing) return;
@@ -443,11 +449,8 @@
 		parallel_ranges(n, host_threads(n, 8192), [&](uint64_t c_lo, uint64_t c_hi, uint32_t) {
 			for (uint32_t c = (uint32_t)c_lo; c < (uint32_t)c_hi; ++c) {
 				uint64_t kstar = 0;
-				uint32_t Cp = RES_ABSENT, Cm = RES_ABSENT, Cc = INF;
-				for (uint64_t q = p.term_begin(c, 0); q < p.term_end(c, 0); ++q) {
-					const CostTerm& t = p.terms[q];
-					if (t.plus) Cp = t.c; else if (t.minus) Cm = t.c; else Cc = std::min(Cc, t.c);
-				}
+				uint32_t Cp, Cm, Cc;
+				single_forms(p, c, RES_ABSENT, Cp, Cm, Cc);
 				pure[c] = Cp != RES_ABSENT && Cm != RES_ABSENT && Cc == INF;
 				if (pure[c]) {
 					kstar = (uint64_t)(uint32_t)(Cp + Cm);
@@ -455,6 +458,11 @@
 					uint64_t dabs = 0, ub = ~0ull;
 					const int32_t* dl = p.delta.data() + (size_t)p.col_ptr[c];
 					for (uint32_t j = 0; j < p.k[c]; ++j) dabs += (uint64_t)std::abs((int64_t)dl[j]);
+					if (p.lazy_single && p.term_end(c, 0) == p.term_begin(c, 0)) {
+						if (Cp != RES_ABSENT) ub = std::min<uint64_t>(ub, (uint64_t)Cp + dabs);
+						if (Cm != RES_ABSENT) ub = std::min<uint64_t>(ub, (uint64_t)Cm + dabs);
+						if (Cc != INF) ub = std::min<uint64_t>(ub, (uint64_t)Cc);
+					}
 					for (uint64_t q = p.term_begin(c, 0); q < p.term_end(c, 0); ++q) {
 						const CostTerm& t = p.terms[q];
 						ub = std::min<uint64_t>(ub, (uint64_t)t.c + ((t.plus || t.minus) ? dabs : 0));
@@ -479,6 +487,56 @@
 		}
 		lap(2);
 	}
+	auto write_rows = [&](const size_t s_first, const size_t s_last) {
+		if (!defer_rows) return;
+		parallel_ranges(s_last - s_first, host_threads(s_last - s_first, 64), [&](uint64_t s_lo, uint64_t s_hi, uint32_t) {
+		for (size_t si = s_first + s_lo; si < s_first + s_hi; ++si) {
+			if (plan.steps[si].kind != 2) continue;
+			const SlotRun& run = plan.runs[plan.steps[si].index];
+			uint32_t exchanges = 0;
+			for (uint32_t i = 0; i < run.ncols; ++i) {
+				const uint32_t c1 = run.c0 + i, kc = p.k[c1];
+				const SlotBtCol& bc = plan.bt_cols[run.row_off + i];
+				SlotRow& row = plan.rows[run.row_off + i];
+				row = SlotRow{};
+				uint32_t Cp, Cm, Cc;
+				single_forms(p, c1, RES_ABSENT, Cp, Cm, Cc);
+				row.K = Cp + Cm;
+				row.Cc = Cc;
+				row.Cp = Cp;
+				const int32_t* dl = p.delta.data() + (size_t)p.col_ptr[c1];
+				for (uint32_t j = 0; j < kc; ++j) row.dslot[bc.slot[j]] = dl[j];
+				for (int s = 0; s < lr; ++s) row.dreg[s] = row.dslot[s];
+				for (int s = 0; s < SLOT_LANE; ++s) row.dlane[s] = row.dslot[lr + s];
+				uint32_t en = 0;
+				const uint32_t ending_bits = ~p.fwd_mask[c1] & (kc >= 32 ? 0xFFFFFFFFu : ((1u << kc) - 1u));
+				for (uint32_t rest = ending_bits; rest; rest &= rest - 1u) {
+					const uint32_t j = (uint32_t)__builtin_ctz(rest);
+					const int s = bc.slot[j];
+					uint32_t M = 0;
+					for (uint32_t q = j + 1; q < kc; ++q) M |= 1u << bc.slot[q];
+					const uint32_t mflip = parity32(M);
+					uint32_t qmask = 0;
+					for (uint32_t r = 0; r < (1u << lr); ++r) {
+						uint32_t bit = parity32(r & M);
+						if (s < lr) bit ^= ((r >> s) & 1u) & mflip;
+						qmask |= bit << r;
+					}
+					if (en < (uint32_t)SLOT_MAXEND) {
+						row.end[en].info = (uint32_t)s | (qmask << 8) | (mflip << 24);
+						row.end[en].M = s >= lr ? M ^ (mflip << s) : M;
+						if (s >= lr + SLOT_LANE) {
+							if (exchanges & 1u) row.end[en].info |= 1u << 16;
+							++exchanges;
+						}
+					}
+					++en;
+				}
+				row.n_end = en;
+			}
+		}
+		});
+	};
 	auto rewrite_rows = [&](const size_t s_first, const size_t s_last) {
 		if (yrun.empty()) return;
 		parallel_ranges(s_last - s_first, host_threads(s_last - s_first, 256), [&](uint64_t s_lo, uint64_t s_hi, uint32_t) {
@@ -605,7 +663,9 @@
 	}
 	});
 	};
-	auto finish_steps = [&](const size_t s_first, const size_t s_last) {
+	auto finish_steps = [&](const size_t s_first, const size_t s_last, const bool rest) {
+		write_rows(s_first, s_last);
+		lap(rest ? 8 : 7);
 		rewrite_rows(s_first, s_last);
 		lap(3);
 		exit_slots(s_first, s_last);
@@ -615,13 +675,13 @@
 	};
 	double head_done_at = 0.0;
 	if (head_first) {
-		finish_steps(0, n_head);
+		finish_steps(0, n_head, false);
 		head_done_at = timing ? timing_stamp_ms() : 0.0;
 		head->at_head((uint32_t)n_head);
 		lap(6);
-		finish_steps(n_head, n_steps);
+		finish_steps(n_head, n_steps, true);
 	} else {
-		finish_steps(0, n_steps);
+		finish_steps(0, n_steps, false);
 	}
 	if (timing) {
 		auto ms = [](std::chrono::steady_clock::time_point a, std::chrono::steady_clock::time_point b) { return std::chrono::duration<double, std::milli>(b - a).count(); };
@@ -630,6 +690,8 @@
 		        ms(tp0, tp1), ms(tp1, tp2), ms(tp2, tp3), ms(tp3, std::chrono::steady_clock::now()) - inside, pf1 - pf0, pf2 - pf1, pf3 - pf2, thread_minor_faults() - pf3);
 		fprintf(stderr, "[whamd timing] slot plan layouts: component list %.2f ms, Y form per column + prefix sum %.2f ms, runs in Y form %.2f ms, rows rewritten %.2f ms, exit slots %.2f ms, "
 		        "entry / exit layouts %.2f ms; concatenation done at t = %.2f ms\n", lap_ms[0], lap_ms[1], lap_ms[2], lap_ms[3], lap_ms[4], lap_ms[5], concatenated_at);
+		fprintf(stderr, "[whamd timing] slot plan rows: %s: rows of the head %.2f ms, rows of the rest %.2f ms\n", defer_rows ? "written per run behind the walk" : "written in the walk",
+		        lap_ms[7], lap_ms[8]);
 		if (head_first)
 			fprintf(stderr, "[whamd timing] slot plan head: %zu of %zu steps finished %.2f ms behind the concatenation, %.2f ms inside the callback\n", n_head, n_steps,
 			        head_done_at - concatenated_at, inside);
diff --git a/whatshap_amd/csrc/slots.h b/whatshap_amd/csrc/slots.h
--- a/whatshap_amd/csrc/slots.h
+++ b/whatshap_amd/csrc/slots.h
@@ -200,6 +200,7 @@
 };
 bool plan_forward_slots(const Problem& p, int l_pref, int use_symmetry, SlotPlan& plan, int lr = 2, bool genotype_mode = false, const SlotPlanHead* head = nullptr);
 inline double timing_stamp_ms() { return std::fmod(std::chrono::duration<double, std::milli>(std::chrono::steady_clock::now().time_since_epoch()).count(), 1e6); }
+inline std::chrono::steady_clock::time_point& create_entered_at() { static thread_local std::chrono::steady_clock::time_point at; return at; }
 
 bool emulate_slot_plan(const Problem& p, const SlotPlan& plan, std::vector<uint32_t>& path_index, uint32_t& score, std::string& msg);
 bool emulate_pedslot_plan(const Problem& p, const SlotPlan& plan, std::vector<uint32_t>& path_index, std::vector<uint32_t>& path_trans,
```
